# ai4co/rl4co

Hardware: AMD Instinct MI355X
Metric: decode_steps_per_sec (higher is better)
Workload: dtype bf16; 1 GPU; BASELINE configs[1]: TSPEnv num_loc=100 batch=4096/GPU AttentionModel(3L,d128,h8) greedy rollout, bf16 encoder GEMMs, bf16 cache; leg=c2_greedy, batch_per_gpu=4096, cache_dtype=bf16, launch=pipeline, input=one synthetic batch resident in HBM, reused by every step, parallelism=replicas x1 (instances sharded)

## Files before the change

### include/rl4co_amd.h

```cpp
#ifndef RL4CO_AMD_H
#define RL4CO_AMD_H

#include <stdint.h>

#ifdef __cplusplus
extern "C" {
#endif

#define RL4CO_ABI_VERSION 15

#define RL4CO_OK 0
#define RL4CO_ERR_ARG 1
#define RL4CO_ERR_HIP 2
#define RL4CO_ERR_UNSUPPORTED 3

#define RL4CO_EBIT_NAN_LOGIT 1
#define RL4CO_EBIT_INFEASIBLE 2
#define RL4CO_EBIT_INVALID_TOUR 4
#define RL4CO_EBIT_CAPACITY 8
#define RL4CO_EBIT_MAX_STEPS 16
#define RL4CO_EBIT_NEG_INF_LOGP 32
#define RL4CO_EBIT_DUPLICATES 64
#define RL4CO_EBIT_MAX_LENGTH 128
#define RL4CO_EBIT_PRIZE 256
#define RL4CO_EBIT_NOT_ALL_NODES 512
#define RL4CO_EBIT_DEPOT_MIDDLE 1024
#define RL4CO_EBIT_NO_PICKUP 2048
#define RL4CO_EBIT_TW_NEGATIVE 4096
#define RL4CO_EBIT_TW_RETURN 8192
#define RL4CO_EBIT_TW_DURATION 16384
#define RL4CO_EBIT_TW_EMPTY 32768
#define RL4CO_EBIT_TW_DEADLINE 65536

#define RL4CO_ENV_TSP 0
#define RL4CO_ENV_CVRP 1
#define RL4CO_ENV_OP 2
#define RL4CO_ENV_PCTSP 3
#define RL4CO_ENV_PDP 4
#define RL4CO_ENV_CVRPTW 5
#define RL4CO_ENV_SDVRP 6
#define RL4CO_ENV_MTSP 7

#define RL4CO_DECODE_GREEDY 0
#define RL4CO_DECODE_SAMPLE 1
#define RL4CO_DECODE_EVALUATE 2

#define RL4CO_DT_F32 0
#define RL4CO_DT_BF16 1
#define RL4CO_DT_F16 2

#define RL4CO_VARIANT_AUTO 0
#define RL4CO_VARIANT_STREAM 1
#define RL4CO_VARIANT_LDS 2
#define RL4CO_VARIANT_WIDE 3
#define RL4CO_VARIANT_MS 4

#define RL4CO_EMBED_DIM 128
#define RL4CO_NUM_HEADS 8

const char* rl4co_version(void);
int rl4co_abi_version(void);
const char* rl4co_last_error(void);

int rl4co_gather_by_index_f32(const float* src, const int64_t* idx, int B, int N, int D,
                              int K, float* out, int32_t* err, void* stream);

int rl4co_tour_length_f32(const float* locs, const int64_t* actions, int B, int B_locs, int N,
                          int T, int prepend_depot, int negate, float* out, void* stream);
int rl4co_tour_length_dyn_f32(const float* locs, const int64_t* actions, int B, int B_locs, int N, int row_stride,
                              const int32_t* steps_dev, int t_add, int prepend_depot, int negate, float* out,
                              void* stream);

int rl4co_tsp_check_solution(const int64_t* actions, int B, int N, int T, int32_t* err,
                             void* stream);
int rl4co_cvrp_check_solution(const int64_t* actions, const float* demand,
                              const float* vehicle_capacity, int B, int B_inst, int N, int T,
                              int32_t* err, void* stream);

int rl4co_tsp_step(const int64_t* action, uint8_t* action_mask, int64_t* first_node,
                   int64_t* current_node, int64_t* step_i, uint8_t* done, int B, int N,
                   int32_t* err, void* stream);

int rl4co_sdvrp_step(const int64_t* action, float* demand_with_depot, float* used_capacity, const float* vehicle_capacity,
                     int64_t* current_node, uint8_t* action_mask, uint8_t* done, int B, int N, int32_t* err, void* stream);

int rl4co_mtsp_step(const int64_t* action, const float* locs, const int64_t* num_agents, int64_t* agent_idx,
                    float* current_length, float* max_subtour_length, int64_t* current_node, uint8_t* action_mask,
                    uint8_t* done, int B, int B_inst, int N, int32_t* err, void* stream);

int rl4co_cvrp_step(const int64_t* action, const float* demand, float* used_capacity,
                    const float* vehicle_capacity, uint8_t* visited, int64_t* current_node,
                    uint8_t* action_mask, uint8_t* done, int B, int B_inst, int N,
// ... 42 lines not shown
  const float* max_length;
  const float* time_windows;
  const float* durations;
  const float* rem_base;
  uint8_t* masks;
  int64_t* prev;
  int64_t* first;
  uint8_t* use_placeholder;
  float* rem;
  float* now;
  int32_t* err;
  uint32_t* mask_bits;
  int32_t mask_words;
  int32_t reserved1;
} rl4co_env_replay_args;

int rl4co_env_replay(const rl4co_env_replay_args* args, void* stream);

int rl4co_cvrptw_step(const int64_t* action, const float* demand, const float* locs, const float* time_windows,
                      const float* durations, float* used_capacity, const float* vehicle_capacity, float* current_time,
                      uint8_t* visited, int64_t* current_node, uint8_t* action_mask, uint8_t* done, int B, int B_inst, int N,
                      int32_t* err, void* stream);
int rl4co_cvrptw_check_solution(const int64_t* actions, const float* locs, const float* time_windows,
                                const float* durations, int B, int B_inst, int N, int T, int32_t* err, void* stream);

typedef struct rl4co_am_decode_args {
  int32_t env;
  int32_t B;
  int32_t B_inst;
  int32_t N;
  int32_t mode;
  int32_t max_steps;
  int32_t mask_inner;
  int32_t mask_logits;
  float tanh_clipping;
  float temperature;
  int32_t cache_dtype;
  int32_t variant;
  const void* glimpse_key;
  const void* glimpse_val;
  const void* logit_key;
  int64_t kvl_row_stride;
  int64_t kvl_batch_stride;
  const void* ctx_first;
  const void* ctx_cur;
  const float* q_bias;
  const float* q_step0;
  const float* w_cap;
  int32_t unfold;
  int32_t ctx_width;
  const float* node_embed;
  const float* w_ctx_t;
  const float* w_out_t;
  const float* w_placeholder;
  uint8_t* action_mask;
  int64_t* first_node;
  int64_t* current_node;
  int64_t* step_i;
  uint8_t* done;
  const float* demand;
  float* used_capacity;
  const float* vehicle_capacity;
  uint8_t* visited;
  const float* locs;
  const float* max_length;
  uint8_t* to_deliver;
  const float* time_windows;
  const float* durations;
  float* current_time;
  const float* w_time;
  const float* dyn_vectors;
  float* demand_state;
  const float* exp_noise;
  uint64_t philox_seed;
  uint64_t philox_offset;
  const uint64_t* philox_seed_dev;
  const int64_t* forced_actions;
  int32_t t0;
  int32_t out_stride;
  int64_t* actions;
  float* logps;
  float* all_logps;
  float* entropy;
  int32_t* n_steps;
  int32_t* steps_summary;
  int32_t* err;
  const float* mtsp_ctx;
  const int64_t* num_agents;
  int32_t ctx_dtype;
  int32_t reserved0;
  int64_t ctx_row_stride;
  int64_t ctx_batch_stride;
  int32_t top_k;
  float top_p;
  uint32_t* kept_bits;
  int32_t kept_words;
  int32_t reserved1;
} rl4co_am_decode_args;

int rl4co_am_decode(const rl4co_am_decode_args* args, void* stream);

int rl4co_am_decode_lds_bytes(int N, int env);

int rl4co_am_decode_row_groups(const rl4co_am_decode_args* args);
int rl4co_am_decode_variant(const rl4co_am_decode_args* args);

typedef struct rl4co_am_encoder_args {
  int32_t env;
  int32_t B;
  int32_t N;
  int32_t num_layers;
  int32_t norm;
  int32_t cache_dtype;
  int32_t act_dtype;
  int32_t ctx_dtype;
  const float* locs;
  const float* demand;
  const float* feature4;
  const float* feature5;
  const float* feature6;
  const float* w_init;
  const float* b_init;
  const float* w_depot;
  const float* b_depot;
  const float* w_extra;
  const float* b_extra;
  const void* wqkv_packed;
  const float* bqkv;
  const void* wo_packed;
  const float* bo;
  const float* n1_scale;
  const float* n1_shift;
  const void* w1_packed;
  const float* b1;
  const void* w2_packed;
  const float* b2;
  const float* n2_scale;
  const float* n2_shift;
  const void* wfold_packed;
  const float* w_fixed;
  void* kvl;
  int64_t kvl_plane_stride;
  int64_t kvl_batch_stride;
  void* ctx_first;
  void* ctx_cur;
  float* q_bias;
  float* hidden;
} rl4co_am_encoder_args;

int rl4co_am_encoder(const rl4co_am_encoder_args* args, void* stream);
int rl4co_am_encoder_max_nodes(void);

int rl4co_mlp_input_grad(const void* dy, const void* h, int64_t M, const void* w2t_packed, const void* w1t_packed, int dtype,
                         void* dh, void* dx, void* stream);

typedef struct rl4co_am_train_save {
  const void* x0;
  void* out;
  void* qkv;
  void* att;
  void* y1;
  void* x1;
  void* h;
  void* y2;
  float* lse;
  float* stats;
// ... 165 lines not shown
```

### rl4co_amd/_lib.py

```python
from __future__ import annotations

import ctypes as C
import os
from functools import lru_cache

from . import build as _build

RL4CO_OK = 0
ABI_VERSION = 15
ENV_TSP, ENV_CVRP, ENV_OP, ENV_PCTSP, ENV_PDP, ENV_CVRPTW, ENV_SDVRP, ENV_MTSP = 0, 1, 2, 3, 4, 5, 6, 7
DECODE_GREEDY, DECODE_SAMPLE, DECODE_EVALUATE = 0, 1, 2
DT_F32, DT_BF16, DT_F16 = 0, 1, 2
VARIANT_AUTO, VARIANT_STREAM, VARIANT_LDS, VARIANT_WIDE, VARIANT_MS = 0, 1, 2, 3, 4

EBIT_NAN_LOGIT = 1
EBIT_INFEASIBLE = 2
EBIT_INVALID_TOUR = 4
EBIT_CAPACITY = 8
EBIT_MAX_STEPS = 16
EBIT_NEG_INF_LOGP = 32
EBIT_DUPLICATES = 64
EBIT_MAX_LENGTH = 128
EBIT_PRIZE = 256
EBIT_NOT_ALL_NODES = 512
EBIT_DEPOT_MIDDLE = 1024
EBIT_NO_PICKUP = 2048
EBIT_TW_NEGATIVE, EBIT_TW_RETURN, EBIT_TW_DURATION, EBIT_TW_EMPTY, EBIT_TW_DEADLINE = 4096, 8192, 16384, 32768, 65536

ERROR_MESSAGES = {
    EBIT_NAN_LOGIT: "Logits contain NaNs",
    EBIT_INFEASIBLE: "infeasible action selected",
    EBIT_INVALID_TOUR: "Invalid tour",
    EBIT_CAPACITY: "Used more than capacity",
    EBIT_MAX_STEPS: "Exceeded maximum number of steps during decoding",
    EBIT_NEG_INF_LOGP: "Logprobs should not be -inf, check sampling procedure!",
    EBIT_DUPLICATES: "Duplicates",
    EBIT_MAX_LENGTH: "Max length exceeded",
    EBIT_PRIZE: "Total prize does not satisfy min total prize",
    EBIT_NOT_ALL_NODES: "Not visiting all nodes",
    EBIT_DEPOT_MIDDLE: "Going back to depot in the middle of the tour (not allowed)",
    EBIT_NO_PICKUP: "Deliverying without pick-up",
    EBIT_TW_NEGATIVE: "Time windows must be non-negative.",
    EBIT_TW_RETURN: "vehicle cannot perform service and get back to depot in time.",
    EBIT_TW_DURATION: "Service durations must be non-negative.",
    EBIT_TW_EMPTY: "there are unfeasible time windows",
    EBIT_TW_DEADLINE: "vehicle cannot start service before deadline",
}

_vp, _i32, _i64, _f32 = C.c_void_p, C.c_int32, C.c_int64, C.c_float


class AmDecodeArgs(C.Structure):

    _fields_ = [
        ("env", _i32), ("B", _i32), ("B_inst", _i32), ("N", _i32),
        ("mode", _i32), ("max_steps", _i32), ("mask_inner", _i32), ("mask_logits", _i32),
        ("tanh_clipping", _f32), ("temperature", _f32),
        ("cache_dtype", _i32), ("variant", _i32),
        ("glimpse_key", _vp), ("glimpse_val", _vp), ("logit_key", _vp),
        ("kvl_row_stride", _i64), ("kvl_batch_stride", _i64),
        ("ctx_first", _vp), ("ctx_cur", _vp), ("q_bias", _vp), ("q_step0", _vp), ("w_cap", _vp),
        ("unfold", _i32), ("ctx_width", _i32), ("node_embed", _vp), ("w_ctx_t", _vp), ("w_out_t", _vp),
        ("w_placeholder", _vp),
        ("action_mask", _vp), ("first_node", _vp), ("current_node", _vp), ("step_i", _vp),
        ("done", _vp),
        ("demand", _vp), ("used_capacity", _vp), ("vehicle_capacity", _vp), ("visited", _vp),
        ("locs", _vp), ("max_length", _vp), ("to_deliver", _vp),
        ("time_windows", _vp), ("durations", _vp), ("current_time", _vp), ("w_time", _vp),
        ("dyn_vectors", _vp), ("demand_state", _vp),
        ("exp_noise", _vp), ("philox_seed", C.c_uint64), ("philox_offset", C.c_uint64), ("philox_seed_dev", _vp),
        ("forced_actions", _vp),
        ("t0", _i32), ("out_stride", _i32),
        ("actions", _vp), ("logps", _vp), ("all_logps", _vp), ("entropy", _vp),
        ("n_steps", _vp), ("steps_summary", _vp), ("err", _vp),
        ("mtsp_ctx", _vp), ("num_agents", _vp),
        ("ctx_dtype", _i32), ("reserved0", _i32), ("ctx_row_stride", _i64), ("ctx_batch_stride", _i64),
        ("top_k", _i32), ("top_p", _f32), ("kept_bits", _vp), ("kept_words", _i32), ("reserved1", _i32),
    ]


class EnvReplayArgs(C.Structure):

    _fields_ = [
        ("env", _i32), ("B", _i32), ("B_inst", _i32), ("N", _i32), ("T", _i32), ("reserved0", _i32),
        ("actions", _vp),
        ("action_mask", _vp), ("current_node", _vp), ("done", _vp), ("first_node", _vp), ("step_i", _vp), ("visited", _vp),
        ("to_deliver", _vp), ("scalar", _vp), ("current_time", _vp),
        ("vehicle_capacity", _vp), ("demand", _vp), ("locs", _vp), ("max_length", _vp), ("time_windows", _vp),
        ("durations", _vp), ("rem_base", _vp),
        ("masks", _vp), ("prev", _vp), ("first", _vp), ("use_placeholder", _vp), ("rem", _vp), ("now", _vp), ("err", _vp),
        ("mask_bits", _vp), ("mask_words", _i32), ("reserved1", _i32),
    ]


class CrossAttnArgs(C.Structure):

    _fields_ = [
        ("B", _i32), ("B_inst", _i32), ("T", _i32), ("N", _i32),
        ("q", _vp), ("q_stride", _i64), ("kv", _vp), ("kv_stride", _i64),
        ("mask", _vp), ("mask_words", _i32), ("reserved0", _i32),
        ("out", _vp), ("lse", _vp), ("dout", _vp), ("dq", _vp), ("dkv", _vp), ("dq_partial", _vp),
    ]


SYMBOLS = {
    "rl4co_version": (C.c_char_p, []),
    "rl4co_last_error": (C.c_char_p, []),
    "rl4co_abi_version": (C.c_int, []),
    "rl4co_gather_by_index_f32": (C.c_int, [_vp, _vp, C.c_int, C.c_int, C.c_int, C.c_int, _vp, _vp, _vp]),
    "rl4co_tour_length_f32": (C.c_int, [_vp, _vp, C.c_int, C.c_int, C.c_int, C.c_int, C.c_int, C.c_int, _vp, _vp]),
    "rl4co_tour_length_dyn_f32": (C.c_int, [_vp, _vp, C.c_int, C.c_int, C.c_int, C.c_int, _vp, C.c_int, C.c_int, C.c_int, _vp, _vp]),
    "rl4co_tsp_check_solution": (C.c_int, [_vp, C.c_int, C.c_int, C.c_int, _vp, _vp]),
    "rl4co_cvrp_check_solution": (C.c_int, [_vp, _vp, _vp, C.c_int, C.c_int, C.c_int, C.c_int, _vp, _vp]),
    "rl4co_tsp_step": (C.c_int, [_vp, _vp, _vp, _vp, _vp, _vp, C.c_int, C.c_int, _vp, _vp]),
    "rl4co_cvrp_step": (C.c_int, [_vp, _vp, _vp, _vp, _vp, _vp, _vp, _vp, C.c_int, C.c_int, C.c_int, _vp, _vp]),
    "rl4co_sdvrp_step": (C.c_int, [_vp, _vp, _vp, _vp, _vp, _vp, _vp, C.c_int, C.c_int, _vp, _vp]),
    "rl4co_mtsp_step": (C.c_int, [_vp, _vp, _vp, _vp, _vp, _vp, _vp, _vp, _vp, C.c_int, C.c_int, C.c_int, _vp, _vp]),
    "rl4co_op_max_length": (C.c_int, [_vp, _vp, C.c_int, C.c_int, _vp, _vp]),
    "rl4co_op_step": (C.c_int, [_vp, _vp, _vp, _vp, _vp, _vp, _vp, _vp, _vp, C.c_int, C.c_int, C.c_int, _vp, _vp]),
    "rl4co_gather_sum_f32": (C.c_int, [_vp, _vp, C.c_int, C.c_int, C.c_int, C.c_int, _vp, _vp]),
    "rl4co_op_check_solution": (C.c_int, [_vp, _vp, _vp, C.c_int, C.c_int, C.c_int, C.c_int, _vp, _vp]),
    "rl4co_pctsp_step": (C.c_int, [_vp, _vp, _vp, _vp, _vp, _vp, _vp, _vp, C.c_int, C.c_int, C.c_int, _vp, _vp]),
    "rl4co_pctsp_check_solution": (C.c_int, [_vp, _vp, C.c_int, C.c_int, C.c_int, _vp, _vp]),
    "rl4co_cvrptw_step": (C.c_int, [_vp] * 12 + [C.c_int, C.c_int, C.c_int, _vp, _vp]),
    "rl4co_cvrptw_check_solution": (C.c_int, [_vp, _vp, _vp, _vp, C.c_int, C.c_int, C.c_int, C.c_int, _vp, _vp]),
    "rl4co_pdp_step": (C.c_int, [_vp, _vp, _vp, _vp, _vp, _vp, _vp, C.c_int, C.c_int, _vp, _vp]),
    "rl4co_pdp_check_solution": (C.c_int, [_vp, C.c_int, C.c_int, C.c_int, C.c_int, _vp, _vp]),
    "rl4co_env_replay": (C.c_int, [C.POINTER(EnvReplayArgs), _vp]),
    "rl4co_am_decode": (C.c_int, [C.POINTER(AmDecodeArgs), _vp]),
    "rl4co_am_teacher_backward": (C.c_int, [_vp, _vp]),
    "rl4co_am_teacher_max_nodes": (C.c_int, []),
    "rl4co_am_teacher_variant": (C.c_int, [_vp]),
    "rl4co_skip_inorm_fwd": (C.c_int, [C.c_int, _vp, _vp, _vp, _vp, C.c_float, C.c_int, C.c_int, _vp, _vp, _vp, _vp, _vp]),
    "rl4co_skip_inorm_bwd": (C.c_int, [C.c_int, _vp, _vp, _vp, _vp, _vp, C.c_int, C.c_int, _vp, _vp, _vp, _vp]),
    "rl4co_skip_lnorm_fwd": (C.c_int, [C.c_int, _vp, _vp, C.c_float, C.c_int, C.c_int, _vp, _vp, _vp, _vp]),
    "rl4co_skip_lnorm_bwd": (C.c_int, [C.c_int, _vp, _vp, _vp, C.c_int, C.c_int, _vp, _vp]),
    "rl4co_skip_inorm_max_nodes": (C.c_int, []),
    "rl4co_mlp_input_grad": (C.c_int, [_vp, _vp, C.c_int64, _vp, _vp, C.c_int, _vp, _vp, _vp]),
    "rl4co_skip_bnorm_stats": (C.c_int, [C.c_int, _vp, _vp, C.c_int64, _vp, _vp, _vp]),
    "rl4co_bnorm_apply": (C.c_int, [C.c_int, _vp, _vp, _vp, _vp, _vp, C.c_int64, _vp, _vp]),
    "rl4co_skip_bnorm_eval": (C.c_int, [C.c_int, _vp, _vp, _vp, _vp, _vp, _vp, C.c_int64, _vp, _vp]),
    "rl4co_bnorm_bwd": (C.c_int, [C.c_int, _vp, _vp, _vp, _vp, _vp, C.c_int64, _vp, _vp, _vp]),
    "rl4co_init_embed": (C.c_int, [C.c_int, _vp, _vp, _vp, C.c_int64, C.c_int, _vp, _vp]),
    "rl4co_init_embed_wgrad": (C.c_int, [C.c_int, _vp, _vp, C.c_int64, C.c_int, _vp, _vp, _vp]),
    "rl4co_linear": (C.c_int, [C.c_int, _vp, _vp, _vp, _vp, _vp, C.c_int64, C.c_int, C.c_int, C.c_int, _vp, _vp]),
    "rl4co_attn_fwd": (C.c_int, [C.c_int, _vp, C.c_int, C.c_int, _vp, _vp, _vp]),
    "rl4co_attn_bwd": (C.c_int, [C.c_int, _vp, _vp, _vp, _vp, C.c_int, C.c_int, _vp, _vp]),
    "rl4co_attn_max_nodes": (C.c_int, []),
    "rl4co_attn_bwd_wide": (C.c_int, [C.c_int, _vp, _vp, _vp, _vp, C.c_int, C.c_int, _vp, _vp, _vp]),
    "rl4co_attn_wide_max_nodes": (C.c_int, []),
    "rl4co_cross_attn_fwd": (C.c_int, [C.c_int, C.POINTER(CrossAttnArgs), _vp]),
    "rl4co_cross_attn_bwd": (C.c_int, [C.c_int, C.POINTER(CrossAttnArgs), _vp]),
    "rl4co_cross_attn_chunks": (C.c_int, [C.c_int]),
    "rl4co_logit_logp_fwd": (C.c_int, [_vp, _vp, C.c_int, _vp, C.c_int64, C.c_int, C.c_float, C.c_float, _vp, _vp, _vp, _vp]),
    "rl4co_logit_logp_bwd": (C.c_int, [_vp, _vp, C.c_int, _vp, _vp, _vp, C.c_int64, C.c_int, C.c_float, C.c_float, _vp, _vp]),
    "rl4co_skip_inorm_wide_max_nodes": (C.c_int, []),
# ... 105 lines not shown
```

### rl4co_amd/build.py

```python
from __future__ import annotations

import hashlib
import os
import shutil
import subprocess
from concurrent.futures import ThreadPoolExecutor
from pathlib import Path

PKG_DIR = Path(__file__).resolve().parent
CSRC = PKG_DIR / "csrc"
INCLUDE = PKG_DIR.parent / "include"
LIB_DIR = PKG_DIR / "lib"
OBJ_DIR = LIB_DIR / "obj"
LIB_PATH = LIB_DIR / "librl4co_amd.so"
HASH_PATH = LIB_DIR / "librl4co_amd.so.hash"

SOURCES = ["api.hip", "entry16.hip", "env_step.hip", "tour_length.hip", "am_decode.hip", "am_decode_ms.hip", "am_encoder.hip", "am_encoder_f32.hip", "am_tokens_f32.hip", "am_teacher.hip", "am_teacher_mma.hip", "am_train_ops.hip", "am_train_attn.hip", "am_attn_flash.hip", "am_cross_attn.hip", "am_logit_logp.hip", "augment.hip",
           "am_train_ops_f16.hip", "am_train_attn_f16.hip", "am_attn_flash_f16.hip", "am_cross_attn_f16.hip",
           "am_decode_ms_f16.hip", "am_teacher_mma_f16.hip"]
HEADERS = ["common.h", "rl4co_math.h", "topkp.h", "elem16.h", "enc_f32.h"]
INCLUDED = {name: [name.replace("_f16.hip", ".hip")] for name in SOURCES if name.endswith("_f16.hip")}
COMPILE_FLAGS = [
    "--offload-arch=gfx950",
    "-O3",
    "-std=c++17",
    "-ffp-contract=off",
    "-fPIC",
]
FLAGS = COMPILE_FLAGS + ["-shared"]


def _hipcc() -> str:
    exe = shutil.which("hipcc") or "/opt/rocm/bin/hipcc"
    if not os.path.exists(exe):
        raise RuntimeError("hipcc not found: cannot build librl4co_amd.so")
    return exe


def _common_hash() -> "hashlib._Hash":
    h = hashlib.sha256()
    for name in HEADERS:
        h.update(name.encode())
        h.update((CSRC / name).read_bytes())
    h.update((INCLUDE / "rl4co_amd.h").read_bytes())
    h.update(" ".join(COMPILE_FLAGS).encode())
    return h


def _object_hash(name: str) -> str:
    h = _common_hash()
    for part in [name] + INCLUDED.get(name, []):
        h.update(part.encode())
        h.update((CSRC / part).read_bytes())
    return h.hexdigest()


def source_hash() -> str:
    h = hashlib.sha256()
    for name in SOURCES:
        h.update(_object_hash(name).encode())
    return h.hexdigest()


def is_fresh() -> bool:
    return LIB_PATH.exists() and HASH_PATH.exists() and HASH_PATH.read_text().strip() == source_hash()


def _compile(name: str, verbose: bool) -> Path:
    obj = OBJ_DIR / (name + ".o")
    stamp = OBJ_DIR / (name + ".o.hash")
    want = _object_hash(name)
    if obj.exists() and stamp.exists() and stamp.read_text().strip() == want:
        return obj
    tmp = OBJ_DIR / f"{name}.o.tmp.{os.getpid()}"
    cmd = [_hipcc(), *COMPILE_FLAGS, f"-I{INCLUDE}", "-c", str(CSRC / name), "-o", str(tmp)]
    if verbose:
        print(" ".join(cmd))
    proc = subprocess.run(cmd, capture_output=True, text=True)
    if proc.returncode != 0:
        raise RuntimeError(f"hipcc failed on {name} ({proc.returncode}):\n{proc.stdout}\n{proc.stderr}")
    os.replace(tmp, obj)
    stamp.write_text(want + "\n")
    return obj


def build_library(force: bool = False, verbose: bool = False) -> Path:
    if not force and is_fresh():
        return LIB_PATH
    OBJ_DIR.mkdir(parents=True, exist_ok=True)
    if force:
        for f in OBJ_DIR.glob("*.o.hash"):
            f.unlink()
    jobs = max(1, min(len(SOURCES), len(os.sched_getaffinity(0)), int(os.environ.get("RL4CO_BUILD_JOBS", "8"))))
    order = sorted(SOURCES, key=lambda n: -sum((CSRC / p).stat().st_size for p in [n] + INCLUDED.get(n, [])))
    with ThreadPoolExecutor(max_workers=jobs) as pool:
        objs = dict(zip(order, pool.map(lambda n: _compile(n, verbose), order)))
    tmp = LIB_DIR / f"librl4co_amd.so.tmp.{os.getpid()}"
    cmd = [_hipcc(), "--offload-arch=gfx950", "-shared", "-fPIC", "-o", str(tmp)] + [str(objs[n]) for n in SOURCES]
    if verbose:
        print(" ".join(cmd))
    proc = subprocess.run(cmd, capture_output=True, text=True)
    if proc.returncode != 0:
        raise RuntimeError(f"link failed ({proc.returncode}):\n{proc.stdout}\n{proc.stderr}")
# ... 8 lines not shown
```

### rl4co_amd/csrc/am_decode.hip

```cpp
#include <hip/hip_runtime.h>

#include "common.h"
#include "rl4co_math.h"
#include "topkp.h"

namespace {

constexpr int kD = RL4CO_EMBED_DIM;
constexpr int kH = RL4CO_NUM_HEADS;
constexpr int kDH = kD / kH;
constexpr int kUnroll = 4;
constexpr int kLdsWaves = 4;
constexpr int kLdsGroups = 16;
constexpr float kNegInf = -__builtin_huge_valf();
constexpr float kSqrtD = 11.3137084989847604f;

struct CacheF32 {
  using elem = float;
  using raw = float4;
  static constexpr int EPL = 4;
  __device__ static inline raw zero() { return make_float4(0.f, 0.f, 0.f, 0.f); }
  __device__ static inline raw ld(const elem* p) { return *reinterpret_cast<const float4*>(p); }
  __device__ static inline void cvt(const raw& t, float (&v)[4]) {
    v[0] = t.x; v[1] = t.y; v[2] = t.z; v[3] = t.w;
  }
};

struct CacheBF16 {
  using elem = uint16_t;
  using raw = uint4;
  static constexpr int EPL = 8;
  __device__ static inline raw zero() { return make_uint4(0u, 0u, 0u, 0u); }
  __device__ static inline raw ld(const elem* p) { return *reinterpret_cast<const uint4*>(p); }
  __device__ static inline void cvt(const raw& t, float (&v)[8]) {
    v[0] = __uint_as_float(t.x << 16); v[1] = __uint_as_float(t.x & 0xffff0000u);
    v[2] = __uint_as_float(t.y << 16); v[3] = __uint_as_float(t.y & 0xffff0000u);
    v[4] = __uint_as_float(t.z << 16); v[5] = __uint_as_float(t.z & 0xffff0000u);
    v[6] = __uint_as_float(t.w << 16); v[7] = __uint_as_float(t.w & 0xffff0000u);
  }
};

struct CacheF16 {
  using elem = uint16_t;
  using raw = uint4;
  static constexpr int EPL = 8;
  typedef _Float16 half2_t __attribute__((ext_vector_type(2)));
  __device__ static inline raw zero() { return make_uint4(0u, 0u, 0u, 0u); }
  __device__ static inline raw ld(const elem* p) { return *reinterpret_cast<const uint4*>(p); }
  __device__ static inline void cvt(const raw& t, float (&v)[8]) {
    const half2_t a = __builtin_bit_cast(half2_t, t.x), b = __builtin_bit_cast(half2_t, t.y);
    const half2_t c = __builtin_bit_cast(half2_t, t.z), d = __builtin_bit_cast(half2_t, t.w);
    v[0] = (float)a[0]; v[1] = (float)a[1]; v[2] = (float)b[0]; v[3] = (float)b[1];
    v[4] = (float)c[0]; v[5] = (float)c[1]; v[6] = (float)d[0]; v[7] = (float)d[1];
  }
};

__host__ __device__ inline int lds_pad(int N) { return (N + 63) & ~63; }

template <class C>
struct CtxTables {
  const char *cur, *first;
  int64_t rs;
  bool half;
  __device__ inline CtxTables(const rl4co_am_decode_args& a, int cb, int N, int e0) {
    half = a.ctx_dtype != RL4CO_DT_F32;
    const int64_t esz = half ? 2 : 4;
    rs = (a.ctx_row_stride ? a.ctx_row_stride : (int64_t)kD) * esz;
    const int64_t off = ((int64_t)cb * (a.ctx_batch_stride ? a.ctx_batch_stride : (int64_t)N * kD) + e0) * esz;
    cur = a.ctx_cur ? static_cast<const char*>(a.ctx_cur) + off : nullptr;
    first = a.ctx_first ? static_cast<const char*>(a.ctx_first) + off : nullptr;
  }
  __device__ inline void load(const char* table, int64_t row, float (&v)[C::EPL]) const {
    const char* p = table + row * rs;
    if constexpr (sizeof(typename C::elem) == 2) {
      if (half) {
        C::cvt(C::ld(reinterpret_cast<const typename C::elem*>(p)), v);
        return;
      }
    }
#pragma unroll
    for (int e = 0; e < C::EPL; ++e) v[e] = reinterpret_cast<const float*>(p)[e];
  }
};

__device__ inline int trajectory_of_block(int b, int B, int B_inst) {
  const int S = B / B_inst;
  if (S == 1 || (B_inst & 7) != 0) return b;
// ... 259 lines not shown
    for (int j = lane; j < N; j += 64) {
      all_visited &= vis[j] != 0;
      if (j >= 1) {
        const bool masked = (vis[j] != 0) || (dem[j - 1] + st.used > thr);
        mk[j] = masked ? 0 : 1;
        any_feasible |= !masked;
      }
    }
    any_feasible = __any(any_feasible);
    st.done = __all(all_visited);
    if (lane == 0) mk[0] = ((st.cur == 0) && any_feasible) ? 0 : 1;
    if (ENV == RL4CO_ENV_CVRPTW) {
      wave_lds_sync();
      const float bx = oplocs[2 * bi], by = oplocs[2 * bi + 1];
      for (int j = lane; j < N; j += 64) {
        const float dx = oplocs[2 * j] - bx, dy = oplocs[2 * j + 1] - by;
        if (!(st.time + sqrtf(fmaf(dy, dy, dx * dx)) <= opmax[2 * j + 1])) mk[j] = 0;
      }
    }
  }
  wave_lds_sync();
  return bi;
}

template <int EPL>
__device__ inline void gemv_t(float (&out)[EPL], const float* __restrict__ wt, const float* in_lds, int width, int e0) {
#pragma unroll
  for (int e = 0; e < EPL; ++e) out[e] = 0.0f;
  for (int k = 0; k < width; ++k) {
    const float c = in_lds[k];
#pragma unroll
    for (int e = 0; e < EPL; ++e) out[e] = fmaf(wt[(int64_t)k * kD + e0 + e], c, out[e]);
  }
}

constexpr int kRowCacheNone = 0xFF;
__host__ __device__ inline int row_cache_bytes(int N, int S, int esz) {
  return S > 0 ? S * 3 * kD * esz + lds_pad(N) + S : 0;
}

template <class C, int ENV, bool UNFOLD = false, bool FILT = false>
__global__ void __launch_bounds__(64) am_decode_kernel(const rl4co_am_decode_args a, const int S) {
  constexpr int EPL = C::EPL;
  constexpr int LPR = kD / EPL;
  constexpr int RPL = 64 / LPR;
  constexpr int LPH = kDH / EPL;
  constexpr bool kRowCache = !UNFOLD && (ENV == RL4CO_ENV_TSP || ENV == RL4CO_ENV_CVRP);
  constexpr bool kDyn = ENV == RL4CO_ENV_SDVRP;
  constexpr bool kMtsp = ENV == RL4CO_ENV_MTSP;
  constexpr int NG = ((kDyn || kMtsp) && RPL == 4) ? kUnroll : 1;
  static_assert(NG == 1 || (kUnroll == 4 && kLdsWaves == 4 && kLdsGroups == 16), "SDVRP: STREAM must keep the LDS / WIDE summation tree");
  using elem = typename C::elem;
  using raw_t = typename C::raw;

  extern __shared__ __align__(16) unsigned char smem[];
  const int lane = threadIdx.x;
  const int r = trajectory_of_block(blockIdx.x, a.B, a.B_inst);
  const int N = a.N;
  const int Np = lds_pad(N);
  float* sc = reinterpret_cast<float*>(smem);
  float* lg = sc + Np * kH;
  float* mh = lg + Np;
  uint16_t* fl = reinterpret_cast<uint16_t*>(mh + kH);
  uint8_t* mk = reinterpret_cast<uint8_t*>(fl + Np);
  uint8_t* vis = mk + Np;
  elem* rc = reinterpret_cast<elem*>(vis + Np);
  uint8_t* rslot = reinterpret_cast<uint8_t*>(rc + S * 3 * kD);
  uint8_t* rpend = rslot + Np;
  float* dd = reinterpret_cast<float*>(vis + Np);

  const int cb = r % a.B_inst;
  const int rg = lane / LPR;
  const int li = lane % LPR;
  const int hd = li / LPH;
  const int e0 = li * EPL;

  const elem* Kg = static_cast<const elem*>(a.glimpse_key) + (int64_t)cb * a.kvl_batch_stride + e0;
  const elem* Vg = static_cast<const elem*>(a.glimpse_val) + (int64_t)cb * a.kvl_batch_stride + e0;
  const elem* Kl = static_cast<const elem*>(a.logit_key) + (int64_t)cb * a.kvl_batch_stride + e0;
  const int64_t rs = a.kvl_row_stride;
  const CtxTables<C> ctx(a, cb, N, e0);
  const float* hrow = UNFOLD ? a.node_embed + (int64_t)cb * N * kD + e0 : nullptr;

  uint8_t* gmask = a.action_mask + (int64_t)r * N;
  for (int j = lane; j < Np; j += 64) mk[j] = (j < N) ? gmask[j] : (uint8_t)0;
  constexpr bool kScalarCtx = ENV == RL4CO_ENV_CVRP || ENV == RL4CO_ENV_OP || ENV == RL4CO_ENV_PCTSP || ENV == RL4CO_ENV_CVRPTW || kDyn || kMtsp;
  constexpr bool kCvrpLike = ENV == RL4CO_ENV_CVRP || ENV == RL4CO_ENV_CVRPTW;
  if (ENV == RL4CO_ENV_PDP) {
    const uint8_t* gv = a.visited + (int64_t)r * N;
    const uint8_t* gt = a.to_deliver + (int64_t)r * N;
    for (int j = lane; j < Np; j += 64) vis[j] = (j < N) ? (uint8_t)((gv[j] != 0 ? 1 : 0) | (gt[j] != 0 ? 2 : 0)) : (uint8_t)0;
  } else if (kDyn) {
    const float* gd = a.demand_state + (int64_t)r * N;
    for (int j = lane; j < Np; j += 64) dd[j] = (j < N) ? gd[j] : 0.0f;
  } else if (ENV != RL4CO_ENV_TSP && !kMtsp) {
    const uint8_t* gv = a.visited + (int64_t)r * N;
    for (int j = lane; j < Np; j += 64) vis[j] = (j < N) ? gv[j] : (uint8_t)1;
  }
  TrajState st;
  st.cur = (int)a.current_node[r];
  st.first = (ENV == RL4CO_ENV_TSP) ? (int)a.first_node[r] : 0;
  st.step_i = !(kCvrpLike || kDyn) ? a.step_i[r] : 0;
  st.time = (ENV == RL4CO_ENV_CVRPTW || kMtsp) ? a.current_time[r] : 0.0f;
  st.used = kScalarCtx ? a.used_capacity[r] : 0.0f;
  st.done = a.done[r] != 0;
  st.errbits = 0;
  st.ent_acc = 0.0f;
  const float* oplocs = (ENV == RL4CO_ENV_OP || ENV == RL4CO_ENV_CVRPTW || kMtsp) ? a.locs + (int64_t)cb * N * 2 : nullptr;
  const float* opmax = (ENV == RL4CO_ENV_OP)       ? a.max_length + (int64_t)cb * N
                       : (ENV == RL4CO_ENV_CVRPTW) ? a.time_windows + (int64_t)cb * N * 2
                                                   : nullptr;
  const float* twdur = (ENV == RL4CO_ENV_CVRPTW) ? a.durations + (int64_t)cb * N : nullptr;
  const float cap = (kCvrpLike || ENV == RL4CO_ENV_PCTSP || kDyn) ? a.vehicle_capacity[r]
                                                                      : ((ENV == RL4CO_ENV_OP) ? opmax[0] : 0.0f);
  const float* dem = kCvrpLike                  ? a.demand + (int64_t)cb * (N - 1)
                     : (ENV == RL4CO_ENV_PCTSP) ? a.demand + (int64_t)cb * N
                                                : nullptr;
  wave_lds_sync();

  const bool list_all = !(a.mask_inner && a.mask_logits);
  auto candidate = [&](int j) -> bool {
    return list_all || (ENV == RL4CO_ENV_TSP ? mk[j] != 0 : (j == 0 || vis[j] == 0));
  };
  const bool caching = kRowCache && S > 0;
  if (caching) {
    for (int j = lane; j < Np; j += 64) rslot[j] = (uint8_t)kRowCacheNone;
    wave_lds_sync();
    int k = 0;
    for (int j0 = N - 1; j0 >= 0 && k < S; j0 -= 64) {
      const int j = j0 - lane;
      const bool f = j >= 0 && candidate(j);
      const unsigned long long bal = __ballot(f);
      const int s = k + __popcll(bal & ((1ull << lane) - 1ull));
      if (f && s < S) {
        rslot[j] = (uint8_t)s;
        rpend[s] = 1;
      }
      k += __popcll(bal);
    }
    wave_lds_sync();
  }
  auto lds_row = [&](int j, int plane) -> const elem* { return rc + (rslot[j] * 3 + plane) * kD + e0; };
  auto fill_row = [&](int j, int plane, const raw_t& v) {
    const int s = rslot[j];
    if (s != kRowCacheNone) *reinterpret_cast<raw_t*>(rc + (s * 3 + plane) * kD + e0) = v;
  };

  float qb[EPL];
#pragma unroll
  for (int e = 0; e < EPL; ++e) qb[e] = a.q_bias ? a.q_bias[(int64_t)cb * kD + e0 + e] : 0.0f;

  const float* dynv = kDyn ? a.dyn_vectors + e0 : nullptr;
  const float* mg = kMtsp ? a.mtsp_ctx + e0 : nullptr;
  const long long nag = kMtsp ? a.num_agents[cb] : 0;
  const bool single = a.max_steps == 1;
  int t = 0;
  int rows_read = 0;

  for (; t < a.max_steps && (!st.done || single); ++t) {
    const int F = build_list(a, mk, fl, N, lane);
    int hend = F, pbeg = F;
    if (caching) {
      const int c_lo = max(F - S, 0);
      int last_hbm = c_lo - 1, first_pend = F;
      for (int c = c_lo + lane; c < F; c += 64) {
        const int s = rslot[fl[c]];
        const bool pend = s != kRowCacheNone && rpend[s] != 0;
        if (s == kRowCacheNone || pend) last_hbm = c;
        if (pend) first_pend = min(first_pend, c);
      }
      hend = rl4co::bfly_i_max(last_hbm) + 1;
      pbeg = -rl4co::bfly_i_max(-first_pend);
    }
    rows_read += hend;

    float q[EPL];
    if constexpr (UNFOLD) {
      float* cv = sc;
      if (rg == 0) {
        if (ENV == RL4CO_ENV_TSP) {
          const bool ph = st.step_i < 1;
#pragma unroll
          for (int e = 0; e < EPL; ++e) {
            cv[e0 + e] = ph ? a.w_placeholder[e0 + e] : hrow[(int64_t)st.first * kD + e];
            cv[kD + e0 + e] = ph ? a.w_placeholder[kD + e0 + e] : hrow[(int64_t)st.cur * kD + e];
          }
        } else {
#pragma unroll
          for (int e = 0; e < EPL; ++e) cv[e0 + e] = hrow[(int64_t)st.cur * kD + e];
          if (li == 0) cv[kD] = cap - st.used;
        }
      }
      wave_lds_sync();
      gemv_t<EPL>(q, a.w_ctx_t, cv, a.ctx_width, e0);
#pragma unroll
      for (int e = 0; e < EPL; ++e) q[e] = q[e] + qb[e];
      wave_lds_sync();
    } else if constexpr (kMtsp) {
      const float f0 = (float)(nag - st.step_i);
      const float ddx = oplocs[2 * st.cur] - oplocs[0], ddy = oplocs[2 * st.cur + 1] - oplocs[1];
// ... 130 lines not shown
               (rl4co::bfly_sum<LPR, 64>(term(2)) + rl4co::bfly_sum<LPR, 64>(term(3)));
      }
    };
    const float l = 1.0f / tree([&](int g) { return lacc[g]; });
    float o[EPL];
    if constexpr (kDyn) {
      const float pd = tree([&](int g) { return pdacc[g]; });
#pragma unroll
      for (int e = 0; e < EPL; ++e) o[e] = fmaf(pd, dynv[kD + e], tree([&](int g) { return oacc[g][e]; })) * l;
    } else {
#pragma unroll
      for (int e = 0; e < EPL; ++e) o[e] = tree([&](int g) { return oacc[g][e]; }) * l;
    }
    if constexpr (UNFOLD) {
      wave_lds_sync();
      if (rg == 0) {
#pragma unroll
        for (int e = 0; e < EPL; ++e) sc[e0 + e] = o[e];
      }
      wave_lds_sync();
      gemv_t<EPL>(o, a.w_out_t, sc, kD, e0);
    }

    float ul = 0.0f;
    if constexpr (kDyn) {
#pragma unroll
      for (int e = 0; e < EPL; ++e) ul = fmaf(o[e], dynv[2 * kD + e], ul);
      ul = rl4co::bfly_sum<1, LPR>(ul);
    }
    auto logit = [&](const raw_t& rw, int c) {
      float k[EPL];
      C::cvt(rw, k);
      float acc = 0.0f;
#pragma unroll
      for (int e = 0; e < EPL; ++e) acc = fmaf(o[e], k[e], acc);
      acc = rl4co::bfly_sum<1, LPR>(acc);
      if constexpr (kDyn) {
        const int j = c < F ? (int)fl[c] : 0;
        acc = fmaf(j > 0 ? dd[j] : 0.0f, ul, acc);
      }
      if (c < F && li == 0) lg[c] = acc;
    };
    for (int c0 = 0; c0 < F; c0 += RPL * kUnroll) {
      raw_t rw[kUnroll];
#pragma unroll
      for (int u = 0; u < kUnroll; ++u) {
        const int c = c0 + u * RPL + rg;
        rw[u] = (c >= F) ? C::zero() : (c < hend ? C::ld(Kl + (int64_t)fl[c] * rs) : C::ld(lds_row(fl[c], 2)));
      }
#pragma unroll
      for (int u = 0; u < kUnroll; ++u) {
        const int c = c0 + u * RPL + rg;
        if (caching && c >= pbeg && c < hend) fill_row(fl[c], 2, rw[u]);
        logit(rw[u], c);
      }
    }
    if (caching) {
      for (int c = pbeg + lane; c < hend; c += 64) {
        const int s = rslot[fl[c]];
        if (s != kRowCacheNone) rpend[s] = 0;
      }
    }
    wave_lds_sync();

    const int bi = finalize_and_step<ENV, FILT>(a, st, lg, sc, fl, F, mk, vis, dem, cap, r, t, N, lane, oplocs, opmax, twdur, dd);
    if (caching && rslot[bi] != kRowCacheNone && !candidate(bi)) {
      int nxt = -1;
      for (int j = lane; j < N; j += 64)
        if (candidate(j) && rslot[j] == kRowCacheNone) nxt = j;
      nxt = rl4co::bfly_i_max(nxt);
      const int s = rslot[bi];
      wave_lds_sync();
      if (lane == 0) {
        rslot[bi] = (uint8_t)kRowCacheNone;
        if (nxt >= 0) {
          rslot[nxt] = (uint8_t)s;
          rpend[s] = 1;
        }
      }
      wave_lds_sync();
    }
  }
  if (!single && !st.done && t >= a.max_steps) st.errbits |= RL4CO_EBIT_MAX_STEPS;

  for (int j = lane; j < N; j += 64) gmask[j] = mk[j];
  if (ENV == RL4CO_ENV_PDP) {
    uint8_t* gv = a.visited + (int64_t)r * N;
    uint8_t* gt = a.to_deliver + (int64_t)r * N;
    for (int j = lane; j < N; j += 64) {
      gv[j] = vis[j] & 1;
      gt[j] = (vis[j] >> 1) & 1;
    }
  } else if (kDyn) {
    float* gd = a.demand_state + (int64_t)r * N;
    for (int j = lane; j < N; j += 64) gd[j] = dd[j];
  } else if (ENV != RL4CO_ENV_TSP && !kMtsp) {
    uint8_t* gv = a.visited + (int64_t)r * N;
    for (int j = lane; j < N; j += 64) gv[j] = vis[j];
  }
  if (lane == 0) {
    a.current_node[r] = st.cur;
    a.done[r] = st.done ? 1 : 0;
    if (ENV == RL4CO_ENV_TSP) a.first_node[r] = st.first;
    if (!(kCvrpLike || kDyn)) a.step_i[r] = st.step_i;
    if (ENV == RL4CO_ENV_CVRPTW || kMtsp) a.current_time[r] = st.time;
    if (kScalarCtx) a.used_capacity[r] = st.used;
    if (a.n_steps) a.n_steps[r] = t;
    if (a.steps_summary) {
      atomicMax(a.steps_summary, t);
      atomicAdd(a.steps_summary + 1, t);
      atomicAdd(reinterpret_cast<unsigned long long*>(a.steps_summary + 2), (unsigned long long)rows_read);
    }
    if (a.entropy) a.entropy[r] += st.ent_acc;
    if (st.errbits) atomicOr(a.err, (int)st.errbits);
  }
}


template <int ENV, bool FILT = false>
__device__ inline int wide_scores(const rl4co_am_decode_args& a, TrajState& st, float* lg, const uint16_t* fl, int F,
                                  const uint8_t* mk, float* xs, int nw, int r, int t, int N, int tid) {
  constexpr int T = 64 * kLdsWaves;
  const int w = tid >> 6, lane = tid & 63;
  float* ex = xs;
  float* xw = xs + 2 * nw;
  bool nan_seen = false;
  float zmax = kNegInf;
  for (int c = tid; c < F; c += T) {
    float z = lg[c] / kSqrtD;
    if (z != z) nan_seen = true;
    if (a.tanh_clipping > 0.0f) z = rl4co_tanhf(z) * a.tanh_clipping;
    if (a.mask_logits && mk[fl[c]] == 0) z = kNegInf;
    if (a.temperature != 1.0f) z = z / a.temperature;
    lg[c] = z;
    zmax = fmaxf(zmax, z);
  }
  zmax = rl4co::bfly_max<1, 64>(zmax);
  const bool wave_nan = __any(nan_seen);
  if (lane == 0) {
    xw[w] = zmax;
    xw[4 + w] = wave_nan ? 1.0f : 0.0f;
  }
  __syncthreads();
  zmax = fmaxf(fmaxf(xw[0], xw[1]), fmaxf(xw[2], xw[3]));
  if ((xw[4] + xw[5]) + (xw[6] + xw[7]) != 0.0f) st.errbits |= RL4CO_EBIT_NAN_LOGIT;
  for (int c = tid; c < F; c += T) ex[c] = rl4co_expf(lg[c] - zmax);
  __syncthreads();
  const int64_t tcol = (int64_t)a.t0 + t;
  constexpr bool filt = FILT;
  if (w == 0) {
    float zsum = 0.0f;
    if (filt) {
      zsum = rl4co::topkp_filter(lg, ex, F, a.top_k, a.top_p, lane);
      if (a.kept_bits)
        rl4co::topkp_write_bits(a.kept_bits + ((int64_t)r * a.out_stride + tcol) * a.kept_words, a.kept_words, lg, fl,
                                F, N, reinterpret_cast<uint32_t*>(xw + 16), lane);
    } else {
      for (int c = lane; c < F; c += 64) zsum = zsum + ex[c];
      zsum = rl4co::bfly_sum<1, 64>(zsum);
    }
    if (lane == 0) xw[8] = rl4co_logf(zsum);
  }
  __syncthreads();
  const float lse = xw[8];
  float* alp = a.all_logps ? a.all_logps + ((int64_t)r * a.out_stride + tcol) * N : nullptr;
  if (alp && F < N) {
// ... 474 lines not shown
template <class C, int ENV, bool UNFOLD = false>
int launch(const rl4co_am_decode_args& a, hipStream_t stream) {
  return rl4co::topkp_on(a) ? launch_f<C, ENV, UNFOLD, true>(a, stream) : launch_f<C, ENV, UNFOLD, false>(a, stream);
}

}

extern "C" int rl4co_am_decode_lds_bytes(int N, int env) {
  const int Np = lds_pad(N);
  return Np * kH * 4 + Np * 4 + kH * 4 + Np * 2 + Np + Np + (env == RL4CO_ENV_SDVRP ? Np * 4 : 0);
}

extern "C" int rl4co_am_decode_row_groups(const rl4co_am_decode_args* args) {
  if (args == nullptr) return -1;
  const int v = resolve_variant(*args);
  if (v < 0) return -1;
  if (v == RL4CO_VARIANT_MS) return 0;
  if (v == RL4CO_VARIANT_LDS || v == RL4CO_VARIANT_WIDE) return kLdsGroups;
  if ((args->env == RL4CO_ENV_SDVRP || args->env == RL4CO_ENV_MTSP) && args->cache_dtype != RL4CO_DT_F32) return kLdsGroups;
  return args->cache_dtype != RL4CO_DT_F32 ? 64 / (kD / CacheBF16::EPL) : 64 / (kD / CacheF32::EPL);
}

extern "C" int rl4co_am_decode_variant(const rl4co_am_decode_args* args) {
  return args == nullptr ? -1 : resolve_variant(*args);
}

extern "C" int rl4co_am_decode(const rl4co_am_decode_args* args, void* stream) {
  RL4CO_REQUIRE(args != nullptr);
  const rl4co_am_decode_args& a = *args;
  RL4CO_REQUIRE(a.env == RL4CO_ENV_TSP || a.env == RL4CO_ENV_CVRP || a.env == RL4CO_ENV_OP ||
                a.env == RL4CO_ENV_PCTSP || a.env == RL4CO_ENV_PDP || a.env == RL4CO_ENV_CVRPTW || a.env == RL4CO_ENV_SDVRP ||
                a.env == RL4CO_ENV_MTSP);
  RL4CO_REQUIRE(a.B > 0 && a.B_inst > 0 && a.B % a.B_inst == 0);
  RL4CO_REQUIRE(a.N >= 2 && a.N <= 4096);
  RL4CO_REQUIRE(a.max_steps >= 1);
  RL4CO_REQUIRE(a.mode >= RL4CO_DECODE_GREEDY && a.mode <= RL4CO_DECODE_EVALUATE);
  RL4CO_REQUIRE(a.cache_dtype == RL4CO_DT_F32 || a.cache_dtype == RL4CO_DT_BF16 || a.cache_dtype == RL4CO_DT_F16);
  RL4CO_REQUIRE(a.cache_dtype != RL4CO_DT_F16 || !a.unfold);
  RL4CO_REQUIRE(a.glimpse_key && a.glimpse_val && a.logit_key && (a.ctx_cur || a.unfold));
  RL4CO_REQUIRE(a.unfold == 0 || a.unfold == 1);
  RL4CO_REQUIRE(a.ctx_dtype == RL4CO_DT_F32 || (a.ctx_dtype == a.cache_dtype && !a.unfold));
  RL4CO_REQUIRE(a.ctx_row_stride == 0 || (a.ctx_row_stride >= kD && a.ctx_row_stride % 8 == 0));
  RL4CO_REQUIRE(a.ctx_batch_stride == 0 || (a.ctx_batch_stride >= (int64_t)a.N * kD && a.ctx_batch_stride % 8 == 0));
  RL4CO_REQUIRE(a.ctx_dtype == RL4CO_DT_F32 || ((reinterpret_cast<uintptr_t>(a.ctx_cur) | reinterpret_cast<uintptr_t>(a.ctx_first)) & 15) == 0);
  if (a.unfold) {
    RL4CO_REQUIRE(a.env == RL4CO_ENV_TSP || a.env == RL4CO_ENV_CVRP);
    RL4CO_REQUIRE(a.node_embed && a.w_ctx_t && a.w_out_t);
    RL4CO_REQUIRE(a.ctx_width == (a.env == RL4CO_ENV_TSP ? 2 * kD : kD + 1));
    RL4CO_REQUIRE(a.env != RL4CO_ENV_TSP || a.w_placeholder);
  }
  RL4CO_REQUIRE(a.kvl_row_stride >= kD && a.kvl_row_stride % 8 == 0);
  RL4CO_REQUIRE(a.kvl_batch_stride >= (int64_t)a.N * kD && a.kvl_batch_stride % 8 == 0);
  RL4CO_REQUIRE(a.action_mask && a.current_node && a.done && a.actions && a.logps && a.err);
  RL4CO_REQUIRE(a.out_stride >= 1 && a.t0 >= 0 && (int64_t)a.t0 + a.max_steps <= a.out_stride);
  RL4CO_REQUIRE(a.temperature > 0.0f);
  RL4CO_REQUIRE((reinterpret_cast<uintptr_t>(a.steps_summary) & 7) == 0);
  RL4CO_REQUIRE(a.mode != RL4CO_DECODE_EVALUATE || a.forced_actions != nullptr);
  RL4CO_REQUIRE(a.top_p == a.top_p && a.top_p <= 1.0f);
  RL4CO_REQUIRE(a.kept_bits == nullptr || (a.kept_words >= (a.N + 31) / 32 && a.kept_words % 4 == 0 &&
                                           (reinterpret_cast<uintptr_t>(a.kept_bits) & 3) == 0));
  if (a.env == RL4CO_ENV_TSP) {
    RL4CO_REQUIRE(((a.ctx_first && a.q_step0) || a.unfold) && a.first_node && a.step_i);
  } else if (a.env == RL4CO_ENV_CVRP) {
    RL4CO_REQUIRE((a.w_cap || a.unfold) && a.demand && a.used_capacity && a.vehicle_capacity && a.visited);
  } else if (a.env == RL4CO_ENV_CVRPTW) {
    RL4CO_REQUIRE(a.w_cap && a.w_time && a.demand && a.used_capacity && a.vehicle_capacity && a.visited);
    RL4CO_REQUIRE(a.locs && a.time_windows && a.durations && a.current_time);
  } else if (a.env == RL4CO_ENV_SDVRP) {
    RL4CO_REQUIRE(a.w_cap && a.dyn_vectors && a.demand_state && a.used_capacity && a.vehicle_capacity);
    RL4CO_REQUIRE((reinterpret_cast<uintptr_t>(a.dyn_vectors) & 15) == 0);
  } else if (a.env == RL4CO_ENV_MTSP) {
    RL4CO_REQUIRE(a.mtsp_ctx && a.num_agents && a.locs && a.used_capacity && a.current_time && a.step_i);
  } else if (a.env == RL4CO_ENV_PDP) {
    RL4CO_REQUIRE(a.visited && a.to_deliver && a.step_i && (a.N - 1) % 2 == 0);
  } else if (a.env == RL4CO_ENV_PCTSP) {
    RL4CO_REQUIRE(a.w_cap && a.demand && a.used_capacity && a.vehicle_capacity && a.step_i && a.visited);
  } else {
    RL4CO_REQUIRE(a.w_cap && a.locs && a.max_length && a.used_capacity && a.step_i && a.visited);
  }
  RL4CO_REQUIRE(rl4co_am_decode_lds_bytes(a.N, a.env) <= 160 * 1024);
  RL4CO_REQUIRE(a.variant >= RL4CO_VARIANT_AUTO && a.variant <= RL4CO_VARIANT_MS);
  const int variant = resolve_variant(a);
  RL4CO_REQUIRE(variant >= 0);
  hipStream_t s = rl4co::as_stream(stream);
  if (a.unfold) {
    if (a.cache_dtype == RL4CO_DT_F32)
      return a.env == RL4CO_ENV_TSP ? launch<CacheF32, RL4CO_ENV_TSP, true>(a, s) : launch<CacheF32, RL4CO_ENV_CVRP, true>(a, s);
    return a.env == RL4CO_ENV_TSP ? launch<CacheBF16, RL4CO_ENV_TSP, true>(a, s) : launch<CacheBF16, RL4CO_ENV_CVRP, true>(a, s);
  }
  if (variant == RL4CO_VARIANT_MS && a.cache_dtype == RL4CO_DT_F16) return rl4co::launch_decode_ms_f16(a, s);
  if (variant == RL4CO_VARIANT_MS) return rl4co::launch_decode_ms(a, s);
  if (variant == RL4CO_VARIANT_LDS || variant == RL4CO_VARIANT_WIDE) {
    const bool res = variant == RL4CO_VARIANT_LDS;
    switch (a.env) {
      case RL4CO_ENV_TSP: return res ? launch_wide<RL4CO_ENV_TSP, true>(a, s) : launch_wide<RL4CO_ENV_TSP, false>(a, s);
      case RL4CO_ENV_CVRP: return res ? launch_wide<RL4CO_ENV_CVRP, true>(a, s) : launch_wide<RL4CO_ENV_CVRP, false>(a, s);
      case RL4CO_ENV_OP: return res ? launch_wide<RL4CO_ENV_OP, true>(a, s) : launch_wide<RL4CO_ENV_OP, false>(a, s);
      case RL4CO_ENV_PCTSP: return res ? launch_wide<RL4CO_ENV_PCTSP, true>(a, s) : launch_wide<RL4CO_ENV_PCTSP, false>(a, s);
      case RL4CO_ENV_PDP: return res ? launch_wide<RL4CO_ENV_PDP, true>(a, s) : launch_wide<RL4CO_ENV_PDP, false>(a, s);
      case RL4CO_ENV_SDVRP: return res ? launch_wide<RL4CO_ENV_SDVRP, true>(a, s) : launch_wide<RL4CO_ENV_SDVRP, false>(a, s);
      case RL4CO_ENV_MTSP: return res ? launch_wide<RL4CO_ENV_MTSP, true>(a, s) : launch_wide<RL4CO_ENV_MTSP, false>(a, s);
      default: return res ? launch_wide<RL4CO_ENV_CVRPTW, true>(a, s) : launch_wide<RL4CO_ENV_CVRPTW, false>(a, s);
    }
  }
  if (a.cache_dtype == RL4CO_DT_F16) {
    switch (a.env) {
      case RL4CO_ENV_TSP: return launch<CacheF16, RL4CO_ENV_TSP>(a, s);
      case RL4CO_ENV_CVRP: return launch<CacheF16, RL4CO_ENV_CVRP>(a, s);
      case RL4CO_ENV_OP: return launch<CacheF16, RL4CO_ENV_OP>(a, s);
      case RL4CO_ENV_PCTSP: return launch<CacheF16, RL4CO_ENV_PCTSP>(a, s);
      case RL4CO_ENV_PDP: return launch<CacheF16, RL4CO_ENV_PDP>(a, s);
      case RL4CO_ENV_SDVRP: return launch<CacheF16, RL4CO_ENV_SDVRP>(a, s);
      case RL4CO_ENV_MTSP: return launch<CacheF16, RL4CO_ENV_MTSP>(a, s);
      default: return launch<CacheF16, RL4CO_ENV_CVRPTW>(a, s);
    }
  }
  if (a.env == RL4CO_ENV_MTSP)
    return a.cache_dtype == RL4CO_DT_F32 ? launch<CacheF32, RL4CO_ENV_MTSP>(a, s) : launch<CacheBF16, RL4CO_ENV_MTSP>(a, s);
  if (a.env == RL4CO_ENV_SDVRP)
    return a.cache_dtype == RL4CO_DT_F32 ? launch<CacheF32, RL4CO_ENV_SDVRP>(a, s) : launch<CacheBF16, RL4CO_ENV_SDVRP>(a, s);
  if (a.env == RL4CO_ENV_CVRPTW)
    return a.cache_dtype == RL4CO_DT_F32 ? launch<CacheF32, RL4CO_ENV_CVRPTW>(a, s)
                                         : launch<CacheBF16, RL4CO_ENV_CVRPTW>(a, s);
  if (a.env == RL4CO_ENV_PDP)
    return a.cache_dtype == RL4CO_DT_F32 ? launch<CacheF32, RL4CO_ENV_PDP>(a, s) : launch<CacheBF16, RL4CO_ENV_PDP>(a, s);
  if (a.env == RL4CO_ENV_PCTSP)
    return a.cache_dtype == RL4CO_DT_F32 ? launch<CacheF32, RL4CO_ENV_PCTSP>(a, s)
                                         : launch<CacheBF16, RL4CO_ENV_PCTSP>(a, s);
  if (a.env == RL4CO_ENV_OP)
    return a.cache_dtype == RL4CO_DT_F32 ? launch<CacheF32, RL4CO_ENV_OP>(a, s) : launch<CacheBF16, RL4CO_ENV_OP>(a, s);
  if (a.cache_dtype == RL4CO_DT_F32) {
    return a.env == RL4CO_ENV_TSP ? launch<CacheF32, RL4CO_ENV_TSP>(a, s)
                                  : launch<CacheF32, RL4CO_ENV_CVRP>(a, s);
  }
  return a.env == RL4CO_ENV_TSP ? launch<CacheBF16, RL4CO_ENV_TSP>(a, s)
                                : launch<CacheBF16, RL4CO_ENV_CVRP>(a, s);
}
```

### rl4co_amd/csrc/tour_length.hip

```cpp
#include <hip/hip_runtime.h>

#include "common.h"

namespace {

struct TourView {
  const float* locs;
  const int64_t* actions;
  int prepend;
  int n;
  const float* values;
  __device__ inline float2 point(int t) const {
    int node;
    if (prepend) node = (t == 0) ? 0 : (int)actions[t - 1];
    else node = (int)actions[t];
    return *reinterpret_cast<const float2*>(locs + 2 * (int64_t)node);
  }
  __device__ inline float seg(int t) const {
    if (values) return values[actions[t]];
    const float2 p0 = point(t);
    const float2 p1 = point(t + 1 == n ? 0 : t + 1);
    const float dx = p1.x - p0.x;
    const float dy = p1.y - p0.y;
    return sqrtf(fmaf(dy, dy, dx * dx));
  }
};

__device__ float lane_row_sum(const TourView& tv, int lane8, int nvec) {
  constexpr int kIlp = 4;
  constexpr int kLevels = 4;
  const int size = nvec / kIlp;
  int ceil_log2 = 0;
  while ((1LL << ceil_log2) < size) ++ceil_log2;
  int level_power = ceil_log2 / kLevels;
  if (level_power < 4) level_power = 4;
  const int level_step = 1 << level_power;
  const int level_mask = level_step - 1;
  float acc[kLevels][kIlp];
  for (int l = 0; l < kLevels; ++l)
    for (int k = 0; k < kIlp; ++k) acc[l][k] = 0.0f;
  int i = 0;
  for (; i + level_step <= size;) {
    for (int j = 0; j < level_step; ++j, ++i) {
      for (int k = 0; k < kIlp; ++k) acc[0][k] = acc[0][k] + tv.seg(8 * (i * kIlp + k) + lane8);
    }
    for (int j = 1; j < kLevels; ++j) {
      for (int k = 0; k < kIlp; ++k) {
        acc[j][k] = acc[j][k] + acc[j - 1][k];
        acc[j - 1][k] = 0.0f;
      }
      const int mask = level_mask << (j * level_power);
      if ((i & mask) != 0) break;
    }
  }
  for (; i < size; ++i) {
    for (int k = 0; k < kIlp; ++k) acc[0][k] = acc[0][k] + tv.seg(8 * (i * kIlp + k) + lane8);
  }
  for (int j = 1; j < kLevels; ++j)
    for (int k = 0; k < kIlp; ++k) acc[0][k] = acc[0][k] + acc[j][k];
  for (int v = size * kIlp; v < nvec; ++v) acc[0][0] = acc[0][0] + tv.seg(8 * v + lane8);
  for (int k = 1; k < kIlp; ++k) acc[0][0] = acc[0][0] + acc[0][k];
  return acc[0][0];
}

__global__ void __launch_bounds__(256) tour_length_kernel(const float* __restrict__ locs,
                                                          const int64_t* __restrict__ actions,
                                                          int B, int B_locs, int N, int T,
                                                          int prepend, int negate,
                                                          float* __restrict__ out,
                                                          const float* __restrict__ gather_values,
                                                          int row_stride, const int32_t* __restrict__ t_dev, int t_add) {
  const int gid = blockIdx.x * blockDim.x + threadIdx.x;
  const int b = gid >> 3;
  const int lane8 = gid & 7;
  const bool active = b < B;
  if (t_dev) T = min(row_stride, t_add + *t_dev);
  TourView tv;
  tv.prepend = prepend;
  tv.n = T + prepend;
  tv.locs = locs ? locs + (int64_t)(active ? b % B_locs : 0) * N * 2 : nullptr;
  tv.actions = actions + (int64_t)(active ? b : 0) * row_stride;
  tv.values = gather_values ? gather_values + (int64_t)(active ? b % B_locs : 0) * N : nullptr;
  const int n = tv.n;
  const int nvec = n / 8;
  if (n < 8) {
    if (active && lane8 == 0) {
      float p[4] = {0.0f, 0.0f, 0.0f, 0.0f};
      const int g = n / 4;
      for (int i = 0; i < g; ++i)
        for (int k = 0; k < 4; ++k) p[k] = p[k] + tv.seg(4 * i + k);
      for (int k = 4 * g; k < n; ++k) p[0] = p[0] + tv.seg(k);
      for (int k = 1; k < 4; ++k) p[0] = p[0] + p[k];
      out[b] = negate ? -p[0] : p[0];
    }
    return;
  }
  float part = 0.0f;
  if (active) part = lane_row_sum(tv, lane8, nvec);
  float fin = 0.0f;
  if (active && lane8 == 0) {
    for (int k = nvec * 8; k < n; ++k) fin = fin + tv.seg(k);
  }
  const int base = (threadIdx.x & 63) & ~7;
  for (int l = 0; l < 8; ++l) {
    const float pl = __shfl(part, base + l, 64);
    fin = fin + pl;
  }
  if (active && lane8 == 0) out[b] = negate ? -fin : fin;
}

__global__ void gather_kernel(const float* __restrict__ src, const int64_t* __restrict__ idx, int B,
                              int N, int D, int K, float* __restrict__ out, int32_t* err) {
  const int64_t total = (int64_t)B * K * D;
  for (int64_t g = (int64_t)blockIdx.x * blockDim.x + threadIdx.x; g < total;
       g += (int64_t)gridDim.x * blockDim.x) {
    const int d = (int)(g % D);
    const int64_t bk = g / D;
    const int b = (int)(bk / K);
    int64_t n = idx[bk];
    if (n < 0 || n >= N) {
      if (err) atomicOr(err, RL4CO_EBIT_INVALID_TOUR);
      n = 0;
    }
    out[g] = src[((int64_t)b * N + n) * D + d];
  }
}

__global__ void __launch_bounds__(64) tsp_check_kernel(const int64_t* __restrict__ actions, int B,
                                                       int N, int T, int32_t* err) {
  extern __shared__ unsigned int seen[];
  const int b = blockIdx.x;
  const int lane = threadIdx.x;
  const int words = (N + 31) / 32;
  for (int w = lane; w < words; w += 64) seen[w] = 0;
  __syncthreads();
  bool bad = (T != N);
  for (int t = lane; t < T; t += 64) {
    const int64_t a = actions[(int64_t)b * T + t];
    if (a < 0 || a >= N) {
      bad = true;
    } else {
      const unsigned int bit = 1u << (a & 31);
      const unsigned int old = atomicOr(&seen[a >> 5], bit);
      if (old & bit) bad = true;
    }
  }
  if (__any(bad) && lane == 0) atomicOr(err, RL4CO_EBIT_INVALID_TOUR);
}

__global__ void __launch_bounds__(64) cvrp_check_kernel(const int64_t* __restrict__ actions,
                                                        const float* __restrict__ demand,
                                                        const float* __restrict__ capacity, int B,
                                                        int B_inst, int N, int T, int32_t* err) {
  extern __shared__ unsigned int seen[];
  const int b = blockIdx.x;
  const int lane = threadIdx.x;
  const int words = (N + 31) / 32;
  for (int w = lane; w < words; w += 64) seen[w] = 0;
  __syncthreads();
  bool bad = false;
  int customers = 0;
  for (int t = lane; t < T; t += 64) {
    const int64_t a = actions[(int64_t)b * T + t];
    if (a < 0 || a >= N) {
      bad = true;
    } else if (a > 0) {
      const unsigned int bit = 1u << (a & 31);
      const unsigned int old = atomicOr(&seen[a >> 5], bit);
      if (old & bit) bad = true;
      ++customers;
    }
  }
  for (int s = 1; s < 64; s <<= 1) customers += __shfl_xor(customers, s, 64);
  if (customers != N - 1) bad = true;
  if (__any(bad) && lane == 0) atomicOr(err, RL4CO_EBIT_INVALID_TOUR);
  if (lane == 0) {
    const int inst = b % B_inst;
    const float cap = capacity[inst];
    const float thr = cap + 1e-5f;
    float used = 0.0f;
    bool over = false;
    for (int t = 0; t < T; ++t) {
      int64_t a = actions[(int64_t)b * T + t];
      if (a < 0 || a >= N) a = 0;
      const float d = (a == 0) ? -cap : demand[(int64_t)inst * (N - 1) + (a - 1)];
      used = used + d;
      if (used < 0.0f) used = 0.0f;
      if (!(used <= thr)) over = true;
    }
    if (over) atomicOr(err, RL4CO_EBIT_CAPACITY);
  }
}

__global__ void select_start_nodes_kernel(int64_t* out, int B, int S, int num_loc, int has_depot) {
  const int64_t total = (int64_t)B * S;
  for (int64_t g = (int64_t)blockIdx.x * blockDim.x + threadIdx.x; g < total;
       g += (int64_t)gridDim.x * blockDim.x) {
    const int64_t s = g / B;
    out[g] = s % num_loc + (has_depot ? 1 : 0);
  }
}

__global__ void __launch_bounds__(256) hbm_read_probe_kernel(const float4* __restrict__ src,
                                                             int64_t n16, float* sink) {
  float acc = 0.0f;
  for (int64_t g = (int64_t)blockIdx.x * blockDim.x + threadIdx.x; g < n16;
       g += (int64_t)gridDim.x * blockDim.x) {
    const float4 v = src[g];
    acc += v.x + v.y + v.z + v.w;
  }
  if (acc == 123.456f) sink[0] = acc;
}

}

extern "C" int rl4co_tour_length_f32(const float* locs, const int64_t* actions, int B, int B_locs,
                                     int N, int T, int prepend_depot, int negate, float* out,
                                     void* stream) {
  RL4CO_REQUIRE(locs && actions && out);
  RL4CO_REQUIRE(B > 0 && B_locs > 0 && B % B_locs == 0 && N > 0 && T > 0);
  const int threads = 256;
  const int64_t total = (int64_t)B * 8;
  const int blocks = (int)((total + threads - 1) / threads);
  hipLaunchKernelGGL(tour_length_kernel, dim3(blocks), dim3(threads), 0, rl4co::as_stream(stream),
                     locs, actions, B, B_locs, N, T, prepend_depot ? 1 : 0, negate ? 1 : 0, out,
                     static_cast<const float*>(nullptr), T, static_cast<const int32_t*>(nullptr), 0);
  RL4CO_HIP_TRY(hipGetLastError());
  return RL4CO_OK;
}

extern "C" int rl4co_tour_length_dyn_f32(const float* locs, const int64_t* actions, int B, int B_locs, int N, int row_stride,
                                         const int32_t* steps_dev, int t_add, int prepend_depot, int negate, float* out,
                                         void* stream) {
  RL4CO_REQUIRE(locs && actions && out && steps_dev);
  RL4CO_REQUIRE(B > 0 && B_locs > 0 && B % B_locs == 0 && N > 0 && row_stride > 0 && t_add >= 0);
  const int threads = 256;
  const int64_t total = (int64_t)B * 8;
  const int blocks = (int)((total + threads - 1) / threads);
  hipLaunchKernelGGL(tour_length_kernel, dim3(blocks), dim3(threads), 0, rl4co::as_stream(stream), locs, actions, B, B_locs, N,
                     row_stride, prepend_depot ? 1 : 0, negate ? 1 : 0, out, static_cast<const float*>(nullptr), row_stride,
                     steps_dev, t_add);
  RL4CO_HIP_TRY(hipGetLastError());
  return RL4CO_OK;
}

extern "C" int rl4co_gather_sum_f32(const float* values, const int64_t* actions, int B, int B_values, int N, int T, float* out,
                                    void* stream) {
  RL4CO_REQUIRE(values && actions && out);
  RL4CO_REQUIRE(B > 0 && B_values > 0 && B % B_values == 0 && N > 0 && T > 0);
  const int threads = 256;
  const int64_t total = (int64_t)B * 8;
  const int blocks = (int)((total + threads - 1) / threads);
  hipLaunchKernelGGL(tour_length_kernel, dim3(blocks), dim3(threads), 0, rl4co::as_stream(stream),
                     static_cast<const float*>(nullptr), actions, B, B_values, N, T, 0, 0, out, values, T,
                     static_cast<const int32_t*>(nullptr), 0);
  RL4CO_HIP_TRY(hipGetLastError());
  return RL4CO_OK;
}

extern "C" int rl4co_gather_by_index_f32(const float* src, const int64_t* idx, int B, int N, int D,
                                         int K, float* out, int32_t* err, void* stream) {
  RL4CO_REQUIRE(src && idx && out);
  RL4CO_REQUIRE(B > 0 && N > 0 && D > 0 && K > 0);
  const int64_t total = (int64_t)B * K * D;
  int blocks = (int)((total + 255) / 256);
  if (blocks > 8192) blocks = 8192;
  hipLaunchKernelGGL(gather_kernel, dim3(blocks), dim3(256), 0, rl4co::as_stream(stream), src, idx,
                     B, N, D, K, out, err);
  RL4CO_HIP_TRY(hipGetLastError());
  return RL4CO_OK;
}

extern "C" int rl4co_tsp_check_solution(const int64_t* actions, int B, int N, int T, int32_t* err,
                                        void* stream) {
// ... 40 lines not shown
```

### rl4co_amd/envs.py

```python
from __future__ import annotations

import os

import torch
import torch.nn.functional as F
from torch import Tensor

from . import kernels as K
from .tensordict import TensorDict

CAPACITIES = {
    10: 20.0, 15: 25.0, 20: 30.0, 30: 33.0, 40: 37.0, 50: 40.0, 60: 43.0, 75: 45.0,
    100: 50.0, 125: 55.0, 150: 60.0, 200: 70.0, 500: 100.0, 1000: 150.0,
}


class Generator:

    def __call__(self, batch_size) -> TensorDict:
        batch_size = [batch_size] if isinstance(batch_size, int) else list(batch_size)
        return self._generate(batch_size)

    def _generate(self, batch_size) -> TensorDict:
        raise NotImplementedError
# ... 93 lines not shown
        max_times[..., 0] = int(self.max_time)
        mask = min_times == max_times
        if bool(mask.any()):
            min_times = torch.where(mask, torch.max(dist.int(), min_times - 1), min_times)
            mask = min_times == max_times
            if bool(mask.any()):
                widened = torch.min(torch.floor(upper_bound).int(),
                                    torch.max(torch.ceil(min_times + durations).int(), max_times + 1))
                max_times = torch.where(mask, widened, max_times)
        if self.scale:
            durations, min_times, max_times = durations / self.max_time, min_times / self.max_time, max_times / self.max_time
            depot, locs = depot / self.max_time, locs / self.max_time
        time_windows = torch.stack((min_times, max_times), dim=-1)
        assert bool((min_times < max_times).all()), \
            "Please make sure the relation between max_loc and max_time allows for feasible solutions."
        return TensorDict({"locs": locs, "depot": depot, "demand": demand / self.capacity, "capacity": capacity,
                           "durations": durations, "time_windows": time_windows}, batch_size=batch_size)


OP_MAX_LENGTHS = {20: 2.0, 50: 3.0, 100: 4.0}


class OPGenerator(TSPGenerator):

    def __init__(self, num_loc: int = 20, min_loc: float = 0.0, max_loc: float = 1.0, prize_type: str = "dist",
                 max_length: float | None = None, device="cpu", **unused):
        super().__init__(num_loc, min_loc, max_loc, device)
        assert prize_type in ("dist", "unif", "const"), f"Invalid prize_type: {prize_type}"
        self.prize_type = prize_type
        if max_length is None:
            max_length = OP_MAX_LENGTHS.get(num_loc, None)
        if max_length is None:
            closest = min(OP_MAX_LENGTHS.keys(), key=lambda x: abs(x - num_loc))
            max_length = OP_MAX_LENGTHS[closest]
        self.max_length = max_length

    def _generate(self, batch_size) -> TensorDict:
        locs_with_depot = self._uniform((*batch_size, self.num_loc + 1, 2), self.min_loc, self.max_loc)
        dev = locs_with_depot.device
        if self.prize_type == "const":
            prize = torch.ones(*batch_size, self.num_loc, device=dev)
        elif self.prize_type == "unif":
            prize = (1 + torch.randint(0, 100, (*batch_size, self.num_loc), device=dev).float()) / 100
        else:
            prize = (locs_with_depot[..., 0:1, :] - locs_with_depot[..., 1:, :]).norm(p=2, dim=-1)
            prize = (1 + (prize / prize.max(dim=-1, keepdim=True)[0] * 99).int()).float() / 100
        max_length = torch.full((*batch_size,), self.max_length, device=dev)
        return TensorDict({"locs": locs_with_depot[..., 1:, :], "depot": locs_with_depot[..., 0, :], "prize": prize,
                           "max_length": max_length}, batch_size=batch_size)


class PCTSPGenerator(TSPGenerator):

    def __init__(self, num_loc: int = 20, min_loc: float = 0.0, max_loc: float = 1.0, penalty_factor: float = 3.0,
                 prize_required: float = 1.0, max_penalty: float | None = None, device="cpu", **unused):
        super().__init__(num_loc, min_loc, max_loc, device)
        self.prize_required = prize_required
        if max_penalty is None:
            max_penalty = OP_MAX_LENGTHS.get(num_loc, None)
        if max_penalty is None:
            closest = min(OP_MAX_LENGTHS.keys(), key=lambda x: abs(x - num_loc))
            max_penalty = OP_MAX_LENGTHS[closest]
        self.max_penalty = max_penalty * penalty_factor / num_loc

    def _generate(self, batch_size) -> TensorDict:
        locs_with_depot = self._uniform((*batch_size, self.num_loc + 1, 2), self.min_loc, self.max_loc)
        penalty = self._uniform((*batch_size, self.num_loc), 0.0, self.max_penalty)
        det = self._uniform((*batch_size, self.num_loc), 0.0, 4.0 / self.num_loc)
        sto = self._uniform((*batch_size, self.num_loc), 0.0, 2.0) * det
        return TensorDict({"locs": locs_with_depot[..., 1:, :], "depot": locs_with_depot[..., 0, :], "penalty": penalty,
                           "deterministic_prize": det, "stochastic_prize": sto}, batch_size=batch_size)


class PDPGenerator(TSPGenerator):

    def __init__(self, num_loc: int = 20, min_loc: float = 0.0, max_loc: float = 1.0, device="cpu", **unused):
        super().__init__(num_loc + (num_loc % 2), min_loc, max_loc, device)

    def _generate(self, batch_size) -> TensorDict:
        locs = self._uniform((*batch_size, self.num_loc + 1, 2), self.min_loc, self.max_loc)
        return TensorDict({"locs": locs[..., 1:, :], "depot": locs[..., 0, :]}, batch_size=batch_size)


def _zero_state(device, **fields) -> dict:
    offs, total = {}, 0
    for name, (shape, dtype) in fields.items():
        nbytes = int(torch.tensor([], dtype=dtype).element_size())
        for d in shape:
            nbytes *= int(d)
        offs[name] = (total, nbytes)
        total += (nbytes + 15) // 16 * 16
    buf = torch.zeros(max(total, 16), dtype=torch.uint8, device=device)
    return {name: buf[o : o + nb].view(fields[name][1]).view(fields[name][0]) for name, (o, nb) in offs.items()}


class RL4COEnvBase:

    name = "base"
    has_depot = False

    def __init__(self, *, generator: Generator | None = None, generator_params: dict | None = None,
                 check_solution: bool = True, device="cuda", seed: int | None = None, **unused):
        self.check_solution = check_solution
        self.device = torch.device(device)
        self.data_dir = unused.get("data_dir", "data/")
        for phase in ("train", "val", "test"):
            f = unused.get(f"{phase}_file", None)
            setattr(self, f"{phase}_file", None if f is None else os.path.join(self.data_dir, f))
        self.generator = generator if generator is not None else self._default_generator(**(generator_params or {}))
        if seed is not None:
            torch.manual_seed(seed)

    def reset(self, td: TensorDict | None = None, batch_size=None) -> TensorDict:
        if batch_size is None:
            batch_size = [] if td is None else td.batch_size
        if td is None or (td.is_empty() if hasattr(td, "is_empty") else len(td) == 0):
            td = self.generator(batch_size=batch_size)
        batch_size = [batch_size] if isinstance(batch_size, int) else list(batch_size)
        td = td.to(self.device)
        out = self._reset(td, batch_size=batch_size)
        if "terminated" not in out.keys():
            out.set("terminated", torch.zeros_like(out["done"]))
        return out

    def step(self, td: TensorDict) -> dict:
        return {"next": self._step(td)}

    def get_reward(self, td: TensorDict, actions: Tensor, check_solution: bool | None = None, horizon=None) -> Tensor:
        check_solution = self.check_solution if check_solution is None else check_solution
        if check_solution:
            self.check_solution_validity(td, actions)
        return self._get_reward(td, actions) if horizon is None else self._get_reward(td, actions, horizon=horizon)

    def accepts_reward_horizon(self) -> bool:
        import inspect

        try:
            return "horizon" in inspect.signature(type(self)._get_reward).parameters
        except (TypeError, ValueError):
            return False

    def dataset(self, batch_size=(), phase: str = "train", filename: str | None = None):
        from .data import TensorDictDataset

        f = getattr(self, f"{phase}_file", None) if filename is None else filename
        batch_size = [batch_size] if isinstance(batch_size, int) else list(batch_size)
        td = None
        if f is not None:
            try:
                td = self.load_data(f, batch_size, device=self.device)
            except FileNotFoundError:
                td = None
        if td is None:
            td = self.generator(batch_size=batch_size)
        return TensorDictDataset(td)

    @staticmethod
    def load_data(fpath, batch_size=(), device=None):
        from .data import load_npz_to_tensordict

        return load_npz_to_tensordict(fpath, device=device)

    def get_num_starts(self, td) -> int:
        num_starts = td["action_mask"].shape[-1]
        return num_starts - 1 if self.has_depot else num_starts

    def select_start_nodes(self, td, num_starts: int) -> Tensor:
        num_loc = getattr(self.generator, "num_loc", 0xFFFFFFFF)
        batch = td["action_mask"].shape[0]
        return K.select_start_nodes(batch, num_starts, num_loc, self.has_depot, td["action_mask"].device)

    def to(self, device):
        if device is not None:
            self.device = torch.device(device)
        return self

    def _default_generator(self, **kw) -> Generator:
        raise NotImplementedError

    def _reset(self, td, batch_size):
        raise NotImplementedError

    def _step(self, td):
        raise NotImplementedError

    def _get_reward(self, td, actions):
        raise NotImplementedError

    def check_solution_validity(self, td, actions) -> None:
        raise NotImplementedError


class TSPEnv(RL4COEnvBase):
    name = "tsp"
    has_depot = False

    def _default_generator(self, **kw):
        return TSPGenerator(**kw)

    def _reset(self, td: TensorDict, batch_size) -> TensorDict:
        init_locs = td["locs"].contiguous()
        device = init_locs.device
        b = init_locs.shape[0]
        num_loc = init_locs.shape[-2]
        z = _zero_state(device, first_node=((b,), torch.int64), current_node=((b,), torch.int64), i=((b, 1), torch.int64),
                        reward=((b, 1), torch.float32), done=((b,), torch.bool))
        return TensorDict(
            {
                "locs": init_locs,
                "first_node": z["first_node"],
                "current_node": z["current_node"],
                "i": z["i"],
                "action_mask": torch.ones((b, num_loc), dtype=torch.bool, device=device),
                "reward": z["reward"],
                "done": z["done"],
            },
            batch_size=[b],
        )

    def _step(self, td: TensorDict) -> TensorDict:
        K.tsp_step(td["action"].contiguous(), td["action_mask"], td["first_node"], td["current_node"],
                   td["i"], td["done"])
        return td

    def _get_reward(self, td: TensorDict, actions: Tensor, horizon=None) -> Tensor:
        return K.tour_length(td["locs"].contiguous(), actions.contiguous(), prepend_depot=False, negate=True, horizon=horizon)

    def check_solution_validity(self, td: TensorDict, actions: Tensor, err: Tensor | None = None) -> None:
        own = err is None
        err = K.new_error_word(actions.device) if own else err
        K.tsp_check_solution(actions.contiguous(), td["locs"].shape[-2], err)
        if own:
            K.raise_if_error(err)


class CVRPEnv(RL4COEnvBase):
    name = "cvrp"
    has_depot = True

    def _default_generator(self, **kw):
        return CVRPGenerator(**kw)

    def _reset(self, td: TensorDict, batch_size) -> TensorDict:
        device = td["locs"].device
        b = td["locs"].shape[0]
        n = td["locs"].shape[-2] + 1
        td_reset = TensorDict(
            {
                "locs": torch.cat((td["depot"][:, None, :], td["locs"]), -2).contiguous(),
                "demand": td["demand"].contiguous(),
                "current_node": torch.zeros(b, 1, dtype=torch.long, device=device),
                "used_capacity": torch.zeros((b, 1), device=device),
                "vehicle_capacity": torch.full((b, 1), self.generator.vehicle_capacity, device=device),
                "visited": torch.zeros((b, n), dtype=torch.uint8, device=device),
                "action_mask": torch.zeros((b, n), dtype=torch.bool, device=device),
                "done": torch.zeros((b,), dtype=torch.bool, device=device),
            },
            batch_size=[b],
        )
        self.get_action_mask(td_reset)
        return td_reset

    def _step(self, td: TensorDict) -> TensorDict:
        K.cvrp_step(td["action"].contiguous(), td["demand"], td["used_capacity"], td["vehicle_capacity"],
                    td["visited"], td["current_node"], td["action_mask"], td["done"])
        return td

    def get_action_mask(self, td: TensorDict) -> Tensor:
        K.cvrp_step(None, td["demand"], td["used_capacity"], td["vehicle_capacity"], td["visited"],
                    td["current_node"], td["action_mask"], None)
        return td["action_mask"]

    @staticmethod
    def load_data(fpath, batch_size=(), device=None):
        from .data import load_npz_to_tensordict

        td = load_npz_to_tensordict(fpath, device=device)
        td.set("demand", td["demand"] / td["capacity"][:, None])
        return td

    def _get_reward(self, td: TensorDict, actions: Tensor, horizon=None) -> Tensor:
        return K.tour_length(td["locs"].contiguous(), actions.contiguous(), prepend_depot=True, negate=True, horizon=horizon)

    def check_solution_validity(self, td: TensorDict, actions: Tensor, err: Tensor | None = None) -> None:
        own = err is None
        err = K.new_error_word(actions.device) if own else err
        K.cvrp_check_solution(actions.contiguous(), td["demand"], td["vehicle_capacity"].reshape(-1).contiguous(), err)
        if own:
            K.raise_if_error(err)


class SDVRPEnv(CVRPEnv):

    name = "sdvrp"

    def _reset(self, td: TensorDict, batch_size) -> TensorDict:
        device = td["locs"].device
        b = td["locs"].shape[0]
        n = td["locs"].shape[-2] + 1
        demand = td["demand"].contiguous()
        td_reset = TensorDict(
            {
                "locs": torch.cat((td["depot"][:, None, :], td["locs"]), -2).contiguous(),
                "demand": demand,
                "demand_with_depot": torch.cat((torch.zeros_like(demand[:, :1]), demand), -1).contiguous(),
                "current_node": torch.zeros(b, 1, dtype=torch.long, device=device),
                "used_capacity": torch.zeros((b, 1), device=device),
                "vehicle_capacity": torch.full((b, 1), self.generator.vehicle_capacity, device=device),
                "action_mask": torch.zeros((b, n), dtype=torch.bool, device=device),
                "done": torch.zeros((b,), dtype=torch.bool, device=device),
            },
            batch_size=[b],
        )
        self.get_action_mask(td_reset)
        return td_reset

    def _step(self, td: TensorDict) -> TensorDict:
        K.sdvrp_step(td["action"].contiguous(), td["demand_with_depot"], td["used_capacity"], td["vehicle_capacity"],
                     td["current_node"], td["action_mask"], td["done"])
        return td

    def get_action_mask(self, td: TensorDict) -> Tensor:
        K.sdvrp_step(None, td["demand_with_depot"], td["used_capacity"], td["vehicle_capacity"], td["current_node"],
                     td["action_mask"], None)
        return td["action_mask"]

    def check_solution_validity(self, td: TensorDict, actions: Tensor, err: Tensor | None = None) -> None:
        b = actions.shape[0]
        demand, cap = td["demand"], td["vehicle_capacity"].reshape(-1)
        s = b // demand.shape[0]
        if s > 1:
            demand = demand.unsqueeze(0).expand(s, *demand.shape).reshape(b, -1)
            cap = cap if cap.shape[0] == b else cap.repeat(s)
        demands = torch.cat((-cap[:, None], demand), 1).clone()
        rng = torch.arange(b, device=actions.device)
        used = torch.zeros_like(cap)
        bad = torch.zeros(b, dtype=torch.bool, device=actions.device)
        a_prev = None
        for a in actions.transpose(0, 1):
            if a_prev is not None:
                bad |= (a_prev == 0) & (a == 0) & (demands != 0).any(-1)
            d = torch.min(demands[rng, a], cap - used)
            demands[rng, a] -= d
# ... 317 lines not shown
```

### rl4co_amd/envspec.py

```python
from __future__ import annotations

from typing import Callable, NamedTuple

import torch

from . import _lib

KERNEL_ENV = {"spctsp": "pctsp"}


def canonical_env(env_name: str) -> str:
    return KERNEL_ENV.get(env_name, env_name)


class Field(NamedTuple):
    key: str
    kind: str
    dtype: str
    slot: str | None
    shape: str


class Scalar(NamedTuple):
    running: str
    base: str
    base_col0: bool = False
    clamp: bool = False
    clock: str | None = None


class Features(NamedTuple):
    names: tuple[str, ...]
    weight: str


class Dynamic(NamedTuple):
    key: str
    weight: str
    slot: str


class EnvSpec(NamedTuple):
    name: str
    env_id: int
    has_depot: bool
    horizon: Callable[[int], int]
    fields: tuple[Field, ...]
    scalar: Scalar | None
    step: tuple[str, tuple[str, ...]]
    passthrough: tuple[str, ...]
    features: tuple[tuple[str, bool, int], ...] = ()
    init: str = "depot"
    ctx_first: bool = False
    feats: Features | None = None
    dynamic: Dynamic | None = None
    state_reward: bool = False
    fixed_horizon: bool = False
    length_reward: bool = False
    depot_flag: str | None = None
    unfold: bool = False
    replay: bool = True
    no_teacher: str | None = None

    @property
    def teacher(self) -> bool:
        return self.no_teacher is None

    @property
    def feature_width(self) -> int:
        return sum(width for _, _, width in self.features)

    def keys(self, kind: str | None = None) -> tuple[str, ...]:
        return tuple(f.key for f in self.fields if kind in (None, f.kind))

    @property
    def teacher_keys(self) -> tuple[str, ...]:
        base = () if self.scalar is None or self.scalar.base_col0 else (self.scalar.base,)
        return self.keys("inst") + base


def _fields(current_node: str, *own: tuple) -> tuple[Field, ...]:
    common = (("action_mask", "traj", "u8", "action_mask", "BN"), ("current_node", "traj", "i64", "current_node", current_node),
              ("done", "traj", "u8", "done", "B"))
    return tuple(Field(*f) for f in common + own)


_I = ("i", "traj", "i64", "step_i", "B")
_VISITED = ("visited", "traj", "u8", "visited", "BN")
_CVRP_FIELDS = (("demand", "inst", "f32", "demand", "N-1"), ("used_capacity", "traj", "f32", "used_capacity", "B1"),
                ("vehicle_capacity", "traj", "f32", "vehicle_capacity", "B1"), _VISITED)

SPECS = {s.name: s for s in (
    EnvSpec("tsp", _lib.ENV_TSP, False, lambda n: n,
            _fields("B", ("first_node", "traj", "i64", "first_node", "B"), ("i", "traj", "i64", "step_i", "B1")),
            None, ("tsp_step", ("action_mask", "first_node", "current_node", "i", "done")),
            ("locs",), init="all", ctx_first=True, fixed_horizon=True, length_reward=True, unfold=True),
    EnvSpec("cvrp", _lib.ENV_CVRP, True, lambda n: 2 * n, _fields("B1", *_CVRP_FIELDS),
            Scalar("used_capacity", "vehicle_capacity"),
            ("cvrp_step", ("demand", "used_capacity", "vehicle_capacity", "visited", "current_node", "action_mask", "done")),
            ("locs", "demand"), features=(("demand", False, 1),), length_reward=True, unfold=True),
    EnvSpec("op", _lib.ENV_OP, True, lambda n: n + 2,
            _fields("B1", ("locs", "inst", "f32", "locs", "N2"), ("max_length", "inst", "f32", "max_length", "N"),
                    ("tour_length", "traj", "f32", "used_capacity", "B"), _I, _VISITED),
            Scalar("tour_length", "max_length", base_col0=True),
            ("op_step", ("locs", "max_length", "tour_length", "visited", "current_node", "i", "action_mask", "done")),
            ("locs", "prize", "max_length"), features=(("prize", True, 1),)),
    EnvSpec("pctsp", _lib.ENV_PCTSP, True, lambda n: n,
            _fields("B", ("real_prize", "inst", "f32", "demand", "N"), ("cur_total_prize", "traj", "f32", "used_capacity", "B"),
                    ("prize_required", "traj", "f32", "vehicle_capacity", "B"), _I, _VISITED),
            Scalar("cur_total_prize", "prize_required", clamp=True),
            ("pctsp_step", ("real_prize", "cur_total_prize", "visited", "current_node", "i", "action_mask", "done")),
            ("locs", "real_prize", "expected_prize", "penalty"), features=(("expected_prize", False, 1), ("penalty", True, 1))),
    EnvSpec("pdp", _lib.ENV_PDP, True, lambda n: n,
            _fields("B1", ("available", "traj", "u8", "visited", "BN"), ("to_deliver", "traj", "u8", "to_deliver", "BN"),
                    ("i", "traj", "i64", "step_i", "B1")),
            None, ("pdp_step", ("available", "to_deliver", "current_node", "i", "action_mask", "done")),
            ("locs",), init="pairs", length_reward=True, depot_flag="force_start_at_depot"),
    EnvSpec("cvrptw", _lib.ENV_CVRPTW, True, lambda n: 2 * n,
            _fields("B1", *_CVRP_FIELDS, ("locs", "inst", "f32", "locs", "N2"),
                    ("time_windows", "inst", "f32", "time_windows", "N2"), ("durations", "inst", "f32", "durations", "N"),
                    ("current_time", "traj", "f32", "current_time", "B1")),
            Scalar("used_capacity", "vehicle_capacity", clock="current_time"),
            ("cvrptw_step", ("demand", "locs", "time_windows", "durations", "used_capacity", "vehicle_capacity", "current_time",
                             "visited", "current_node", "action_mask", "done")),
            ("locs", "demand", "time_windows", "durations"),
            features=(("demand", False, 1), ("time_windows", True, 2), ("durations", True, 1)), length_reward=True),
    EnvSpec("sdvrp", _lib.ENV_SDVRP, True, lambda n: 6 * n,
            _fields("B1", ("demand_with_depot", "traj", "f32", "demand_state", "BN"),
                    ("used_capacity", "traj", "f32", "used_capacity", "B1"),
                    ("vehicle_capacity", "traj", "f32", "vehicle_capacity", "B1")),
            Scalar("used_capacity", "vehicle_capacity"),
            ("sdvrp_step", ("demand_with_depot", "used_capacity", "vehicle_capacity", "current_node", "action_mask", "done")),
            ("locs", "demand"), features=(("demand", False, 1),), length_reward=True, replay=False,
            dynamic=Dynamic("demand_with_depot", "projection", "dyn_vectors"),
            no_teacher="the dynamic embedding (remaining demand in keys and values) is not in the backward kernels"),
    EnvSpec("mtsp", _lib.ENV_MTSP, True, lambda n: 2 * n,
            tuple(Field(*f) for f in (
                ("action_mask", "traj", "u8", "action_mask", "BN"), ("current_node", "traj", "i64", "current_node", "B"),
                ("done", "traj", "u8", "done", "B1"),
                ("locs", "inst", "f32", "locs", "N2"), ("num_agents", "inst", "i64", "num_agents", ""),
                ("agent_idx", "traj", "i64", "step_i", "B"), ("current_length", "traj", "f32", "used_capacity", "B"),
                ("max_subtour_length", "traj", "f32", "current_time", "B"))),
            None,
            ("mtsp_step", ("locs", "num_agents", "agent_idx", "current_length", "max_subtour_length", "current_node",
                           "action_mask", "done")),
            ("locs", "num_agents"),
            feats=Features(("remaining_agents", "current_length", "max_subtour_length", "depot_distance"), "proj_dynamic_feats"),
            state_reward=True, replay=False,
            no_teacher="the four-scalar context (proj_dynamic_feats) and the min-max state are not in the backward kernels"),
)}


def spec(env_name: str) -> EnvSpec:
    return SPECS[canonical_env(env_name)]


def rem_base(sp: EnvSpec, state: dict, b: int):
    if sp.scalar is None:
        return None
    base = state[sp.scalar.base]
    if sp.scalar.base_col0:
        base = base[:, 0]
        base = (base if base.shape[0] == b else base.repeat(b // base.shape[0])).contiguous()
    return base


def customer_features(sp: EnvSpec, td, dtype=torch.float32) -> list:
    cols = [(td[key][:, 1:] if drop_depot else td[key]).to(dtype) for key, drop_depot, _ in sp.features]
    return [c if c.dim() == 3 else c[..., None] for c in cols]
```

### rl4co_amd/graph.py

```python
from __future__ import annotations

import torch

from .envspec import spec
from .tensordict import TensorDict


class GraphedRollout:
    def __init__(self, policy, env, example, decode_type: str = "greedy", warmup: int = 2, **forward_kwargs):
        if not example["locs"].is_cuda:
            raise RuntimeError("GraphedRollout needs CUDA tensors (HIP graph capture)")
        name = getattr(policy, "env_name", None)
        if name is not None and spec(name).state_reward:
            raise NotImplementedError(f"{name}: captured-graph rollouts are not served (the padding step of the finished rows "
                                      "follows the rollout's read-back)")
        self.policy, self.env = policy, env
        self.decode_type = decode_type
        self.kw = dict(forward_kwargs)
        self.batch = example.batch_size[0]
        dev = example["locs"].device
        self.static_in = TensorDict({k: v.clone() for k, v in example.items() if torch.is_tensor(v)}, batch_size=[self.batch])
        self.seed_dev = torch.zeros(1, dtype=torch.int64, device=dev)
        self._calls = 0
        side = torch.cuda.Stream(device=dev)
        side.wait_stream(torch.cuda.current_stream())
        with torch.cuda.stream(side), torch.inference_mode():
            for _ in range(max(1, warmup)):
                self._enqueue()()
        torch.cuda.current_stream().wait_stream(side)
        torch.cuda.synchronize(dev)
        pe = getattr(policy, "_packed", None)
        self._fused = pe is not None and bool(pe.t) and pe.version == pe._current_version()
        self._captured: dict = {}
        self._packed_version = None
        if self._fused:
            self._captured = dict(pe.t)
            self._packed_version = pe.version
            self._act_dtype = pe.act_dtype
        self.graph = torch.cuda.CUDAGraph()
        with torch.inference_mode(), torch.cuda.graph(self.graph):
            self._finish = self._enqueue()
        if self._fused:
            assert all(pe.t[k] is v for k, v in self._captured.items()), "the capture re-packed the encoder weights"

    def _enqueue(self):
        td = self.env.reset(self.static_in)
        return self.policy(td, self.env, phase="test", decode_type=self.decode_type, philox_seed_dev=self.seed_dev,
                           _defer_finish=True, **self.kw)

    def _sync_packed_weights(self) -> None:
        pe = self.policy._packed
        if pe.act_dtype != self._act_dtype:
            pe.refresh(act_dtype=self._act_dtype)
        ver = pe._current_version()
        if ver == self._packed_version:
            if any(pe.t.get(k) is not v for k, v in self._captured.items()):
                pe.t = dict(self._captured)
            return
        fresh = pe.refresh(act_dtype=self._act_dtype)
        for k, held in self._captured.items():
            new = fresh.get(k)
            if torch.is_tensor(held):
                if not torch.is_tensor(new) or new.shape != held.shape or new.dtype != held.dtype:
                    raise RuntimeError(f"packed encoder entry {k!r} changed layout: capture a new GraphedRollout")
                if new.data_ptr() != held.data_ptr():
                    held.copy_(new)
            elif new is not None:
                raise RuntimeError(f"packed encoder entry {k!r} appeared after the capture: capture a new GraphedRollout")
        pe.t = dict(self._captured)
        self._packed_version = ver

    def enqueue(self, batch, call_index: int | None = None) -> None:
        if batch.batch_size[0] != self.batch:
            raise ValueError(f"captured for {self.batch} instances, got {batch.batch_size[0]}")
        with torch.inference_mode():
            for k, v in self.static_in.items():
                src = batch[k]
                if src.data_ptr() != v.data_ptr():
                    v.copy_(src, non_blocking=True)
            if self._fused:
                self._sync_packed_weights()
            self._calls += 1
            index = self._calls if call_index is None else int(call_index)
            self.seed_dev.fill_(index * 0x9E3779B97F4A7C15 % (1 << 62))
            self.graph.replay()

    def finish(self) -> dict:
        with torch.inference_mode():
            return self._finish()

    def __call__(self, batch) -> dict:
        self.enqueue(batch)
        return self.finish()


def _tensors_of(obj):
    if torch.is_tensor(obj):
        if obj.is_cuda:
            yield obj
    elif isinstance(obj, dict) or hasattr(obj, "items"):
        for _, v in obj.items():
            yield from _tensors_of(v)
    elif isinstance(obj, (list, tuple)):
        for v in obj:
            yield from _tensors_of(v)


class PipelinedRollout:

    def __init__(self, policy, env, example, decode_type: str = "greedy", depth: int = 2, **forward_kwargs):
        dev = example["locs"].device
        self.depth = int(depth)
        self.streams = [torch.cuda.Stream(device=dev) for _ in range(self.depth)]
        self.slots = []
        for s in self.streams:
            s.wait_stream(torch.cuda.current_stream())
            with torch.cuda.stream(s):
                self.slots.append(GraphedRollout(policy, env, example, decode_type=decode_type, **forward_kwargs))
        torch.cuda.synchronize(dev)
        self.policy = policy
        self._pending = [False] * self.depth
        self._next = 0
        self._submitted = 0
        self._weights = self._weights_version()

    def _weights_version(self):
        pe = getattr(self.policy, "_packed", None)
        return pe._current_version() if (pe is not None and self.slots[0]._fused) else None
# ... 46 lines not shown
```

### rl4co_amd/kernels.py

```python
from __future__ import annotations

import ctypes as C

import torch
from torch import Tensor

from . import _lib
from .cache import FoldedCache
from .envspec import SPECS, EnvSpec, spec

MODE_IDS = {"greedy": _lib.DECODE_GREEDY, "sampling": _lib.DECODE_SAMPLE, "evaluate": _lib.DECODE_EVALUATE}
ENV_IDS = {name: sp.env_id for name, sp in SPECS.items()}
VARIANT_IDS = {"auto": _lib.VARIANT_AUTO, "stream": _lib.VARIANT_STREAM, "lds": _lib.VARIANT_LDS, "wide": _lib.VARIANT_WIDE, "ms": _lib.VARIANT_MS}


def decode_row_groups(num_nodes: int, cache_dtype: torch.dtype, max_steps: int, variant: str = "auto",
                      num_trajectories: int = 1 << 20, num_instances: int | None = None) -> int:
    dt = _lib.dtype_id(cache_dtype)
    return _lib.decode_row_groups(num_nodes, dt, max_steps, VARIANT_IDS[variant], num_trajectories, num_instances)


def decode_variant(num_nodes: int, cache_dtype: torch.dtype, max_steps: int, num_trajectories: int,
                   num_instances: int | None = None, env_name: str = "tsp") -> int:
    a = _lib.AmDecodeArgs()
    a.env = spec(env_name).env_id
    a.N, a.max_steps, a.B = int(num_nodes), int(max_steps), int(num_trajectories)
    a.B_inst = int(num_trajectories if num_instances is None else num_instances)
    a.cache_dtype = _lib.dtype_id(cache_dtype)
    return _lib.lib().rl4co_am_decode_variant(C.byref(a))


def _ptr(t: Tensor | None) -> int | None:
    return None if t is None else t.data_ptr()


def _stream() -> int:
    return torch.cuda.current_stream().cuda_stream


def _dev(t: Tensor, dtype: torch.dtype | None = None, name: str = "tensor") -> Tensor:
    if not t.is_cuda:
        raise _lib.Rl4coLibraryError(
            f"{name} lives on {t.device}; the rl4co_amd kernels only run on the MI355X (no CPU fallback)"
        )
    if dtype is not None and t.dtype != dtype:
        raise TypeError(f"{name} must be {dtype}, got {t.dtype}")
    if not t.is_contiguous():
        raise ValueError(f"{name} must be contiguous")
    return t


def _ctx_table(a, t: Tensor, plane_dtype: torch.dtype, name: str) -> Tensor:
    if not t.is_cuda:
        raise _lib.Rl4coLibraryError(f"{name} lives on {t.device}; the rl4co_amd kernels only run on the MI355X (no CPU fallback)")
    if t.dtype == torch.float32:
        return _dev(t, torch.float32, name)
    if t.dtype != plane_dtype or t.dim() != 3 or t.stride(2) != 1:
        raise TypeError(f"{name} must be fp32, or [B,N,128] in the planes' dtype {plane_dtype} with unit channel stride")
    dt, rs, bs = _lib.dtype_id(t.dtype), t.stride(1), t.stride(0)
    if a.ctx_dtype not in (0, dt) or (a.ctx_row_stride not in (0, rs)) or (a.ctx_batch_stride not in (0, bs)):
        raise ValueError("ctx_first and ctx_cur must share dtype and strides")
    a.ctx_dtype, a.ctx_row_stride, a.ctx_batch_stride = dt, rs, bs
    return t


def _u8(t: Tensor, name: str) -> Tensor:
    _dev(t, None, name)
    if t.dtype == torch.bool:
        return t.view(torch.uint8)
    if t.dtype != torch.uint8:
        raise TypeError(f"{name} must be bool or uint8, got {t.dtype}")
    return t


def _check_rows(b: int, **tensors) -> None:
    for name, t in tensors.items():
        if t is not None and t.shape[0] != b:
            raise ValueError(f"{name} has {t.shape[0]} rows, action_mask has {b}")


_SLOT_DTYPES = {"i64": torch.int64, "f32": torch.float32}


def bind_env_state(a, sp: EnvSpec, state: dict, b: int, n: int) -> int:
    replay = isinstance(a, _lib.EnvReplayArgs)
# ... 107 lines not shown
    st = _lib.lib().rl4co_cvrp_step(
        _ptr(None if action is None else _dev(action, torch.int64, "action")),
        _ptr(_dev(demand, torch.float32, "demand")), _ptr(_dev(used_capacity, torch.float32, "used_capacity")),
        _ptr(_dev(vehicle_capacity, torch.float32, "vehicle_capacity")), _ptr(_u8(visited, "visited")),
        _ptr(_dev(current_node, torch.int64, "current_node")), _ptr(mask),
        _ptr(None if done is None else _u8(done, "done")), b, b_inst, n, _ptr(err), _stream(),
    )
    _lib.check(st, "rl4co_cvrp_step")


def sdvrp_step(action: Tensor | None, demand_with_depot: Tensor, used_capacity: Tensor, vehicle_capacity: Tensor,
               current_node: Tensor, action_mask: Tensor, done: Tensor | None, err: Tensor | None = None) -> None:
    mask = _u8(action_mask, "action_mask")
    b, n = mask.shape
    _check_rows(b, action=action, demand_with_depot=demand_with_depot, used_capacity=used_capacity,
                vehicle_capacity=vehicle_capacity, current_node=current_node, done=done)
    if tuple(demand_with_depot.shape) != (b, n):
        raise ValueError(f"demand_with_depot must be [{b}, {n}], got {tuple(demand_with_depot.shape)}")
    st = _lib.lib().rl4co_sdvrp_step(
        _ptr(None if action is None else _dev(action, torch.int64, "action")),
        _ptr(_dev(demand_with_depot, torch.float32, "demand_with_depot")), _ptr(_dev(used_capacity, torch.float32, "used_capacity")),
        _ptr(_dev(vehicle_capacity, torch.float32, "vehicle_capacity")), _ptr(_dev(current_node, torch.int64, "current_node")),
        _ptr(mask), _ptr(None if done is None else _u8(done, "done")), b, n, _ptr(err), _stream())
    _lib.check(st, "rl4co_sdvrp_step")


def mtsp_step(action: Tensor, locs: Tensor, num_agents: Tensor, agent_idx: Tensor, current_length: Tensor,
              max_subtour_length: Tensor, current_node: Tensor, action_mask: Tensor, done: Tensor,
              err: Tensor | None = None) -> None:
    mask = _u8(action_mask, "action_mask")
    b, n = mask.shape
    _check_rows(b, action=action, agent_idx=agent_idx, current_length=current_length, max_subtour_length=max_subtour_length,
                current_node=current_node, done=done)
    b_inst = locs.shape[0]
    if tuple(locs.shape) != (b_inst, n, 2) or tuple(num_agents.shape) != (b_inst,) or b % b_inst:
        raise ValueError(f"locs must be [B_inst, {n}, 2] and num_agents [B_inst] with {b} % B_inst == 0, got "
                         f"{tuple(locs.shape)} and {tuple(num_agents.shape)}")
    st = _lib.lib().rl4co_mtsp_step(
        _ptr(_dev(action, torch.int64, "action")), _ptr(_dev(locs, torch.float32, "locs")),
        _ptr(_dev(num_agents, torch.int64, "num_agents")), _ptr(_dev(agent_idx, torch.int64, "agent_idx")),
        _ptr(_dev(current_length, torch.float32, "current_length")),
        _ptr(_dev(max_subtour_length, torch.float32, "max_subtour_length")),
        _ptr(_dev(current_node, torch.int64, "current_node")), _ptr(mask), _ptr(_u8(done, "done")), b, b_inst, n, _ptr(err),
        _stream())
    _lib.check(st, "rl4co_mtsp_step")


def select_start_nodes(batch: int, num_starts: int, num_loc: int, has_depot: bool, device) -> Tensor:
    out = torch.empty((batch * num_starts,), dtype=torch.int64, device=device)
    if not out.is_cuda:
        raise _lib.Rl4coLibraryError("select_start_nodes needs a CUDA device")
    st = _lib.lib().rl4co_select_start_nodes(_ptr(out), batch, num_starts, num_loc, int(has_depot), _stream())
    _lib.check(st, "rl4co_select_start_nodes")
    return out


def am_decode(
    cache: FoldedCache,
    state: dict,
    *,
    mode: str,
    max_steps: int,
    actions: Tensor,
    logps: Tensor,
    err: Tensor,
    t0: int = 0,
    tanh_clipping: float = 10.0,
    temperature: float = 1.0,
    mask_inner: bool = True,
    mask_logits: bool = True,
    exp_noise: Tensor | None = None,
    philox_seed: int = 0,
    philox_offset: int = 0,
    philox_seed_dev: Tensor | None = None,
    forced_actions: Tensor | None = None,
    all_logps: Tensor | None = None,
    entropy: Tensor | None = None,
    n_steps: Tensor | None = None,
    steps_summary: Tensor | None = None,
    variant: str = "auto",
    top_k: int = 0,
    top_p: float = 0.0,
    kept_bits: Tensor | None = None,
) -> None:
    sp = spec(cache.env_name)
    a = _lib.AmDecodeArgs()
    b, n = state["action_mask"].shape
    assert n == cache.num_nodes, (n, cache.num_nodes)
    a.env = sp.env_id
    a.B, a.B_inst, a.N = b, cache.num_instances, n
    a.mode = MODE_IDS[mode]
    a.max_steps = int(max_steps)
    a.variant = VARIANT_IDS[variant]
    a.mask_inner, a.mask_logits = int(mask_inner), int(mask_logits)
    a.tanh_clipping, a.temperature = float(tanh_clipping), float(temperature)
    kvl = cache.kvl
    if not kvl.is_cuda:
        raise _lib.Rl4coLibraryError(f"cache.kvl lives on {kvl.device}; the rl4co_amd kernels only run on the MI355X (no CPU fallback)")
    if not (kvl.dim() == 4 and kvl.stride(3) == 1):
        raise ValueError("cache.kvl must be [3, B, N, 128] with unit stride along the channels")
    a.cache_dtype = _lib.dtype_id(kvl.dtype)
    a.glimpse_key, a.glimpse_val, a.logit_key = (cache.plane(i).data_ptr() for i in range(3))
    a.kvl_row_stride, a.kvl_batch_stride = cache.row_stride, cache.batch_stride
    if cache.unfold:
        a.unfold, a.ctx_width = 1, cache.w_ctx_t.shape[0]
        a.node_embed = _ptr(_dev(cache.node_embed, torch.float32, "node_embed"))
        a.w_ctx_t = _ptr(_dev(cache.w_ctx_t, torch.float32, "w_ctx_t"))
        a.w_out_t = _ptr(_dev(cache.w_out_t, torch.float32, "w_out_t"))
        a.w_placeholder = _ptr(None if cache.w_placeholder is None else _dev(cache.w_placeholder, torch.float32, "w_placeholder"))
    else:
        a.ctx_cur = _ptr(_ctx_table(a, cache.ctx_cur, kvl.dtype, "ctx_cur"))
    a.q_bias = _ptr(None if cache.q_bias is None else _dev(cache.q_bias, torch.float32, "q_bias"))
    if not cache.unfold:
        if sp.ctx_first:
            a.ctx_first = _ptr(_ctx_table(a, cache.ctx_first, kvl.dtype, "ctx_first"))
            a.q_step0 = _ptr(_dev(cache.q_step0, torch.float32, "q_step0"))
        if sp.scalar is not None:
            a.w_cap = _ptr(_dev(cache.w_cap, torch.float32, "w_cap"))
            if sp.scalar.clock:
                a.w_time = _ptr(_dev(cache.w_time, torch.float32, "w_time"))
    if cache.unfold and not sp.unfold:
        raise ValueError("the unfolded parity mode serves tsp / cvrp")
    if sp.dynamic is not None:
        dyn = _dev(cache.dyn, torch.float32, "dyn")
        if tuple(dyn.shape) != (3, 128):
            raise ValueError(f"cache.dyn must be [3, 128], got {tuple(dyn.shape)}")
        setattr(a, sp.dynamic.slot, dyn.data_ptr())
    if sp.feats is not None:
        feat = _dev(cache.feat, torch.float32, "feat")
        if tuple(feat.shape) != (len(sp.feats.names), 128):
            raise ValueError(f"cache.feat must be [{len(sp.feats.names)}, 128], got {tuple(feat.shape)}")
        if b != cache.num_instances:
            raise ValueError(f"{sp.name} runs one trajectory per instance (no multistart rows): {b} trajectories over "
                             f"{cache.num_instances} instances")
        a.mtsp_ctx = feat.data_ptr()
    b_inst = bind_env_state(a, sp, state, b, n)
    assert b_inst == cache.num_instances or not sp.keys("inst"), "instance data rows must match cache instances"
    if exp_noise is not None:
        _dev(exp_noise, torch.float32, "exp_noise")
        assert exp_noise.numel() >= max_steps * b * n, "exp_noise must hold [max_steps,B,N] draws"
        a.exp_noise = _ptr(exp_noise)
    a.philox_seed, a.philox_offset = int(philox_seed), int(philox_offset)
    if philox_seed_dev is not None:
        a.philox_seed_dev = _ptr(_dev(philox_seed_dev, torch.int64, "philox_seed_dev"))
    if forced_actions is not None:
        _dev(forced_actions, torch.int64, "forced_actions")
        assert forced_actions.shape == actions.shape
        a.forced_actions = _ptr(forced_actions)
    _dev(actions, torch.int64, "actions"), _dev(logps, torch.float32, "logps")
    assert actions.shape == logps.shape and actions.shape[0] == b
    a.t0, a.out_stride = int(t0), actions.shape[1]
    a.actions, a.logps = _ptr(actions), _ptr(logps)
    a.all_logps = _ptr(None if all_logps is None else _dev(all_logps, torch.float32, "all_logps"))
    a.entropy = _ptr(None if entropy is None else _dev(entropy, torch.float32, "entropy"))
    a.n_steps = _ptr(None if n_steps is None else _dev(n_steps, torch.int32, "n_steps"))
    if steps_summary is not None:
        _dev(steps_summary, torch.int32, "steps_summary")
        if steps_summary.numel() < 4 or steps_summary.data_ptr() % 8:
            raise ValueError("steps_summary must be 4 int32 words on an 8-byte boundary (rl4co_am_decode_args.steps_summary)")
    a.steps_summary = _ptr(steps_summary)
    a.err = _ptr(_dev(err, torch.int32, "err"))
    a.top_k, a.top_p = decoding_filter(top_k, top_p, n)
    if kept_bits is not None:
        _dev(kept_bits, torch.int32, "kept_bits")
        words = 4 * ((n + 127) // 128)
        if tuple(kept_bits.shape) != (b, actions.shape[1], words) or not kept_bits.is_contiguous():
            raise ValueError(f"kept_bits must be a contiguous [{b}, {actions.shape[1]}, {words}] int32 tensor")
        a.kept_bits, a.kept_words = _ptr(kept_bits), words
    st = _lib.lib().rl4co_am_decode(C.byref(a), _stream())
    _lib.check(st, "rl4co_am_decode")


def decoding_filter(top_k, top_p, n: int) -> tuple[int, float]:
    k = int(top_k or 0)
    p = float(top_p or 0.0)
    assert p <= 1.0, "top-p should be in (0, 1]."
    k = min(k, n) if k > 0 else 0
    if k >= n:
        k = 0
    if not (0.0 < p < 1.0):
        p = 0.0
    return k, p


def op_max_length(locs: Tensor, max_length: Tensor) -> Tensor:
    b, n, _ = locs.shape
    locs = _dev(locs, torch.float32, "locs")
    ml = _dev(max_length.reshape(-1).contiguous(), torch.float32, "max_length")
    out = torch.empty((b, n), dtype=torch.float32, device=locs.device)
    st = _lib.lib().rl4co_op_max_length(_ptr(locs), _ptr(ml), b, n, _ptr(out), _stream())
    _lib.check(st, "rl4co_op_max_length")
    return out


def op_step(action: Tensor | None, locs: Tensor, max_length: Tensor, tour_length: Tensor, visited: Tensor,
            current_node: Tensor, step_i: Tensor, action_mask: Tensor, done: Tensor, err: Tensor | None = None) -> None:
    b, n = action_mask.shape
    _check_rows(b, action=action, tour_length=tour_length, visited=visited, current_node=current_node, i=step_i, done=done)
    st = _lib.lib().rl4co_op_step(
        _ptr(None if action is None else _dev(action, torch.int64, "action")), _ptr(_dev(locs, torch.float32, "locs")),
        _ptr(_dev(max_length, torch.float32, "max_length")), _ptr(_dev(tour_length, torch.float32, "tour_length")),
        _ptr(_u8(visited, "visited")), _ptr(_dev(current_node, torch.int64, "current_node")),
        _ptr(_dev(step_i, torch.int64, "i")), _ptr(_u8(action_mask, "action_mask")), _ptr(_u8(done, "done")),
        b, locs.shape[0], n, _ptr(err), _stream())
    _lib.check(st, "rl4co_op_step")


def cvrptw_step(action: Tensor | None, demand: Tensor, locs: Tensor, time_windows: Tensor, durations: Tensor,
                used_capacity: Tensor, vehicle_capacity: Tensor, current_time: Tensor, visited: Tensor, current_node: Tensor,
                action_mask: Tensor, done: Tensor | None, err: Tensor | None = None) -> None:
    b, n = action_mask.shape
    _check_rows(b, action=action, used_capacity=used_capacity, vehicle_capacity=vehicle_capacity, current_time=current_time,
                visited=visited, current_node=current_node, done=done)
    st = _lib.lib().rl4co_cvrptw_step(
        _ptr(None if action is None else _dev(action, torch.int64, "action")), _ptr(_dev(demand, torch.float32, "demand")),
        _ptr(_dev(locs, torch.float32, "locs")), _ptr(_dev(time_windows, torch.float32, "time_windows")),
        _ptr(_dev(durations, torch.float32, "durations")), _ptr(_dev(used_capacity, torch.float32, "used_capacity")),
        _ptr(_dev(vehicle_capacity, torch.float32, "vehicle_capacity")), _ptr(_dev(current_time, torch.float32, "current_time")),
        _ptr(_u8(visited, "visited")), _ptr(_dev(current_node, torch.int64, "current_node")),
        _ptr(_u8(action_mask, "action_mask")), _ptr(None if done is None else _u8(done, "done")),
        b, demand.shape[0], n, _ptr(err), _stream())
    _lib.check(st, "rl4co_cvrptw_step")


def cvrptw_check_solution(actions: Tensor, locs: Tensor, time_windows: Tensor, durations: Tensor, err: Tensor) -> None:
    b, t = actions.shape
    st = _lib.lib().rl4co_cvrptw_check_solution(
        _ptr(_dev(actions, torch.int64, "actions")), _ptr(_dev(locs, torch.float32, "locs")),
        _ptr(_dev(time_windows, torch.float32, "time_windows")), _ptr(_dev(durations, torch.float32, "durations")),
        b, locs.shape[0], locs.shape[1], t, _ptr(_dev(err, torch.int32, "err")), _stream())
    _lib.check(st, "rl4co_cvrptw_check_solution")


def pdp_step(action: Tensor | None, available: Tensor, to_deliver: Tensor, current_node: Tensor, step_i: Tensor,
             action_mask: Tensor, done: Tensor, err: Tensor | None = None) -> None:
    b, n = action_mask.shape
    _check_rows(b, action=action, available=available, to_deliver=to_deliver, current_node=current_node, i=step_i, done=done)
    st = _lib.lib().rl4co_pdp_step(
        _ptr(None if action is None else _dev(action, torch.int64, "action")), _ptr(_u8(available, "available")),
        _ptr(_u8(to_deliver, "to_deliver")), _ptr(_dev(current_node, torch.int64, "current_node")),
        _ptr(_dev(step_i, torch.int64, "i")), _ptr(_u8(action_mask, "action_mask")), _ptr(_u8(done, "done")),
        b, n, _ptr(err), _stream())
    _lib.check(st, "rl4co_pdp_step")


def env_replay(env_name: str, state: dict, actions: Tensor, rem_base: Tensor | None, err: Tensor | None = None,
               mask_bits: bool = False) -> dict:
    sp = spec(env_name)
    if not sp.replay:
        served = sorted(name for name, s in SPECS.items() if s.replay)
        raise NotImplementedError(f"the one-launch replay (rl4co_env_replay) serves {served}, not {sp.name}: use "
                                  "env_replay_stepwise")
    b, n = state["action_mask"].shape
# ... 203 lines not shown
```

### rl4co_amd/policy.py

```python
from __future__ import annotations

import math

import torch
import torch.nn as nn
import torch.nn.functional as F
from torch import Tensor

from . import kernels as K
from .cache import FoldedCache, build_folded_cache, canonical_env
from .envs import RL4COEnvBase, get_env
from .envspec import customer_features, rem_base, spec
from .tensordict import TensorDict



class _Skip(nn.Module):

    def __init__(self, module: nn.Module):
        super().__init__()
        self.module = module

    def forward(self, x):
        return x + self.module(x)


class _Norm(nn.Module):

    def __init__(self, embed_dim: int, normalization: str):
        super().__init__()
        self.kind = normalization
        if normalization == "batch":
            self.normalizer = nn.BatchNorm1d(embed_dim, affine=True)
        elif normalization == "instance":
            self.normalizer = nn.InstanceNorm1d(embed_dim, affine=True)
        elif normalization == "layer":
            self.normalizer = "layer"
        else:
            raise ValueError(f"unknown normalization {normalization!r}")

    def forward(self, x: Tensor) -> Tensor:
        if self.kind == "batch":
            b, n, d = x.shape
            return self.normalizer(x.reshape(b * n, d)).view(b, n, d)
        if self.kind == "instance":
            if self.training and x.is_cuda and torch.is_grad_enabled():
                n = self.normalizer
                mean = x.mean(dim=1, keepdim=True)
                var = x.var(dim=1, unbiased=False, keepdim=True)
                return (x - mean) * torch.rsqrt(var + n.eps) * n.weight + n.bias
            return self.normalizer(x.transpose(1, 2)).transpose(1, 2)
        mean = x.mean((1, 2), keepdim=True)
        var = x.var((1, 2), keepdim=True)
        return (x - mean) / torch.sqrt(var + 1e-5)


class _SelfAttention(nn.Module):

    def __init__(self, embed_dim: int, num_heads: int):
        super().__init__()
        self.num_heads = num_heads
        self.Wqkv = nn.Linear(embed_dim, 3 * embed_dim, bias=True)
        self.out_proj = nn.Linear(embed_dim, embed_dim, bias=True)

    def forward(self, x: Tensor, fused: bool = False) -> Tensor:
        b, n, d = x.shape
        if fused:
            from . import train_ops

            qkv = train_ops.linear(x, self.Wqkv.weight, self.Wqkv.bias)
            if self.num_heads == 8 and train_ops.attention_usable(qkv):
                return train_ops.linear(train_ops.attention(qkv), self.out_proj.weight, self.out_proj.bias)
            qkv = qkv.view(b, n, 3, self.num_heads, d // self.num_heads)
        else:
            qkv = self.Wqkv(x).view(b, n, 3, self.num_heads, d // self.num_heads)
        q, k, v = qkv.permute(2, 0, 3, 1, 4).unbind(0)
        out = F.scaled_dot_product_attention(q, k, v).transpose(1, 2).reshape(b, n, d)
        if fused:
            return train_ops.linear(out, self.out_proj.weight, self.out_proj.bias)
        return self.out_proj(out)


class _FeedForward(nn.Module):

    def __init__(self, embed_dim: int, hidden: int):
        super().__init__()
        dims = [embed_dim] + ([hidden] if hidden > 0 else []) + [embed_dim]
        self.lins = nn.ModuleList(nn.Linear(i, o) for i, o in zip(dims[:-1], dims[1:]))

    def forward(self, x: Tensor, fused: bool = False) -> Tensor:
        if fused and len(self.lins) == 2:
            from . import train_ops

            return train_ops.mlp(x, self.lins[0].weight, self.lins[0].bias, self.lins[1].weight, self.lins[1].bias)
# ... 129 lines not shown
            width = 2 * embed_dim
        else:
            width = embed_dim + (0 if sp.scalar is None else 2 if sp.scalar.clock else 1)
        self.project_context = nn.Linear(width, embed_dim, bias=False)
        if sp.ctx_first:
            self.W_placeholder = nn.Parameter(torch.Tensor(2 * embed_dim).uniform_(-1, 1))
        if sp.feats is not None:
            setattr(self, sp.feats.weight, nn.Linear(len(sp.feats.names), embed_dim, bias=False))


class _DynamicEmbedding(nn.Module):

    def __init__(self, env_name, embed_dim):
        super().__init__()
        sp = spec(env_name)
        if sp.dynamic is not None:
            setattr(self, sp.dynamic.weight, nn.Linear(1, 3 * embed_dim, bias=False))


class AttentionModelEncoder(nn.Module):

    def __init__(self, embed_dim=128, env_name="tsp", num_heads=8, num_layers=3, normalization="batch",
                 feedforward_hidden=512):
        super().__init__()
        self.env_name = env_name = canonical_env(env_name)
        self.init_embedding = _InitEmbedding(env_name, embed_dim)
        self.net = _GraphAttentionNetwork(num_heads, embed_dim, num_layers, normalization, feedforward_hidden)

    def forward(self, td):
        init_h = self.init_embedding(td)
        return self.net(init_h), init_h


class _Pointer(nn.Module):

    def __init__(self, embed_dim, out_bias=False):
        super().__init__()
        self.project_out = nn.Linear(embed_dim, embed_dim, bias=out_bias)


class AttentionModelDecoder(nn.Module):

    def __init__(self, embed_dim=128, num_heads=8, env_name="tsp", mask_inner=True,
                 use_graph_context=True, check_nan=True):
        super().__init__()
        self.env_name = env_name = canonical_env(env_name)
        self.embed_dim = embed_dim
        self.num_heads = num_heads
        self.mask_inner = mask_inner
        self.check_nan = check_nan
        self.context_embedding = _ContextEmbedding(env_name, embed_dim)
        self.dynamic_embedding = _DynamicEmbedding(env_name, embed_dim)
        self.pointer = _Pointer(embed_dim)
        self.project_node_embeddings = nn.Linear(embed_dim, 3 * embed_dim, bias=False)
        self.project_fixed_context = nn.Linear(embed_dim, embed_dim, bias=False)
        self.use_graph_context = use_graph_context

    def precompute_cache(self, h: Tensor, cache_dtype: torch.dtype,
                         gemm_dtype: torch.dtype = torch.float32, fold: bool = True) -> FoldedCache:
        return build_folded_cache(
            self.env_name, h,
            w_node=self.project_node_embeddings.weight,
            w_fixed=self.project_fixed_context.weight if self.use_graph_context else None,
            cache_dtype=cache_dtype,
            gemm_dtype=gemm_dtype,
            fold=fold,
            **self.constant_weights(),
        )

    def constant_weights(self) -> dict:
        sp = spec(self.env_name)
        ctx = self.context_embedding
        return dict(
            w_ctx=ctx.project_context.weight,
            w_out=self.pointer.project_out.weight,
            w_placeholder=getattr(ctx, "W_placeholder", None),
            w_dyn=getattr(self.dynamic_embedding, sp.dynamic.weight).weight if sp.dynamic is not None else None,
            w_feat=getattr(ctx, sp.feats.weight).weight if sp.feats is not None else None,
        )



_KNOWN_DECODE_TYPES = ("greedy", "sampling", "multistart_greedy", "multistart_sampling", "evaluate")


def _cuda_tensors(objs):
    for o in objs:
        if torch.is_tensor(o):
            if o.is_cuda:
                yield o
        elif isinstance(o, FoldedCache):
            for k in FoldedCache.TENSOR_FIELDS:
                t = getattr(o, k)
                if t is not None and t.is_cuda:
                    yield t


def _parse_decode_type(decode_type: str):
    if decode_type not in _KNOWN_DECODE_TYPES:
        if decode_type == "beam_search":
            raise NotImplementedError("beam_search is outside the accelerated hot path (SURVEY.md §2 row 2)")
        decode_type = "sampling"
    multistart = "multistart" in decode_type
    mode = "greedy" if "greedy" in decode_type else ("evaluate" if decode_type == "evaluate" else "sampling")
    return mode, multistart


class AttentionModelPolicy(nn.Module):

    def __init__(self, env_name: str = "tsp", embed_dim: int = 128, num_encoder_layers: int = 3,
                 num_heads: int = 8, normalization: str = "batch", feedforward_hidden: int = 512,
                 use_graph_context: bool = True, mask_inner: bool = True, check_nan: bool = True,
                 temperature: float = 1.0, tanh_clipping: float = 10.0, mask_logits: bool = True,
                 train_decode_type: str = "sampling", val_decode_type: str = "greedy",
                 test_decode_type: str = "greedy", cache_dtype: torch.dtype | None = None,
                 encoder_autocast: torch.dtype | None = None, fused_encoder: bool = True,
                 fused_backward: bool = True, teacher_variant: str = "auto", fold: bool = True,
                 train_half_as_bf16: bool = False, **unused_kwargs):
        super().__init__()
        if isinstance(env_name, RL4COEnvBase):
            env_name = env_name.name
        if embed_dim != 128 or num_heads != 8:
            raise ValueError("the fused decode kernel is specialised for embed_dim=128, num_heads=8")
        self.env_name = env_name = canonical_env(env_name)
        self.encoder = AttentionModelEncoder(embed_dim, env_name, num_heads, num_encoder_layers,
                                             normalization, feedforward_hidden)
        self.decoder = AttentionModelDecoder(embed_dim, num_heads, env_name, mask_inner,
                                             use_graph_context, check_nan)
        self.temperature = temperature
        self.tanh_clipping = tanh_clipping
        self.mask_logits = mask_logits
        self.train_decode_type = train_decode_type
        self.val_decode_type = val_decode_type
        self.test_decode_type = test_decode_type
        self.cache_dtype = cache_dtype
        self.encoder_autocast = encoder_autocast
        self.fused_encoder = fused_encoder
        self.fused_backward = fused_backward
        self.teacher_variant = teacher_variant
        self.fold = fold
        self.train_half_as_bf16 = train_half_as_bf16
        self._packed = None
        self._ambient_autocast = None
        self._bwd_err = None
        self.async_train_status = not __import__("os").environ.get("RL4CO_SYNC_TRAIN_STATUS")
        self._pending_status = None
        self._status_host: list = []
        self._philox_calls = 0
        self.last_instance_steps = 0
        self.last_rows_read = 0
        self.encode_events: list | None = None
        self.decode_events: list | None = None

    def _packed_encoder(self):
        if self._packed is None:
            from .encoder import PackedEncoder

            self._packed = PackedEncoder(self)
        return self._packed

    def _encode_tokens_bf16(self, td):
        from . import train_ops as T

        enc = self.encoder
        bf = self._encoder_regime()
        assert bf in (torch.bfloat16, torch.float16)
        x = [T.init_embed(f, lin, dtype=bf) for f, lin in enc.init_embedding.features(td)]
        init_h = x = x[0] if len(x) == 1 else torch.cat(x, -2)
        b, n, d = x.shape
        for layer in enc.net.layers:
            attn, norm1, ffn, norm2 = layer[0].module, layer[1].normalizer, layer[2].module, layer[3].normalizer
            x2 = x.reshape(b * n, d)
            qkv = T._gemm(x2, attn.Wqkv.weight.to(bf).contiguous(), attn.Wqkv.bias.float().contiguous())
            o = T.attention_flash(qkv.view(b, n, 3 * d)).view(b * n, d)
            s_ = T._gemm(o, attn.out_proj.weight.to(bf).contiguous(), attn.out_proj.bias.float().contiguous())
            x2 = T.skip_batch_norm_eval(x2, s_, norm1)
            h = T._gemm(x2, ffn.lins[0].weight.to(bf).contiguous(), ffn.lins[0].bias.float().contiguous(), relu=True)
            s_ = T._gemm(h, ffn.lins[1].weight.to(bf).contiguous(), ffn.lins[1].bias.float().contiguous())
            x = T.skip_batch_norm_eval(x2, s_, norm2).view(b, n, d)
        return x, init_h

    def _bf16_regime(self) -> bool:
        return self._encoder_regime() == torch.bfloat16

    def _plane_dtype(self, training: bool) -> torch.dtype:
        if self.cache_dtype is not None:
            return self.cache_dtype
        regime = self._encoder_regime()
        if regime == torch.bfloat16:
            return torch.bfloat16
        if regime == torch.float16:
            return torch.bfloat16 if training else torch.float16
        return torch.float32

    def _encoder_regime(self):
        return self.encoder_autocast if self.encoder_autocast is not None else self._ambient_autocast

    def _token_encoder_usable(self, td) -> bool:
        layer0 = self.encoder.net.layers[0]
        return (td["locs"].is_cuda and self._encoder_regime() in (torch.bfloat16, torch.float16) and layer0[1].kind == "batch"
                and not self.training and len(layer0[2].module.lins) == 2 and layer0[2].module.lins[0].out_features % 128 == 0)

    def _encode(self, td):
        regime = self._encoder_regime()
        if regime == torch.float16 and self.train_half_as_bf16 and torch.is_grad_enabled():
            regime = torch.bfloat16
        if regime is not None and td["locs"].is_cuda:
            with torch.autocast("cuda", dtype=regime):
                return self.encoder(td)
        return self.encoder(td)

    @staticmethod
    def _max_horizon(env_name: str, n: int) -> int:
        return spec(env_name).horizon(n)

    def _initial_state(self, td, num_starts: int):
        s = max(num_starts, 1)
        st = {}
        for f in spec(self.env_name).fields:
            x = td[f.key]
            if f.kind == "inst":
                st[f.key] = (x.float() if f.dtype == "f32" else x).contiguous()
                continue
            x = x if f.shape == "BN" else x.reshape(-1)
            st[f.key] = x.clone(memory_format=torch.contiguous_format) if s == 1 else x.unsqueeze(0).expand(s, *x.shape).reshape(s * x.shape[0], *x.shape[1:]).contiguous()
        return st

    def forward(self, td: TensorDict, *args, **kwargs) -> dict:
        on_cuda = td["locs"].is_cuda if "locs" in td.keys() else torch.cuda.is_available()
        if on_cuda and torch.is_autocast_enabled():
            self._ambient_autocast = torch.get_autocast_dtype("cuda")
            try:
                with torch.autocast("cuda", enabled=False):
                    return self._forward(td, *args, **kwargs)
            finally:
                self._ambient_autocast = None
        return self._forward(td, *args, **kwargs)

    def _encode_for_rollout(self, td: TensorDict, grad_path: bool, cache_dtype, return_hidden: bool, return_init_embeds: bool):
        init_embeds = None
        regime16 = self._encoder_regime() if self._encoder_regime() in (torch.bfloat16, torch.float16) else None
        ie_ok = not return_init_embeds or td["locs"].shape[0] <= 65535
        use_fused = (self.fused_encoder and self.fold and regime16 is not None and not grad_path
                     and cache_dtype in (torch.float32, regime16) and ie_ok
                     and self._packed_encoder().supported(td))
        use_fused_f32 = (self.fused_encoder and self._encoder_regime() is None and not grad_path and td["locs"].is_cuda
                         and (self.fold or spec(self.env_name).unfold) and ie_ok
                         and self._packed_encoder().supported(td, torch.float32))
        if use_fused_f32:
            use_fused, regime16 = True, torch.float32
        if use_fused:
            if self.encode_events is not None:
                ev0, ev1 = torch.cuda.Event(enable_timing=True), torch.cuda.Event(enable_timing=True)
                ev0.record()
            init_embeds = (torch.empty((*td["locs"].shape[:2], 128), dtype=regime16, device=td["locs"].device)
                           if return_init_embeds else None)
            cache, hidden = self._packed_encoder().encode(td, cache_dtype, want_hidden=return_hidden, act_dtype=regime16,
                                                          fold=self.fold, init_embeds_out=init_embeds)
            if self.encode_events is not None:
                ev1.record()
                self.encode_events.append((ev0, ev1))
        else:
            cache = None
            if not grad_path and self.fused_encoder and self._token_encoder_usable(td):
                if self.encode_events is not None:
                    ev0, ev1 = torch.cuda.Event(enable_timing=True), torch.cuda.Event(enable_timing=True)
                    ev0.record()
                hidden, init_embeds = self._encode_tokens_bf16(td)
                if self.encode_events is not None:
                    ev1.record()
                    self.encode_events.append((ev0, ev1))
            else:
                if (td["locs"].is_cuda and not grad_path and self._encoder_regime() is not None
                        and self.fused_encoder and self.fold):
                    from . import _lib as _l

                    n_nodes = td["action_mask"].shape[-1]
                    _l.warn_fallback(f"infer-encoder/{self._encoder_regime()}/{n_nodes > 128}/{self.fused_encoder}/{self.fold}",
                                     f"inference encoder for {n_nodes} nodes under autocast({self._encoder_regime()}) runs on torch: "
                                     "the fused MFMA encoder (up to 128 nodes) and the token-tile kernels (beyond) serve bf16 / fp16 with the "
                                     "folded cache and planes in fp32 or the activations' type")
                hidden, init_embeds = self._encode(td)
        return cache, hidden, init_embeds

    def _parse_decoding(self, td: TensorDict, env, phase: str, actions, decoding_kwargs: dict):
        from types import SimpleNamespace

        decode_type = decoding_kwargs.pop("decode_type", None)
        if actions is not None:
            decode_type = "evaluate"
        elif decode_type is None:
            decode_type = getattr(self, f"{phase}_decode_type")
        mode, multistart = _parse_decode_type(decode_type)
        temperature = decoding_kwargs.pop("temperature", self.temperature)
        tanh_clipping = decoding_kwargs.pop("tanh_clipping", self.tanh_clipping)
        mask_logits = decoding_kwargs.pop("mask_logits", self.mask_logits)
        return_all_logp = bool(decoding_kwargs.pop("return_all_logp", False))
        store_all_logp = bool(decoding_kwargs.pop("store_all_logp", False)) or return_all_logp
        select_best = decoding_kwargs.pop("select_best", False)
        num_starts = decoding_kwargs.pop("num_starts", None)
        num_samples = decoding_kwargs.pop("num_samples", None)
        exp_noise = decoding_kwargs.pop("exp_noise", None)
        seed = decoding_kwargs.pop("seed", None)
        multisample = bool(decoding_kwargs.pop("multisample", False))
        select_start_nodes_fn = decoding_kwargs.pop("select_start_nodes_fn", None)
        top_k = int(decoding_kwargs.pop("top_k", 0) or 0)
        top_p = float(decoding_kwargs.pop("top_p", 0.0) or 0.0)
        if top_p > 0:
            assert top_p <= 1.0, "top-p should be in (0, 1]."
        if decoding_kwargs.pop("softmax_temp", None) is not None:
            raise NotImplementedError("softmax_temp is not supported; use temperature")
        assert not (multistart and multisample), "Using both multistart and multisample is not supported"
        if num_samples and num_starts:
            assert not (num_samples > 1 and num_starts > 1), f"num_samples={num_samples} and num_starts={num_starts} are both > 1"
        if num_samples is not None:
            multisample = num_samples > 1
        if num_starts is not None:
            multistart = num_starts > 1
        if multistart or multisample:
            n_rep = num_starts if multistart else num_samples
            if n_rep is None:
                n_rep = env.get_num_starts(td)
        else:
            n_rep = 0

        return SimpleNamespace(mode=mode, multistart=multistart, n_rep=n_rep, temperature=temperature, tanh_clipping=tanh_clipping,
                               mask_logits=mask_logits, return_all_logp=return_all_logp, store_all_logp=store_all_logp,
                               select_best=select_best, exp_noise=exp_noise, seed=seed, select_start_nodes_fn=select_start_nodes_fn,
                               top_k=top_k, top_p=top_p)

    def _forward(self, td: TensorDict, env: str | RL4COEnvBase | None = None, phase: str = "train",
                 calc_reward: bool = True, return_actions: bool = True, return_entropy: bool = False,
                 return_hidden: bool = False, return_init_embeds: bool = False,
                 return_sum_log_likelihood: bool = True, actions: Tensor | None = None,
                 max_steps: int = 1_000_000, **decoding_kwargs) -> dict:
        grad_path = torch.is_grad_enabled() and any(p.requires_grad for p in self.parameters())
        cache_dtype = self._plane_dtype(grad_path)
        es = getattr(self, "encoder_stream", None)
        if es is not None and not grad_path and td["locs"].is_cuda:
            cur = torch.cuda.current_stream()
            es.wait_stream(cur)
            with torch.cuda.stream(es):
                cache, hidden, init_embeds = self._encode_for_rollout(td, grad_path, cache_dtype, return_hidden, return_init_embeds)
            cur.wait_stream(es)
            for t in _cuda_tensors((cache, hidden, init_embeds)):
                t.record_stream(cur)
        else:
            cache, hidden, init_embeds = self._encode_for_rollout(td, grad_path, cache_dtype, return_hidden, return_init_embeds)
        if isinstance(env, str) or env is None:
            env = get_env(self.env_name if env is None else env)
        opt = self._parse_decoding(td, env, phase, actions, decoding_kwargs)
        mode, multistart, n_rep = opt.mode, opt.multistart, opt.n_rep
        temperature, tanh_clipping, mask_logits = opt.temperature, opt.tanh_clipping, opt.mask_logits
        return_all_logp, store_all_logp, select_best = opt.return_all_logp, opt.store_all_logp or return_entropy, opt.select_best
        exp_noise, seed, select_start_nodes_fn = opt.exp_noise, opt.seed, opt.select_start_nodes_fn

        device = td["action_mask"].device
        b_inst, n = td["action_mask"].shape[0], td["action_mask"].shape[-1]
        b = b_inst * max(n_rep, 1)
        sp = spec(self.env_name)
        if sp.state_reward:
            if n_rep > 0:
                raise NotImplementedError(f"{sp.name}: multistart / multisample rollouts are not served (the multistart variant "
                                          "does not carry the four-scalar context; one trajectory per instance)")
            if decoding_kwargs.get("_defer_finish"):
                raise NotImplementedError(f"{sp.name}: captured-graph rollouts are not served (the padding step of the finished "
                                          "rows follows the rollout's read-back)")
        top_k, top_p = K.decoding_filter(opt.top_k, opt.top_p, n)
        filtered = bool(top_k or top_p)
        if filtered and not td["action_mask"].is_cuda:
            raise NotImplementedError("top-k / top-p sampling runs inside the MI355X decode kernels only")
        cache_g = None
        if cache is None and grad_path and self.fused_backward and hidden.is_cuda and self.fold and not filtered:
            from . import teacher

            if teacher.supports(self.env_name, cache_dtype, n) and not return_entropy:
                half = (torch.bfloat16, torch.float16)
                fused_planes = hidden.dtype in half and cache_dtype in half and self.teacher_variant != "replay"
                h_fold = hidden.to(cache_dtype) if (fused_planes and hidden.dtype != cache_dtype) else hidden
                cache_g = teacher.build_cache_autograd(self.env_name, h_fold, self.decoder, fused_planes=fused_planes)
                cache = teacher.detached_cache(self.env_name, cache_g, cache_dtype)
        if cache is None:
            with torch.no_grad():
                regime = self._encoder_regime()
                cache = self.decoder.precompute_cache(hidden.detach(), cache_dtype,
                                                      torch.bfloat16 if (regime == torch.bfloat16 and cache_dtype != torch.float16)
                                                      else torch.float32, fold=self.fold)
        self.last_ctx_elem_bytes = cache.ctx_cur.element_size() if cache.ctx_cur is not None else 4
        state = self._initial_state(td, n_rep)
        horizon = min(self._max_horizon(self.env_name, n), max_steps)
        if sp.depot_flag is not None and not getattr(env, sp.depot_flag, False):
            horizon = min(horizon, n - 1)
        status = torch.zeros(6, dtype=torch.int32, device=device)
        err = status[:1]

        t0 = 1 if (multistart and n_rep >= 1) else 0
        if mode == "evaluate":
            given = actions.contiguous()
            tmax = t0 + given.shape[1]
            forced = torch.zeros((b, tmax), dtype=torch.int64, device=device)
            forced[:, t0:] = given
        else:
            forced = None
            tmax = horizon
        out_actions = torch.zeros((b, tmax), dtype=torch.int64, device=device)
        logps = torch.zeros((b, tmax), dtype=torch.float32, device=device)
        all_logps = torch.zeros((b, tmax, n), dtype=torch.float32, device=device) if store_all_logp else None
        kept_bits = (torch.full((b, tmax, 4 * ((n + 127) // 128)), -1, dtype=torch.int32, device=device)
                     if (grad_path and filtered) else None)

        if t0 == 1:
            if select_start_nodes_fn is not None:
                first = select_start_nodes_fn(td, env, n_rep).to(device=device, dtype=torch.int64).contiguous()
            else:
                first = env.select_start_nodes(td, num_starts=n_rep)
            out_actions[:, 0] = first
            self._env_step_state(state, first, err)

        if mode == "sampling" and exp_noise is None:
            self._philox_calls += 1
            philox_seed = int(seed) if seed is not None else int(torch.randint(0, 2**62, (1,)).item())
        else:
            philox_seed = 0
        seed_dev = decoding_kwargs.pop("philox_seed_dev", None)
        if self.decode_events is not None:
            ev0, ev1 = torch.cuda.Event(enable_timing=True), torch.cuda.Event(enable_timing=True)
            ev0.record()
        K.am_decode(
            cache, state, mode=mode, max_steps=tmax - t0, t0=t0, actions=out_actions, logps=logps, err=err,
            tanh_clipping=tanh_clipping, temperature=temperature, mask_inner=self.decoder.mask_inner,
            mask_logits=mask_logits, exp_noise=exp_noise, philox_seed=philox_seed, philox_seed_dev=seed_dev,
            forced_actions=forced, all_logps=all_logps, steps_summary=status[2:6],
            variant=getattr(self, "decode_variant", "auto"),
            **(dict(top_k=top_k, top_p=top_p, kept_bits=kept_bits) if filtered else {}),
        )
        if self.decode_events is not None:
            ev1.record()
            self.decode_events.append((ev0, ev1))
        native_env = isinstance(env, RL4COEnvBase)
        checked = bool(native_env and calc_reward and env.check_solution and not (n_rep > 0 and select_best))
        if checked:
            env.check_solution_validity(td, out_actions, err=err)
        td_early = reward_early = None
        if (native_env and sp.length_reward and calc_reward and mode != "evaluate"
                and (checked or not env.check_solution) and not (n_rep > 0 and select_best)
                and env.accepts_reward_horizon()):
            td_early = self._final_td(td, state, n_rep)
            reward_early = env.get_reward(td_early, out_actions, check_solution=False, horizon=(status[2:3], t0))
        if self._bwd_err is not None and self._bwd_err.device == device:
            status[:1].bitwise_or_(self._bwd_err)
            self._bwd_err.zero_()
        defer = bool(decoding_kwargs.pop("_defer_finish", False))
        launched = (out_actions, logps, all_logps, td_early, reward_early)

        from types import SimpleNamespace

        r = SimpleNamespace(
            launched=launched, status=status, t0=t0, td=td, env=env, state=state, n_rep=n_rep, b_inst=b_inst, n=n,
            device=device, grad_path=grad_path, cache_g=cache_g, cache=cache, cache_dtype=cache_dtype, hidden=hidden,
            init_embeds=init_embeds, mask_logits=mask_logits, tanh_clipping=tanh_clipping, temperature=temperature,
            return_entropy=return_entropy, select_best=select_best, calc_reward=calc_reward, checked=checked,
            return_sum_log_likelihood=return_sum_log_likelihood, return_actions=return_actions,
            return_all_logp=return_all_logp, return_hidden=return_hidden, return_init_embeds=return_init_embeds,
            kept_bits=kept_bits,
        )
        if defer:
            return lambda: self._finish_rollout(r)
        return self._finish_rollout(r)

    def _finish_rollout(self, r) -> dict:
        from . import _lib as _l

        out_actions, logps, all_logps, td_early, reward_early = r.launched
        status, t0, td, env, state, n_rep, device = r.status, r.t0, r.td, r.env, r.state, r.n_rep, r.device
        grad_path, cache_g, hidden, return_entropy = r.grad_path, r.cache_g, r.hidden, r.return_entropy
        sp = spec(self.env_name)
        self._drain_status()
        if (self.async_train_status and grad_path and cache_g is not None and sp.fixed_horizon and status.is_cuda
                and not r.select_best):
            if len(self._status_host) < 2:
                self._status_host.append(torch.empty(6, dtype=torch.int32, pin_memory=True))
            host = self._status_host.pop(0)
            self._status_host.append(host)
            host.copy_(status, non_blocking=True)
            ev = torch.cuda.Event()
            ev.record()
            self._pending_status = (host, ev)
            t_used = out_actions.shape[1]
            self.last_instance_steps = out_actions.shape[0] * (t_used - t0)
            self.last_rows_read = 0
        else:
            err_bits, _, horizon_used, streamed, rows_lo, rows_hi = status.tolist()
            rows_read = (rows_hi << 32) | (rows_lo & 0xFFFFFFFF)
            t_used = t0 + int(horizon_used)
            self.last_instance_steps = int(streamed)
            self.last_rows_read = int(rows_read)
            _l.raise_for_error_bits(int(err_bits))
        out_actions = out_actions[:, :t_used].contiguous()
        logps = logps[:, :t_used]
        if all_logps is not None:
            all_logps = all_logps[:, :t_used]

        if sp.state_reward:
            self._mtsp_pad_finished(state, out_actions)
        td_out = td_early if td_early is not None else self._final_td(td, state, n_rep)
        td_out.set("action", out_actions[:, -1])
        if sp.state_reward:
            td_out.set("i", torch.full((out_actions.shape[0],), out_actions.shape[1], dtype=torch.int64, device=device))
            td_out.set("first_node", out_actions[:, 0].clone())

        full_logp = None
        if grad_path and cache_g is not None:
            from . import teacher

            if self._bwd_err is None or self._bwd_err.device != device:
                self._bwd_err = torch.zeros(1, dtype=torch.int32, device=device)
            meta = dict(t0=t0, mask_inner=self.decoder.mask_inner, mask_logits=r.mask_logits, err_sink=self._bwd_err,
                        tanh_clipping=r.tanh_clipping, temperature=r.temperature, teacher_variant=self.teacher_variant)
            meta.update((k, td[k]) for k in sp.teacher_keys)
            step_logps = teacher.teacher_forced_logps(self.env_name, cache_g, r.cache, out_actions, logps, meta)
        elif grad_path:
            kept = r.kept_bits[:, :t_used].contiguous() if r.kept_bits is not None else None
            if kept is not None and hidden.is_cuda and self.fused_backward:
                _l.warn_fallback(f"teacher-topkp/{self.env_name}",
                                 f"teacher-forced backward for {self.env_name}: the top-k / top-p filter is not in the backward "
                                 "kernels — dense re-evaluation of all steps with autograd, the rollout's kept sets as the logit mask")
            elif hidden.is_cuda and self.fused_backward and not return_entropy:
                t_max = __import__("rl4co_amd.teacher", fromlist=["max_nodes"]).max_nodes()
                why = (sp.no_teacher if sp.no_teacher is not None else
                       "fold=False keeps the reference's per-step association, which the backward kernels do not implement" if not self.fold else
                       f"{r.n} nodes are beyond the kernels' limit ({t_max})" if r.n > t_max else
# ... 235 lines not shown
```

Before: 139.7 million instance·step/s.

## Fuse solution check, tour reward and output padding into greedy decode kernel

```diff
diff --git a/include/rl4co_amd.h b/include/rl4co_amd.h
--- a/include/rl4co_amd.h
+++ b/include/rl4co_amd.h
@@ -7,7 +7,7 @@
 extern "C" {
 #endif
 
-#define RL4CO_ABI_VERSION 15
+#define RL4CO_ABI_VERSION 16
 
 #define RL4CO_OK 0
 #define RL4CO_ERR_ARG 1
@@ -216,6 +216,12 @@
   float* logps;
   float* all_logps;
   float* entropy;
+  int32_t fresh;
+  int32_t pad_outputs;
+  int32_t fused_check;
+  int32_t reserved2;
+  float* fused_reward;
+  const float* fused_locs;
   int32_t* n_steps;
   int32_t* steps_summary;
   int32_t* err;
diff --git a/rl4co_amd/_lib.py b/rl4co_amd/_lib.py
--- a/rl4co_amd/_lib.py
+++ b/rl4co_amd/_lib.py
@@ -7,7 +7,7 @@
 from . import build as _build
 
 RL4CO_OK = 0
-ABI_VERSION = 15
+ABI_VERSION = 16
 ENV_TSP, ENV_CVRP, ENV_OP, ENV_PCTSP, ENV_PDP, ENV_CVRPTW, ENV_SDVRP, ENV_MTSP = 0, 1, 2, 3, 4, 5, 6, 7
 DECODE_GREEDY, DECODE_SAMPLE, DECODE_EVALUATE = 0, 1, 2
 DT_F32, DT_BF16, DT_F16 = 0, 1, 2
@@ -72,6 +72,8 @@
         ("forced_actions", _vp),
         ("t0", _i32), ("out_stride", _i32),
         ("actions", _vp), ("logps", _vp), ("all_logps", _vp), ("entropy", _vp),
+        ("fresh", _i32), ("pad_outputs", _i32), ("fused_check", _i32), ("reserved2", _i32),
+        ("fused_reward", _vp), ("fused_locs", _vp),
         ("n_steps", _vp), ("steps_summary", _vp), ("err", _vp),
         ("mtsp_ctx", _vp), ("num_agents", _vp),
         ("ctx_dtype", _i32), ("reserved0", _i32), ("ctx_row_stride", _i64), ("ctx_batch_stride", _i64),
diff --git a/rl4co_amd/build.py b/rl4co_amd/build.py
--- a/rl4co_amd/build.py
+++ b/rl4co_amd/build.py
@@ -18,7 +18,7 @@
 SOURCES = ["api.hip", "entry16.hip", "env_step.hip", "tour_length.hip", "am_decode.hip", "am_decode_ms.hip", "am_encoder.hip", "am_encoder_f32.hip", "am_tokens_f32.hip", "am_teacher.hip", "am_teacher_mma.hip", "am_train_ops.hip", "am_train_attn.hip", "am_attn_flash.hip", "am_cross_attn.hip", "am_logit_logp.hip", "augment.hip",
            "am_train_ops_f16.hip", "am_train_attn_f16.hip", "am_attn_flash_f16.hip", "am_cross_attn_f16.hip",
            "am_decode_ms_f16.hip", "am_teacher_mma_f16.hip"]
-HEADERS = ["common.h", "rl4co_math.h", "topkp.h", "elem16.h", "enc_f32.h"]
+HEADERS = ["common.h", "rl4co_math.h", "topkp.h", "elem16.h", "enc_f32.h", "check_solution.h", "tour_sum.h"]
 INCLUDED = {name: [name.replace("_f16.hip", ".hip")] for name in SOURCES if name.endswith("_f16.hip")}
 COMPILE_FLAGS = [
     "--offload-arch=gfx950",
diff --git a/rl4co_amd/csrc/am_decode.hip b/rl4co_amd/csrc/am_decode.hip
--- a/rl4co_amd/csrc/am_decode.hip
+++ b/rl4co_amd/csrc/am_decode.hip
@@ -1,8 +1,10 @@
 #include <hip/hip_runtime.h>
 
+#include "check_solution.h"
 #include "common.h"
 #include "rl4co_math.h"
 #include "topkp.h"
+#include "tour_sum.h"
 
 namespace {
 
@@ -428,8 +430,14 @@
   const CtxTables<C> ctx(a, cb, N, e0);
   const float* hrow = UNFOLD ? a.node_embed + (int64_t)cb * N * kD + e0 : nullptr;
 
+  constexpr bool kFusable = !UNFOLD && (ENV == RL4CO_ENV_TSP || ENV == RL4CO_ENV_CVRP);
+  const bool fresh = kFusable && a.fresh != 0;
   uint8_t* gmask = a.action_mask + (int64_t)r * N;
-  for (int j = lane; j < Np; j += 64) mk[j] = (j < N) ? gmask[j] : (uint8_t)0;
+  if (!fresh) {
+    for (int j = lane; j < Np; j += 64) mk[j] = (j < N) ? gmask[j] : (uint8_t)0;
+  } else if (ENV == RL4CO_ENV_TSP) {
+    for (int j = lane; j < Np; j += 64) mk[j] = (j < N) ? (uint8_t)1 : (uint8_t)0;
+  }
   constexpr bool kScalarCtx = ENV == RL4CO_ENV_CVRP || ENV == RL4CO_ENV_OP || ENV == RL4CO_ENV_PCTSP || ENV == RL4CO_ENV_CVRPTW || kDyn || kMtsp;
   constexpr bool kCvrpLike = ENV == RL4CO_ENV_CVRP || ENV == RL4CO_ENV_CVRPTW;
   if (ENV == RL4CO_ENV_PDP) {
@@ -441,15 +449,19 @@
     for (int j = lane; j < Np; j += 64) dd[j] = (j < N) ? gd[j] : 0.0f;
   } else if (ENV != RL4CO_ENV_TSP && !kMtsp) {
     const uint8_t* gv = a.visited + (int64_t)r * N;
-    for (int j = lane; j < Np; j += 64) vis[j] = (j < N) ? gv[j] : (uint8_t)1;
+    if (fresh) {
+      for (int j = lane; j < Np; j += 64) vis[j] = (j < N) ? (uint8_t)0 : (uint8_t)1;
+    } else {
+      for (int j = lane; j < Np; j += 64) vis[j] = (j < N) ? gv[j] : (uint8_t)1;
+    }
   }
   TrajState st;
-  st.cur = (int)a.current_node[r];
-  st.first = (ENV == RL4CO_ENV_TSP) ? (int)a.first_node[r] : 0;
-  st.step_i = !(kCvrpLike || kDyn) ? a.step_i[r] : 0;
+  st.cur = fresh ? 0 : (int)a.current_node[r];
+  st.first = (ENV == RL4CO_ENV_TSP && !fresh) ? (int)a.first_node[r] : 0;
+  st.step_i = (!(kCvrpLike || kDyn) && !fresh) ? a.step_i[r] : 0;
   st.time = (ENV == RL4CO_ENV_CVRPTW || kMtsp) ? a.current_time[r] : 0.0f;
-  st.used = kScalarCtx ? a.used_capacity[r] : 0.0f;
-  st.done = a.done[r] != 0;
+  st.used = (kScalarCtx && !fresh) ? a.used_capacity[r] : 0.0f;
+  st.done = fresh ? false : a.done[r] != 0;
   st.errbits = 0;
   st.ent_acc = 0.0f;
   const float* oplocs = (ENV == RL4CO_ENV_OP || ENV == RL4CO_ENV_CVRPTW || kMtsp) ? a.locs + (int64_t)cb * N * 2 : nullptr;
@@ -462,6 +474,20 @@
   const float* dem = kCvrpLike                  ? a.demand + (int64_t)cb * (N - 1)
                      : (ENV == RL4CO_ENV_PCTSP) ? a.demand + (int64_t)cb * N
                                                 : nullptr;
+  if (ENV == RL4CO_ENV_CVRP && fresh) {
+    const float thr = cap + 1e-5f;
+    bool any_feasible = false;
+    for (int j = lane; j < Np; j += 64) {
+      bool masked = true;
+      if (j >= 1 && j < N) {
+        masked = dem[j - 1] + st.used > thr;
+        any_feasible |= !masked;
+      }
+      if (j >= 1) mk[j] = masked ? 0 : 1;
+    }
+    any_feasible = __any(any_feasible);
+    if (lane == 0) mk[0] = any_feasible ? 0 : 1;
+  }
   wave_lds_sync();
 
   const bool list_all = !(a.mask_inner && a.mask_logits);
@@ -758,6 +784,38 @@
     }
   }
   if (!single && !st.done && t >= a.max_steps) st.errbits |= RL4CO_EBIT_MAX_STEPS;
+
+  if constexpr (kFusable) {
+    const int T = a.out_stride;
+    int64_t* arow = a.actions + (int64_t)r * T;
+    if (a.pad_outputs) {
+      float* lrow = a.logps + (int64_t)r * T;
+      for (int c = a.t0 + t + lane; c < T; c += 64) {
+        arow[c] = 0;
+        lrow[c] = 0.0f;
+      }
+    }
+    if (a.fused_check || (ENV == RL4CO_ENV_TSP && a.fused_reward)) {
+      __builtin_amdgcn_fence(__ATOMIC_SEQ_CST, "agent");
+      if (a.fused_check) {
+        unsigned int* seen = reinterpret_cast<unsigned int*>(sc);
+        if constexpr (ENV == RL4CO_ENV_TSP) st.errbits |= rl4co::tsp_check_row(arow, N, T, seen, lane);
+        else st.errbits |= rl4co::cvrp_check_row(arow, dem, cap, N, T, seen, lane);
+      }
+      if constexpr (ENV == RL4CO_ENV_TSP) {
+        if (a.fused_reward) {
+          rl4co::TourView tv;
+          tv.locs = a.fused_locs + (int64_t)cb * N * 2;
+          tv.actions = arow;
+          tv.prepend = 0;
+          tv.n = T;
+          tv.values = nullptr;
+          const float len = rl4co::tour_row_sum(tv, T, lane & 7, lane & ~7, lane < 8);
+          if (lane == 0) a.fused_reward[r] = -len;
+        }
+      }
+    }
+  }
 
   for (int j = lane; j < N; j += 64) gmask[j] = mk[j];
   if (ENV == RL4CO_ENV_PDP) {
@@ -1398,6 +1456,12 @@
   RL4CO_REQUIRE(a.variant >= RL4CO_VARIANT_AUTO && a.variant <= RL4CO_VARIANT_MS);
   const int variant = resolve_variant(a);
   RL4CO_REQUIRE(variant >= 0);
+  RL4CO_REQUIRE((a.fresh | 1) == 1 && (a.pad_outputs | 1) == 1 && (a.fused_check | 1) == 1);
+  if (a.fresh || a.pad_outputs || a.fused_check || a.fused_reward) {
+    RL4CO_REQUIRE(variant == RL4CO_VARIANT_STREAM && !a.unfold && a.max_steps > 1);
+    RL4CO_REQUIRE(a.env == RL4CO_ENV_TSP || a.env == RL4CO_ENV_CVRP);
+    RL4CO_REQUIRE(a.fused_reward == nullptr || (a.env == RL4CO_ENV_TSP && a.fused_locs != nullptr));
+  }
   hipStream_t s = rl4co::as_stream(stream);
   if (a.unfold) {
     if (a.cache_dtype == RL4CO_DT_F32)
diff --git a/rl4co_amd/csrc/check_solution.h b/rl4co_amd/csrc/check_solution.h
--- /dev/null
+++ b/rl4co_amd/csrc/check_solution.h
@@ -0,0 +1,73 @@
+#pragma once
+
+#include <hip/hip_runtime.h>
+
+#include <stdint.h>
+
+#include "rl4co_amd.h"
+
+namespace rl4co {
+
+__device__ inline void check_lds_sync() {
+  __builtin_amdgcn_fence(__ATOMIC_RELEASE, "workgroup");
+  __builtin_amdgcn_wave_barrier();
+  __builtin_amdgcn_fence(__ATOMIC_ACQUIRE, "workgroup");
+}
+
+__device__ inline uint32_t tsp_check_row(const int64_t* row, int N, int T, unsigned int* seen, int lane) {
+  const int words = (N + 31) / 32;
+  for (int w = lane; w < words; w += 64) seen[w] = 0;
+  check_lds_sync();
+  bool bad = (T != N);
+  for (int t = lane; t < T; t += 64) {
+    const int64_t a = row[t];
+    if (a < 0 || a >= N) {
+      bad = true;
+    } else {
+      const unsigned int bit = 1u << (a & 31);
+      const unsigned int old = atomicOr(&seen[a >> 5], bit);
+      if (old & bit) bad = true;
+    }
+  }
+  return __any(bad) ? (uint32_t)RL4CO_EBIT_INVALID_TOUR : 0u;
+}
+
+__device__ inline uint32_t cvrp_check_row(const int64_t* row, const float* dem, float cap, int N, int T,
+                                          unsigned int* seen, int lane) {
+  const int words = (N + 31) / 32;
+  for (int w = lane; w < words; w += 64) seen[w] = 0;
+  check_lds_sync();
+  bool bad = false;
+  int customers = 0;
+  for (int t = lane; t < T; t += 64) {
+    const int64_t a = row[t];
+    if (a < 0 || a >= N) {
+      bad = true;
+    } else if (a > 0) {
+      const unsigned int bit = 1u << (a & 31);
+      const unsigned int old = atomicOr(&seen[a >> 5], bit);
+      if (old & bit) bad = true;
+      ++customers;
+    }
+  }
+  for (int s = 1; s < 64; s <<= 1) customers += __shfl_xor(customers, s, 64);
+  if (customers != N - 1) bad = true;
+  uint32_t bits = __any(bad) ? (uint32_t)RL4CO_EBIT_INVALID_TOUR : 0u;
+  if (lane == 0) {
+    const float thr = cap + 1e-5f;
+    float used = 0.0f;
+    bool over = false;
+    for (int t = 0; t < T; ++t) {
+      int64_t a = row[t];
+      if (a < 0 || a >= N) a = 0;
+      const float d = (a == 0) ? -cap : dem[a - 1];
+      used = used + d;
+      if (used < 0.0f) used = 0.0f;
+      if (!(used <= thr)) over = true;
+    }
+    if (over) bits |= (uint32_t)RL4CO_EBIT_CAPACITY;
+  }
+  return bits;
+}
+
+}
diff --git a/rl4co_amd/csrc/tour_length.hip b/rl4co_amd/csrc/tour_length.hip
--- a/rl4co_amd/csrc/tour_length.hip
+++ b/rl4co_amd/csrc/tour_length.hip
@@ -1,67 +1,12 @@
 #include <hip/hip_runtime.h>
 
+#include "check_solution.h"
 #include "common.h"
+#include "tour_sum.h"
 
 namespace {
 
-struct TourView {
-  const float* locs;
-  const int64_t* actions;
-  int prepend;
-  int n;
-  const float* values;
-  __device__ inline float2 point(int t) const {
-    int node;
-    if (prepend) node = (t == 0) ? 0 : (int)actions[t - 1];
-    else node = (int)actions[t];
-    return *reinterpret_cast<const float2*>(locs + 2 * (int64_t)node);
-  }
-  __device__ inline float seg(int t) const {
-    if (values) return values[actions[t]];
-    const float2 p0 = point(t);
-    const float2 p1 = point(t + 1 == n ? 0 : t + 1);
-    const float dx = p1.x - p0.x;
-    const float dy = p1.y - p0.y;
-    return sqrtf(fmaf(dy, dy, dx * dx));
-  }
-};
-
-__device__ float lane_row_sum(const TourView& tv, int lane8, int nvec) {
-  constexpr int kIlp = 4;
-  constexpr int kLevels = 4;
-  const int size = nvec / kIlp;
-  int ceil_log2 = 0;
-  while ((1LL << ceil_log2) < size) ++ceil_log2;
-  int level_power = ceil_log2 / kLevels;
-  if (level_power < 4) level_power = 4;
-  const int level_step = 1 << level_power;
-  const int level_mask = level_step - 1;
-  float acc[kLevels][kIlp];
-  for (int l = 0; l < kLevels; ++l)
-    for (int k = 0; k < kIlp; ++k) acc[l][k] = 0.0f;
-  int i = 0;
-  for (; i + level_step <= size;) {
-    for (int j = 0; j < level_step; ++j, ++i) {
-      for (int k = 0; k < kIlp; ++k) acc[0][k] = acc[0][k] + tv.seg(8 * (i * kIlp + k) + lane8);
-    }
-    for (int j = 1; j < kLevels; ++j) {
-      for (int k = 0; k < kIlp; ++k) {
-        acc[j][k] = acc[j][k] + acc[j - 1][k];
-        acc[j - 1][k] = 0.0f;
-      }
-      const int mask = level_mask << (j * level_power);
-      if ((i & mask) != 0) break;
-    }
-  }
-  for (; i < size; ++i) {
-    for (int k = 0; k < kIlp; ++k) acc[0][k] = acc[0][k] + tv.seg(8 * (i * kIlp + k) + lane8);
-  }
-  for (int j = 1; j < kLevels; ++j)
-    for (int k = 0; k < kIlp; ++k) acc[0][k] = acc[0][k] + acc[j][k];
-  for (int v = size * kIlp; v < nvec; ++v) acc[0][0] = acc[0][0] + tv.seg(8 * v + lane8);
-  for (int k = 1; k < kIlp; ++k) acc[0][0] = acc[0][0] + acc[0][k];
-  return acc[0][0];
-}
+using rl4co::TourView;
 
 __global__ void __launch_bounds__(256) tour_length_kernel(const float* __restrict__ locs,
                                                           const int64_t* __restrict__ actions,
@@ -81,31 +26,7 @@
   tv.locs = locs ? locs + (int64_t)(active ? b % B_locs : 0) * N * 2 : nullptr;
   tv.actions = actions + (int64_t)(active ? b : 0) * row_stride;
   tv.values = gather_values ? gather_values + (int64_t)(active ? b % B_locs : 0) * N : nullptr;
-  const int n = tv.n;
-  const int nvec = n / 8;
-  if (n < 8) {
-    if (active && lane8 == 0) {
-      float p[4] = {0.0f, 0.0f, 0.0f, 0.0f};
-      const int g = n / 4;
-      for (int i = 0; i < g; ++i)
-        for (int k = 0; k < 4; ++k) p[k] = p[k] + tv.seg(4 * i + k);
-      for (int k = 4 * g; k < n; ++k) p[0] = p[0] + tv.seg(k);
-      for (int k = 1; k < 4; ++k) p[0] = p[0] + p[k];
-      out[b] = negate ? -p[0] : p[0];
-    }
-    return;
-  }
-  float part = 0.0f;
-  if (active) part = lane_row_sum(tv, lane8, nvec);
-  float fin = 0.0f;
-  if (active && lane8 == 0) {
-    for (int k = nvec * 8; k < n; ++k) fin = fin + tv.seg(k);
-  }
-  const int base = (threadIdx.x & 63) & ~7;
-  for (int l = 0; l < 8; ++l) {
-    const float pl = __shfl(part, base + l, 64);
-    fin = fin + pl;
-  }
+  const float fin = rl4co::tour_row_sum(tv, tv.n, lane8, (threadIdx.x & 63) & ~7, active);
   if (active && lane8 == 0) out[b] = negate ? -fin : fin;
 }
 
@@ -129,23 +50,9 @@
 __global__ void __launch_bounds__(64) tsp_check_kernel(const int64_t* __restrict__ actions, int B,
                                                        int N, int T, int32_t* err) {
   extern __shared__ unsigned int seen[];
-  const int b = blockIdx.x;
   const int lane = threadIdx.x;
-  const int words = (N + 31) / 32;
-  for (int w = lane; w < words; w += 64) seen[w] = 0;
-  __syncthreads();
-  bool bad = (T != N);
-  for (int t = lane; t < T; t += 64) {
-    const int64_t a = actions[(int64_t)b * T + t];
-    if (a < 0 || a >= N) {
-      bad = true;
-    } else {
-      const unsigned int bit = 1u << (a & 31);
-      const unsigned int old = atomicOr(&seen[a >> 5], bit);
-      if (old & bit) bad = true;
-    }
-  }
-  if (__any(bad) && lane == 0) atomicOr(err, RL4CO_EBIT_INVALID_TOUR);
+  const uint32_t bits = rl4co::tsp_check_row(actions + (int64_t)blockIdx.x * T, N, T, seen, lane);
+  if (bits && lane == 0) atomicOr(err, (int)bits);
 }
 
 __global__ void __launch_bounds__(64) cvrp_check_kernel(const int64_t* __restrict__ actions,
@@ -155,41 +62,10 @@
   extern __shared__ unsigned int seen[];
   const int b = blockIdx.x;
   const int lane = threadIdx.x;
-  const int words = (N + 31) / 32;
-  for (int w = lane; w < words; w += 64) seen[w] = 0;
-  __syncthreads();
-  bool bad = false;
-  int customers = 0;
-  for (int t = lane; t < T; t += 64) {
-    const int64_t a = actions[(int64_t)b * T + t];
-    if (a < 0 || a >= N) {
-      bad = true;
-    } else if (a > 0) {
-      const unsigned int bit = 1u << (a & 31);
-      const unsigned int old = atomicOr(&seen[a >> 5], bit);
-      if (old & bit) bad = true;
-      ++customers;
-    }
-  }
-  for (int s = 1; s < 64; s <<= 1) customers += __shfl_xor(customers, s, 64);
-  if (customers != N - 1) bad = true;
-  if (__any(bad) && lane == 0) atomicOr(err, RL4CO_EBIT_INVALID_TOUR);
-  if (lane == 0) {
-    const int inst = b % B_inst;
-    const float cap = capacity[inst];
-    const float thr = cap + 1e-5f;
-    float used = 0.0f;
-    bool over = false;
-    for (int t = 0; t < T; ++t) {
-      int64_t a = actions[(int64_t)b * T + t];
-      if (a < 0 || a >= N) a = 0;
-      const float d = (a == 0) ? -cap : demand[(int64_t)inst * (N - 1) + (a - 1)];
-      used = used + d;
-      if (used < 0.0f) used = 0.0f;
-      if (!(used <= thr)) over = true;
-    }
-    if (over) atomicOr(err, RL4CO_EBIT_CAPACITY);
-  }
+  const int inst = b % B_inst;
+  const uint32_t bits = rl4co::cvrp_check_row(actions + (int64_t)b * T, demand + (int64_t)inst * (N - 1), capacity[inst], N, T,
+                                              seen, lane);
+  if (bits && lane == 0) atomicOr(err, (int)bits);
 }
 
 __global__ void select_start_nodes_kernel(int64_t* out, int B, int S, int num_loc, int has_depot) {
diff --git a/rl4co_amd/csrc/tour_sum.h b/rl4co_amd/csrc/tour_sum.h
--- /dev/null
+++ b/rl4co_amd/csrc/tour_sum.h
@@ -0,0 +1,96 @@
+#pragma once
+
+#include <hip/hip_runtime.h>
+
+#include <stdint.h>
+
+namespace rl4co {
+
+struct TourView {
+  const float* locs;
+  const int64_t* actions;
+  int prepend;
+  int n;
+  const float* values;
+  __device__ inline float2 point(int t) const {
+    int node;
+    if (prepend) node = (t == 0) ? 0 : (int)actions[t - 1];
+    else node = (int)actions[t];
+    return *reinterpret_cast<const float2*>(locs + 2 * (int64_t)node);
+  }
+  __device__ inline float seg(int t) const {
+    if (values) return values[actions[t]];
+    const float2 p0 = point(t);
+    const float2 p1 = point(t + 1 == n ? 0 : t + 1);
+    const float dx = p1.x - p0.x;
+    const float dy = p1.y - p0.y;
+    return sqrtf(fmaf(dy, dy, dx * dx));
+  }
+};
+
+template <class Segs>
+__device__ inline float lane_row_sum(const Segs& tv, int lane8, int nvec) {
+  constexpr int kIlp = 4;
+  constexpr int kLevels = 4;
+  const int size = nvec / kIlp;
+  int ceil_log2 = 0;
+  while ((1LL << ceil_log2) < size) ++ceil_log2;
+  int level_power = ceil_log2 / kLevels;
+  if (level_power < 4) level_power = 4;
+  const int level_step = 1 << level_power;
+  const int level_mask = level_step - 1;
+  float acc[kLevels][kIlp];
+  for (int l = 0; l < kLevels; ++l)
+    for (int k = 0; k < kIlp; ++k) acc[l][k] = 0.0f;
+  int i = 0;
+  for (; i + level_step <= size;) {
+    for (int j = 0; j < level_step; ++j, ++i) {
+      for (int k = 0; k < kIlp; ++k) acc[0][k] = acc[0][k] + tv.seg(8 * (i * kIlp + k) + lane8);
+    }
+    for (int j = 1; j < kLevels; ++j) {
+      for (int k = 0; k < kIlp; ++k) {
+        acc[j][k] = acc[j][k] + acc[j - 1][k];
+        acc[j - 1][k] = 0.0f;
+      }
+      const int mask = level_mask << (j * level_power);
+      if ((i & mask) != 0) break;
+    }
+  }
+  for (; i < size; ++i) {
+    for (int k = 0; k < kIlp; ++k) acc[0][k] = acc[0][k] + tv.seg(8 * (i * kIlp + k) + lane8);
+  }
+  for (int j = 1; j < kLevels; ++j)
+    for (int k = 0; k < kIlp; ++k) acc[0][k] = acc[0][k] + acc[j][k];
+  for (int v = size * kIlp; v < nvec; ++v) acc[0][0] = acc[0][0] + tv.seg(8 * v + lane8);
+  for (int k = 1; k < kIlp; ++k) acc[0][0] = acc[0][0] + acc[0][k];
+  return acc[0][0];
+}
+
+template <class Segs>
+__device__ inline float tour_row_sum(const Segs& tv, int n, int lane8, int base, bool active) {
+  const int nvec = n / 8;
+  if (n < 8) {
+    float p[4] = {0.0f, 0.0f, 0.0f, 0.0f};
+    if (active && lane8 == 0) {
+      const int g = n / 4;
+      for (int i = 0; i < g; ++i)
+        for (int k = 0; k < 4; ++k) p[k] = p[k] + tv.seg(4 * i + k);
+      for (int k = 4 * g; k < n; ++k) p[0] = p[0] + tv.seg(k);
+      for (int k = 1; k < 4; ++k) p[0] = p[0] + p[k];
+    }
+    return p[0];
+  }
+  float part = 0.0f;
+  if (active) part = lane_row_sum(tv, lane8, nvec);
+  float fin = 0.0f;
+  if (active && lane8 == 0) {
+    for (int k = nvec * 8; k < n; ++k) fin = fin + tv.seg(k);
+  }
+  for (int l = 0; l < 8; ++l) {
+    const float pl = __shfl(part, base + l, 64);
+    fin = fin + pl;
+  }
+  return fin;
+}
+
+}
diff --git a/rl4co_amd/envs.py b/rl4co_amd/envs.py
--- a/rl4co_amd/envs.py
+++ b/rl4co_amd/envs.py
@@ -199,7 +199,7 @@
         return TensorDict({"locs": locs[..., 1:, :], "depot": locs[..., 0, :]}, batch_size=batch_size)
 
 
-def _zero_state(device, **fields) -> dict:
+def _zero_state(device, fill: bool = True, **fields) -> dict:
     offs, total = {}, 0
     for name, (shape, dtype) in fields.items():
         nbytes = int(torch.tensor([], dtype=dtype).element_size())
@@ -207,7 +207,7 @@
             nbytes *= int(d)
         offs[name] = (total, nbytes)
         total += (nbytes + 15) // 16 * 16
-    buf = torch.zeros(max(total, 16), dtype=torch.uint8, device=device)
+    buf = (torch.zeros if fill else torch.empty)(max(total, 16), dtype=torch.uint8, device=device)
     return {name: buf[o : o + nb].view(fields[name][1]).view(fields[name][0]) for name, (o, nb) in offs.items()}
 
 
@@ -228,16 +228,18 @@
         if seed is not None:
             torch.manual_seed(seed)
 
-    def reset(self, td: TensorDict | None = None, batch_size=None) -> TensorDict:
+    def reset(self, td: TensorDict | None = None, batch_size=None, init_state: bool = True) -> TensorDict:
         if batch_size is None:
             batch_size = [] if td is None else td.batch_size
         if td is None or (td.is_empty() if hasattr(td, "is_empty") else len(td) == 0):
             td = self.generator(batch_size=batch_size)
         batch_size = [batch_size] if isinstance(batch_size, int) else list(batch_size)
         td = td.to(self.device)
-        out = self._reset(td, batch_size=batch_size)
+        if not init_state and not self.accepts_deferred_state():
+            raise NotImplementedError(f"{self.name}: reset(init_state=False) is served for the environments of the fused rollout step")
+        out = self._reset(td, batch_size=batch_size) if init_state else self._reset(td, batch_size=batch_size, init_state=False)
         if "terminated" not in out.keys():
-            out.set("terminated", torch.zeros_like(out["done"]))
+            out.set("terminated", torch.zeros_like(out["done"]) if init_state else torch.empty_like(out["done"]))
         return out
 
     def step(self, td: TensorDict) -> dict:
@@ -248,6 +250,14 @@
         if check_solution:
             self.check_solution_validity(td, actions)
         return self._get_reward(td, actions) if horizon is None else self._get_reward(td, actions, horizon=horizon)
+
+    def accepts_deferred_state(self) -> bool:
+        import inspect
+
+        try:
+            return "init_state" in inspect.signature(type(self)._reset).parameters
+        except (TypeError, ValueError):
+            return False
 
     def accepts_reward_horizon(self) -> bool:
         import inspect
@@ -315,12 +325,12 @@
     def _default_generator(self, **kw):
         return TSPGenerator(**kw)
 
-    def _reset(self, td: TensorDict, batch_size) -> TensorDict:
+    def _reset(self, td: TensorDict, batch_size, init_state: bool = True) -> TensorDict:
         init_locs = td["locs"].contiguous()
         device = init_locs.device
         b = init_locs.shape[0]
         num_loc = init_locs.shape[-2]
-        z = _zero_state(device, first_node=((b,), torch.int64), current_node=((b,), torch.int64), i=((b, 1), torch.int64),
+        z = _zero_state(device, init_state, first_node=((b,), torch.int64), current_node=((b,), torch.int64), i=((b, 1), torch.int64),
                         reward=((b, 1), torch.float32), done=((b,), torch.bool))
         return TensorDict(
             {
@@ -328,7 +338,7 @@
                 "first_node": z["first_node"],
                 "current_node": z["current_node"],
                 "i": z["i"],
-                "action_mask": torch.ones((b, num_loc), dtype=torch.bool, device=device),
+                "action_mask": (torch.ones if init_state else torch.empty)((b, num_loc), dtype=torch.bool, device=device),
                 "reward": z["reward"],
                 "done": z["done"],
             },
@@ -358,24 +368,26 @@
     def _default_generator(self, **kw):
         return CVRPGenerator(**kw)
 
-    def _reset(self, td: TensorDict, batch_size) -> TensorDict:
+    def _reset(self, td: TensorDict, batch_size, init_state: bool = True) -> TensorDict:
         device = td["locs"].device
         b = td["locs"].shape[0]
         n = td["locs"].shape[-2] + 1
+        zeros = torch.zeros if init_state else torch.empty
         td_reset = TensorDict(
             {
                 "locs": torch.cat((td["depot"][:, None, :], td["locs"]), -2).contiguous(),
                 "demand": td["demand"].contiguous(),
-                "current_node": torch.zeros(b, 1, dtype=torch.long, device=device),
-                "used_capacity": torch.zeros((b, 1), device=device),
+                "current_node": zeros(b, 1, dtype=torch.long, device=device),
+                "used_capacity": zeros((b, 1), device=device),
                 "vehicle_capacity": torch.full((b, 1), self.generator.vehicle_capacity, device=device),
-                "visited": torch.zeros((b, n), dtype=torch.uint8, device=device),
-                "action_mask": torch.zeros((b, n), dtype=torch.bool, device=device),
-                "done": torch.zeros((b,), dtype=torch.bool, device=device),
+                "visited": zeros((b, n), dtype=torch.uint8, device=device),
+                "action_mask": zeros((b, n), dtype=torch.bool, device=device),
+                "done": zeros((b,), dtype=torch.bool, device=device),
             },
             batch_size=[b],
         )
-        self.get_action_mask(td_reset)
+        if init_state:
+            self.get_action_mask(td_reset)
         return td_reset
 
     def _step(self, td: TensorDict) -> TensorDict:
diff --git a/rl4co_amd/envspec.py b/rl4co_amd/envspec.py
--- a/rl4co_amd/envspec.py
+++ b/rl4co_amd/envspec.py
@@ -59,6 +59,7 @@
     length_reward: bool = False
     depot_flag: str | None = None
     unfold: bool = False
+    fused_step: tuple[str, ...] = ()
     replay: bool = True
     no_teacher: str | None = None
 
@@ -94,11 +95,13 @@
     EnvSpec("tsp", _lib.ENV_TSP, False, lambda n: n,
             _fields("B", ("first_node", "traj", "i64", "first_node", "B"), ("i", "traj", "i64", "step_i", "B1")),
             None, ("tsp_step", ("action_mask", "first_node", "current_node", "i", "done")),
-            ("locs",), init="all", ctx_first=True, fixed_horizon=True, length_reward=True, unfold=True),
+            ("locs",), init="all", ctx_first=True, fixed_horizon=True, length_reward=True, unfold=True,
+            fused_step=("action_mask", "first_node", "current_node", "i", "done")),
     EnvSpec("cvrp", _lib.ENV_CVRP, True, lambda n: 2 * n, _fields("B1", *_CVRP_FIELDS),
             Scalar("used_capacity", "vehicle_capacity"),
             ("cvrp_step", ("demand", "used_capacity", "vehicle_capacity", "visited", "current_node", "action_mask", "done")),
-            ("locs", "demand"), features=(("demand", False, 1),), length_reward=True, unfold=True),
+            ("locs", "demand"), features=(("demand", False, 1),), length_reward=True, unfold=True,
+            fused_step=("action_mask", "current_node", "done", "used_capacity", "visited")),
     EnvSpec("op", _lib.ENV_OP, True, lambda n: n + 2,
             _fields("B1", ("locs", "inst", "f32", "locs", "N2"), ("max_length", "inst", "f32", "max_length", "N"),
                     ("tour_length", "traj", "f32", "used_capacity", "B"), _I, _VISITED),
diff --git a/rl4co_amd/graph.py b/rl4co_amd/graph.py
--- a/rl4co_amd/graph.py
+++ b/rl4co_amd/graph.py
@@ -22,10 +22,14 @@
         self.static_in = TensorDict({k: v.clone() for k, v in example.items() if torch.is_tensor(v)}, batch_size=[self.batch])
         self.seed_dev = torch.zeros(1, dtype=torch.int64, device=dev)
         self._calls = 0
+        self._fresh_state = False
         side = torch.cuda.Stream(device=dev)
         side.wait_stream(torch.cuda.current_stream())
         with torch.cuda.stream(side), torch.inference_mode():
             for _ in range(max(1, warmup)):
+                self._enqueue()()
+                self._fresh_state = bool(getattr(policy, "last_fused_step", False)) and self._can_defer_state()
+            if self._fresh_state and warmup < 2:
                 self._enqueue()()
         torch.cuda.current_stream().wait_stream(side)
         torch.cuda.synchronize(dev)
@@ -43,7 +47,15 @@
         if self._fused:
             assert all(pe.t[k] is v for k, v in self._captured.items()), "the capture re-packed the encoder weights"
 
+    def _can_defer_state(self) -> bool:
+        fn = getattr(self.env, "accepts_deferred_state", None)
+        return bool(fn is not None and fn())
+
     def _enqueue(self):
+        if self._fresh_state:
+            td = self.env.reset(self.static_in, init_state=False)
+            return self.policy(td, self.env, phase="test", decode_type=self.decode_type, philox_seed_dev=self.seed_dev,
+                               _defer_finish=True, _fresh_state=True, **self.kw)
         td = self.env.reset(self.static_in)
         return self.policy(td, self.env, phase="test", decode_type=self.decode_type, philox_seed_dev=self.seed_dev,
                            _defer_finish=True, **self.kw)
diff --git a/rl4co_amd/kernels.py b/rl4co_amd/kernels.py
--- a/rl4co_amd/kernels.py
+++ b/rl4co_amd/kernels.py
@@ -1,6 +1,7 @@
 from __future__ import annotations
 
 import ctypes as C
+import os
 
 import torch
 from torch import Tensor
@@ -274,6 +275,11 @@
     top_k: int = 0,
     top_p: float = 0.0,
     kept_bits: Tensor | None = None,
+    fresh: bool = False,
+    pad_outputs: bool = False,
+    fused_check: bool = False,
+    fused_reward: Tensor | None = None,
+    fused_locs: Tensor | None = None,
 ) -> None:
     sp = spec(cache.env_name)
     a = _lib.AmDecodeArgs()
@@ -359,8 +365,32 @@
         if tuple(kept_bits.shape) != (b, actions.shape[1], words) or not kept_bits.is_contiguous():
             raise ValueError(f"kept_bits must be a contiguous [{b}, {actions.shape[1]}, {words}] int32 tensor")
         a.kept_bits, a.kept_words = _ptr(kept_bits), words
+    a.fresh, a.pad_outputs, a.fused_check = int(bool(fresh)), int(bool(pad_outputs)), int(bool(fused_check))
+    if fused_reward is not None:
+        _dev(fused_reward, torch.float32, "fused_reward"), _dev(fused_locs, torch.float32, "fused_locs")
+        if tuple(fused_reward.shape) != (b,) or tuple(fused_locs.shape) != (cache.num_instances, n, 2):
+            raise ValueError(f"fused_reward must be [{b}] and fused_locs [{cache.num_instances}, {n}, 2], got "
+                             f"{tuple(fused_reward.shape)} and {tuple(fused_locs.shape)}")
+        a.fused_reward, a.fused_locs = _ptr(fused_reward), _ptr(fused_locs)
     st = _lib.lib().rl4co_am_decode(C.byref(a), _stream())
     _lib.check(st, "rl4co_am_decode")
+
+
+def fused_step_available(cache: FoldedCache, b: int, n: int, *, max_steps: int, variant: str = "auto", top_k: int = 0,
+                         top_p: float = 0.0, all_logps: bool = False, entropy: bool = False) -> bool:
+    if os.environ.get("RL4CO_FUSED_STEP", "1").strip() == "0":
+        return False
+    sp = spec(cache.env_name)
+    if not sp.fused_step or cache.unfold or max_steps <= 1 or not cache.kvl.is_cuda:
+        return False
+    a = _lib.AmDecodeArgs()
+    a.env, a.B, a.B_inst, a.N = sp.env_id, b, cache.num_instances, n
+    a.max_steps, a.variant = int(max_steps), VARIANT_IDS[variant]
+    a.cache_dtype = _lib.dtype_id(cache.kvl.dtype)
+    a.top_k, a.top_p = decoding_filter(top_k, top_p, n)
+    a.all_logps = 1 if all_logps else None
+    a.entropy = 1 if entropy else None
+    return _lib.lib().rl4co_am_decode_variant(C.byref(a)) == VARIANT_IDS["stream"]
 
 
 def decoding_filter(top_k, top_p, n: int) -> tuple[int, float]:
diff --git a/rl4co_amd/policy.py b/rl4co_amd/policy.py
--- a/rl4co_amd/policy.py
+++ b/rl4co_amd/policy.py
@@ -9,7 +9,7 @@
 
 from . import kernels as K
 from .cache import FoldedCache, build_folded_cache, canonical_env
-from .envs import RL4COEnvBase, get_env
+from .envs import CVRPEnv, RL4COEnvBase, TSPEnv, get_env
 from .envspec import customer_features, rem_base, spec
 from .tensordict import TensorDict
 
@@ -305,6 +305,10 @@
 
 
 _KNOWN_DECODE_TYPES = ("greedy", "sampling", "multistart_greedy", "multistart_sampling", "evaluate")
+
+
+_FUSED_CHECKS = (TSPEnv.check_solution_validity, CVRPEnv.check_solution_validity)
+_FUSED_REWARDS = (TSPEnv._get_reward,)
 
 
 def _cuda_tensors(objs):
@@ -437,7 +441,7 @@
     def _max_horizon(env_name: str, n: int) -> int:
         return spec(env_name).horizon(n)
 
-    def _initial_state(self, td, num_starts: int):
+    def _initial_state(self, td, num_starts: int, built_by_kernel: tuple = ()):
         s = max(num_starts, 1)
         st = {}
         for f in spec(self.env_name).fields:
@@ -446,6 +450,9 @@
                 st[f.key] = (x.float() if f.dtype == "f32" else x).contiguous()
                 continue
             x = x if f.shape == "BN" else x.reshape(-1)
+            if f.key in built_by_kernel:
+                st[f.key] = torch.empty((s * x.shape[0], *x.shape[1:]), dtype=x.dtype, device=x.device)
+                continue
             st[f.key] = x.clone(memory_format=torch.contiguous_format) if s == 1 else x.unsqueeze(0).expand(s, *x.shape).reshape(s * x.shape[0], *x.shape[1:]).contiguous()
         return st
 
@@ -610,14 +617,21 @@
                                                       torch.bfloat16 if (regime == torch.bfloat16 and cache_dtype != torch.float16)
                                                       else torch.float32, fold=self.fold)
         self.last_ctx_elem_bytes = cache.ctx_cur.element_size() if cache.ctx_cur is not None else 4
-        state = self._initial_state(td, n_rep)
         horizon = min(self._max_horizon(self.env_name, n), max_steps)
         if sp.depot_flag is not None and not getattr(env, sp.depot_flag, False):
             horizon = min(horizon, n - 1)
+        t0 = 1 if (multistart and n_rep >= 1) else 0
+        fused = (mode != "evaluate" and not grad_path and not store_all_logp and device.type == "cuda" and t0 == 0
+                 and K.fused_step_available(cache, b, n, max_steps=horizon, variant=getattr(self, "decode_variant", "auto"),
+                                            top_k=top_k, top_p=top_p))
+        fresh = bool(decoding_kwargs.pop("_fresh_state", False))
+        if fresh and not fused:
+            raise RuntimeError("_fresh_state: this call is not served by the fused rollout step; pass the state of env.reset()")
+        self.last_fused_step = fused
+        state = self._initial_state(td, n_rep, sp.fused_step if fresh else ())
         status = torch.zeros(6, dtype=torch.int32, device=device)
         err = status[:1]
 
-        t0 = 1 if (multistart and n_rep >= 1) else 0
         if mode == "evaluate":
             given = actions.contiguous()
             tmax = t0 + given.shape[1]
@@ -626,8 +640,8 @@
         else:
             forced = None
             tmax = horizon
-        out_actions = torch.zeros((b, tmax), dtype=torch.int64, device=device)
-        logps = torch.zeros((b, tmax), dtype=torch.float32, device=device)
+        out_actions = (torch.empty if fused else torch.zeros)((b, tmax), dtype=torch.int64, device=device)
+        logps = (torch.empty if fused else torch.zeros)((b, tmax), dtype=torch.float32, device=device)
         all_logps = torch.zeros((b, tmax, n), dtype=torch.float32, device=device) if store_all_logp else None
         kept_bits = (torch.full((b, tmax, 4 * ((n + 127) // 128)), -1, dtype=torch.int32, device=device)
                      if (grad_path and filtered) else None)
@@ -649,6 +663,14 @@
         if self.decode_events is not None:
             ev0, ev1 = torch.cuda.Event(enable_timing=True), torch.cuda.Event(enable_timing=True)
             ev0.record()
+        native_env = isinstance(env, RL4COEnvBase)
+        checked = bool(native_env and calc_reward and env.check_solution and not (n_rep > 0 and select_best))
+        early = bool(native_env and sp.length_reward and calc_reward and mode != "evaluate"
+                     and (checked or not env.check_solution) and not (n_rep > 0 and select_best)
+                     and env.accepts_reward_horizon())
+        fused_check = fused and checked and type(env).check_solution_validity in _FUSED_CHECKS
+        fused_reward = (torch.empty(b, dtype=torch.float32, device=device)
+                        if (fused and early and sp.fixed_horizon and type(env)._get_reward in _FUSED_REWARDS) else None)
         K.am_decode(
             cache, state, mode=mode, max_steps=tmax - t0, t0=t0, actions=out_actions, logps=logps, err=err,
             tanh_clipping=tanh_clipping, temperature=temperature, mask_inner=self.decoder.mask_inner,
@@ -656,20 +678,19 @@
             forced_actions=forced, all_logps=all_logps, steps_summary=status[2:6],
             variant=getattr(self, "decode_variant", "auto"),
             **(dict(top_k=top_k, top_p=top_p, kept_bits=kept_bits) if filtered else {}),
+            **(dict(fresh=fresh, pad_outputs=True, fused_check=fused_check, fused_reward=fused_reward,
+                    fused_locs=None if fused_reward is None else td["locs"].contiguous()) if fused else {}),
         )
         if self.decode_events is not None:
             ev1.record()
             self.decode_events.append((ev0, ev1))
-        native_env = isinstance(env, RL4COEnvBase)
-        checked = bool(native_env and calc_reward and env.check_solution and not (n_rep > 0 and select_best))
-        if checked:
+        if checked and not fused_check:
             env.check_solution_validity(td, out_actions, err=err)
         td_early = reward_early = None
-        if (native_env and sp.length_reward and calc_reward and mode != "evaluate"
-                and (checked or not env.check_solution) and not (n_rep > 0 and select_best)
-                and env.accepts_reward_horizon()):
+        if early:
             td_early = self._final_td(td, state, n_rep)
-            reward_early = env.get_reward(td_early, out_actions, check_solution=False, horizon=(status[2:3], t0))
+            reward_early = (fused_reward if fused_reward is not None else
+                            env.get_reward(td_early, out_actions, check_solution=False, horizon=(status[2:3], t0)))
         if self._bwd_err is not None and self._bwd_err.device == device:
             status[:1].bitwise_or_(self._bwd_err)
             self._bwd_err.zero_()
```

New measurement: 137.1 million instance·step/s. -1.9%, worse.
